# mountain/qingdai

Measured on AMD Instinct MI355X. Metric: simulated planet-days/sec at 721x1440 f64, higher is better.
Workload: dtype f64; 1 GPU; 721x1440 seed-42 planet, dt=300 s: forcing + time_step(Teq, dt, albedo) with QD_ENERGY_W=1 QD_CLOUD_COUPLE=1 + slab-ocean coupling + driver-side precipitation/cloud/albedo diagnostics (run_simulation.py:1766-1934,2063-2146) (BASELINE configs[2]; loop order of benchmark_jax.py:124-158); ocean_n_sub=13, parallelism=lat-bands x1

## Files before the change

include/qingdai_hip.h:

```cpp
#ifndef QINGDAI_HIP_H
#define QINGDAI_HIP_H

#include <stddef.h>
#include <stdint.h>

#ifdef __cplusplus
extern "C" {
#endif

#define QD_ABI_VERSION 1

typedef struct qd_ctx* qd_handle;

typedef struct qd_grid_desc {
    int32_t n_lat, n_lon;
    int32_t row0, n_rows, halo;
    int32_t device;
    int32_t rank, world;
} qd_grid_desc;

enum qd_field {
    QD_F_U = 0, QD_F_V, QD_F_H, QD_F_TS, QD_F_Q, QD_F_CLOUD, QD_F_HICE,
    QD_F_ISR, QD_F_ISR_A, QD_F_ISR_B, QD_F_TEQ, QD_F_ALBEDO,
    QD_F_OLR, QD_F_EFLUX, QD_F_PCOND, QD_F_LH, QD_F_LHREL, QD_F_CLOUD_EFF,
// ... 45 lines not shown
int qd_device_count(void);
int qd_create(const qd_grid_desc* desc, const qd_params* params, double q_init_rh, qd_handle* out);
int qd_destroy(qd_handle h);
const char* qd_last_error(qd_handle h);

int qd_upload(qd_handle h, int field, const void* host_global, size_t bytes);
int qd_download(qd_handle h, int field, void* host_global, size_t bytes);
int qd_set_params(qd_handle h, const qd_params* params, size_t sizeof_params);
int qd_get_step_counter(qd_handle h, int64_t* atmos_counter, int64_t* ocean_counter);
int qd_set_step_counter(qd_handle h, int64_t atmos_counter, int64_t ocean_counter);

int qd_forcing(qd_handle h, const double star_a[3], const double star_b[3], double theta, int with_teq);
int qd_simple_albedo(qd_handle h, double ocean_albedo);
int qd_atmos_step(qd_handle h, double dt, int has_albedo);
int qd_ocean_step(qd_handle h, double dt, int compute_qnet, int use_ice_mask, int inject_sst);
int qd_driver_physics(qd_handle h, double dt);
int qd_hydrology_commit(qd_handle h, double dt);
int qd_step_n(qd_handle h, int n, double dt, int flags, const double* stars);
int qd_last_ocean_nsub(qd_handle h, int* n_sub);
int qd_sync(qd_handle h);

int qd_op_laplacian(qd_handle h, const double* F, int cos_kind, double* out);
int qd_op_hyperdiffuse(qd_handle h, const double* F, const double* k4_row, double k4_scalar, double dt,
                       int n_substeps, int cos_kind, double* out);
int qd_op_advect(qd_handle h, const double* field, const double* u, const double* v, double dt,
                 int cos_kind, double* out);
int qd_op_shapiro(qd_handle h, const double* F, int n, double* out);
int qd_op_zonal_filter(qd_handle h, const double* F, double cutoff, double damp, double* out);
int qd_op_divergence(qd_handle h, const double* u, const double* v, double* out);
int qd_op_vorticity(qd_handle h, const double* u, const double* v, double* out);
int qd_op_gaussian(qd_handle h, const double* F, double sigma, int mode_wrap, double* out);
int qd_op_median_positive(qd_handle h, const double* x, double dflt, double* out);
int qd_median_state(qd_handle h, double* out64);

int qd_band_insolation(qd_handle h, int nb, const double* specA, const double* specB, const double* tray, double* out_host_or_null);

typedef struct qd_eco_params {
    double k_canopy;
    double leaf_scalar;
    double soil_ref;
    double w_lai;
    double light_update_hours;
    double recompute_lai_delta;
    int32_t substep_every_nphys;
    int32_t albedo_couple;
    int32_t bands_couple;
    int32_t water_couple;
    int32_t use_lai;
    int32_t map_f32;
} qd_eco_params;
int qd_eco_configure(qd_handle h, const qd_eco_params* p, size_t sizeof_params);
int qd_eco_set_lai_layers(qd_handle h, const double* layers, int n_planes, int init);
int qd_eco_substep(qd_handle h, double dt);
int qd_eco_banded_alpha(qd_handle h, int nb, const double* r_eff, const double* w_b);
int qd_eco_get_state(qd_handle h, double out[5]);
int qd_eco_set_state(qd_handle h, const double in[3]);

int qd_indiv_configure(qd_handle h, int n_cells, const int32_t* sample_j, const int32_t* sample_i, int n_indiv,
                       const int32_t* cell_index, const double* Ab, const double* tol, int nb, const double* specA,
                       const double* specB, const double* tray, int substeps_per_day, double day_seconds, double soil_cap,
                       int ab_f32);
int qd_indiv_substep(qd_handle h, double dt, int* fired_or_null);
int qd_indiv_download(qd_handle h, double* E_day, double* stress_days);
int qd_indiv_upload(qd_handle h, const double* E_day, const double* stress_days);

int qd_phyto_configure(qd_handle h, int n_species, double K_h, double adv_alpha);
// ... 266 lines not shown
```

qingdai_amd/_lib.py:

```python
from __future__ import annotations

import ctypes
import os

from .params import qd_params

_HERE = os.path.dirname(os.path.abspath(__file__))
LIB_PATH = os.environ.get("QD_LIB_PATH") or os.path.join(_HERE, "libqingdai_hip.so")

FIELDS = ["U", "V", "H", "TS", "Q", "CLOUD", "HICE", "ISR", "ISR_A", "ISR_B", "TEQ", "ALBEDO",
          "OLR", "EFLUX", "PCOND", "LH", "LHREL", "CLOUD_EFF", "FRICTION", "CSMAP", "BASE_ALBEDO", "ELEVATION",
          "UO", "VO", "ETA", "SST", "QNET", "PRECIP", "CLOUD_FROM_P", "CLOUD_SRC", "W_LAND", "S_SNOW", "C_SNOW",
          "S_SNOW_NEXT", "MELT", "P_RAIN", "GLACIER", "RUNOFF",
          "ECO_LAI", "ECO_LAI_SNAP", "ECO_F", "ECO_EDAY", "ECO_ALPHA", "ECO_ALPHA_BANDED", "WATER_ALPHA",
          "ECO_AGE", "ECO_SEEDBANK", "ECO_GATE", "PHYTO_N", "KD490"]
F = {n: i for i, n in enumerate(FIELDS)}
F["LAND_MASK"] = 100
F["ICE_MASK"] = 101
F.update({"ECO_DIV_LS": 110, "ECO_DIV_ALPHA": 111, "ECO_DIV_BC": 112, "ECO_DIV_SUMMARY": 113})
R_SUM, R_COSMEAN, R_MAX, R_MIN, R_MAXABS = 0, 1, 2, 3, 4

SYMBOLS = [
    "qd_abi_version", "qd_device_count", "qd_create", "qd_destroy", "qd_last_error", "qd_upload", "qd_download", "qd_set_params",
    "qd_get_step_counter", "qd_set_step_counter", "qd_forcing", "qd_simple_albedo", "qd_atmos_step",
    "qd_ocean_step", "qd_driver_physics", "qd_hydrology_commit", "qd_step_n", "qd_last_ocean_nsub", "qd_sync",
    "qd_op_laplacian", "qd_op_hyperdiffuse", "qd_op_advect", "qd_op_shapiro", "qd_op_zonal_filter", "qd_op_divergence",
    "qd_op_vorticity", "qd_op_gaussian", "qd_op_median_positive", "qd_median_state", "qd_reduce", "qd_energy_diagnostics", "qd_energy_diagnostics_last", "qd_band_insolation",
    "qd_comm_unique_id", "qd_comm_init", "qd_comm_init_local", "qd_comm_stats", "qd_comm_allreduce_count", "qd_comm_grouped_sum_count", "qd_comm_init_shm", "qd_comm_host_allreduce_count", "qd_hostring_open", "qd_hostring_allreduce",
    "qd_hostring_close", "qd_comm_barrier", "qd_comm_allreduce_max", "qd_peer_export", "qd_peer_connect", "qd_comm_peer_stats", "qd_comm_peer_carried", "qd_peer_selftest", "qd_peer_disable", "qd_tune_reload",
    "qd_plansim_create", "qd_plansim_destroy", "qd_plansim_plan", "qd_plansim_mark", "qd_plansim_margin", "qd_plansim_segments",
    "qd_plansim_pop_exchange", "qd_plansim_segments_rows",
    "qd_eco_configure", "qd_eco_set_lai_layers", "qd_eco_substep", "qd_eco_banded_alpha", "qd_eco_get_state", "qd_eco_set_state",
    "qd_indiv_configure", "qd_indiv_substep", "qd_indiv_download", "qd_indiv_upload",
    "qd_phyto_configure", "qd_phyto_upload", "qd_phyto_download", "qd_phyto_advect_diffuse",
    "qd_phyto_daily_configure", "qd_phyto_daily", "qd_phyto_daily_schedule", "qd_phyto_daily_log", "qd_phyto_daily_download_bands",
    "qd_phyto_daily_state", "qd_phyto_daily_insolation",
    "qd_eco_daily_configure", "qd_eco_daily_set_layers", "qd_eco_daily_get_layers", "qd_eco_daily_step", "qd_eco_daily_schedule",
    "qd_eco_daily_log", "qd_eco_daily_state", "qd_eco_daily_speciate",
    "qd_eco_state_restore",
    "qd_indiv_daily_configure", "qd_indiv_daily_step", "qd_indiv_daily_log", "qd_indiv_daily_weights", "qd_indiv_daily_state",
    "qd_eco_diversity", "qd_eco_diversity_on", "qd_eco_diversity_download",
    "qd_truecolor_configure", "qd_truecolor_render", "qd_truecolor_download",
    "qd_stateframe_configure", "qd_stateframe_scan", "qd_stateframe_render", "qd_stateframe_download",
    "qd_tiles_configure", "qd_tiles_set_plane", "qd_tiles_available", "qd_tiles_scan", "qd_tiles_order_stats", "qd_tiles_render", "qd_tiles_download",
    "qd_budget_diag_configure", "qd_budget_diag_schedule", "qd_budget_diag_log", "qd_budget_diag_reset",
    "qd_route_configure", "qd_route_free", "qd_route_reset", "qd_route_accumulate", "qd_route_event", "qd_route_schedule",
    "qd_route_download", "qd_route_events",
    "qd_hydronet_build", "qd_hydronet_sweeps",
    "qd_topogen_smooth", "qd_topogen_build", "qd_topogen_last_ms",
    "qd_copy_ceiling", "qd_timing_enable", "qd_timing_select", "qd_timing_get", "qd_timing_reset",
]


class qd_eco_params(ctypes.Structure):
    _fields_ = ([(n, ctypes.c_double) for n in ("k_canopy", "leaf_scalar", "soil_ref", "w_lai", "light_update_hours",
                                                 "recompute_lai_delta")] +
                [(n, ctypes.c_int32) for n in ("substep_every_nphys", "albedo_couple", "bands_couple", "water_couple", "use_lai", "map_f32")])


class qd_phyto_daily_params(ctypes.Structure):
# ... 169 lines not shown
    lib.qd_eco_daily_state.argtypes = [vp, ctypes.POINTER(i64)]
    lib.qd_eco_daily_speciate.argtypes = [vp, i32, ctypes.c_double, dp]
    lib.qd_indiv_daily_configure.argtypes = [vp, ctypes.POINTER(qd_indiv_daily_params), sz, ip, ip]
    lib.qd_indiv_daily_step.argtypes = [vp, vp]
    lib.qd_indiv_daily_log.argtypes = [vp, dp, i32, ip]
    lib.qd_indiv_daily_weights.argtypes = [vp, dp, i32]
    lib.qd_indiv_daily_state.argtypes = [vp, ctypes.POINTER(i64)]
    lib.qd_eco_diversity.argtypes = [vp, vp, i32, i32, dp, dp]
    lib.qd_eco_diversity_on.argtypes = [vp, i32, i32, u8p, vp, i32, i32, dp, dp]
    lib.qd_eco_diversity_download.argtypes = [vp, i32, dp, sz]
    lib.qd_truecolor_configure.argtypes = [vp, ctypes.POINTER(qd_truecolor_params), sz, dp, dp, dp, u8p]
    lib.qd_truecolor_render.argtypes = [vp, i32, dp, dp]
    lib.qd_truecolor_download.argtypes = [vp, i32, vp, sz]
    lib.qd_stateframe_configure.argtypes = [vp, ctypes.POINTER(qd_stateframe_params), sz, u8p]
    lib.qd_stateframe_scan.argtypes = [vp, dp, ctypes.POINTER(i64)]
    lib.qd_stateframe_render.argtypes = [vp, ctypes.POINTER(qd_stateframe_table), sz, dp, i32]
    lib.qd_stateframe_download.argtypes = [vp, i32, vp, sz]
    lib.qd_tiles_configure.argtypes = [vp, dbl, dp, i32, i32]
    lib.qd_tiles_set_plane.argtypes = [vp, dp]
    lib.qd_tiles_available.argtypes = [vp, ip]
    lib.qd_tiles_scan.argtypes = [vp, ctypes.POINTER(qd_tile_ref), i32, dp, ctypes.POINTER(i64)]
    lib.qd_tiles_order_stats.argtypes = [vp, i32, i32, ctypes.POINTER(i64), i32, dp, ctypes.POINTER(i64)]
    lib.qd_tiles_render.argtypes = [vp, ctypes.POINTER(qd_tile_desc), sz, i32, i32]
    lib.qd_tiles_download.argtypes = [vp, i32, vp, sz]
    lib.qd_budget_diag_configure.argtypes = [vp, i32, u8p]
    lib.qd_budget_diag_schedule.argtypes = [vp, i32, ip]
    lib.qd_budget_diag_log.argtypes = [vp, dp, i32, ip]
    lib.qd_budget_diag_reset.argtypes = [vp]
    lib.qd_comm_unique_id.argtypes = [vp, sz]
    lib.qd_comm_init.argtypes = [vp, vp, sz]
    lib.qd_comm_barrier.argtypes = [vp]
    lib.qd_comm_init_local.argtypes = [ctypes.POINTER(vp), i32]
    lib.qd_median_state.argtypes = [vp, dp]
    lib.qd_comm_stats.argtypes = [vp, ctypes.POINTER(i32)]
    lib.qd_comm_allreduce_count.argtypes = [vp, ctypes.POINTER(i32)]
    lib.qd_comm_grouped_sum_count.argtypes = [vp, ctypes.POINTER(i32)]
    lib.qd_comm_init_shm.argtypes = [vp, ctypes.c_char_p]
    lib.qd_comm_host_allreduce_count.argtypes = [vp, ctypes.POINTER(i32)]
    lib.qd_hostring_open.argtypes = [ctypes.c_char_p, i32, i32, ctypes.POINTER(vp)]
    lib.qd_hostring_allreduce.argtypes = [vp, dp, i32, i32]
    lib.qd_hostring_close.argtypes = [vp]
    lib.qd_comm_allreduce_max.argtypes = [vp, dp, i32]
    lib.qd_tune_reload.argtypes = [vp]
    lib.qd_peer_export.argtypes = [vp, vp, sz]
    lib.qd_peer_connect.argtypes = [vp, vp, sz, i32]
    lib.qd_peer_selftest.argtypes = [vp, i32, ctypes.POINTER(ctypes.c_longlong)]
    lib.qd_peer_disable.argtypes = [vp]
    lib.qd_comm_peer_stats.argtypes = [vp, ctypes.POINTER(i32), ctypes.POINTER(i32)]
    lib.qd_comm_peer_carried.argtypes = [vp]
    lib.qd_plansim_create.argtypes = [ctypes.POINTER(qd_grid_desc), ctypes.POINTER(vp)]
    lib.qd_plansim_destroy.argtypes = [vp]
    lib.qd_plansim_plan.argtypes = [vp, ip, ip, i32, i32]
    lib.qd_plansim_mark.argtypes = [vp, ip, i32, i32]
    lib.qd_plansim_margin.argtypes = [vp, i32]
    lib.qd_plansim_segments.argtypes = [vp, i32, ip]
    lib.qd_plansim_pop_exchange.argtypes = [vp, ip, i32, ip]
    lib.qd_plansim_segments_rows.argtypes = [vp, i32, i32, ip]
    lib.qd_route_configure.argtypes = [vp, ctypes.POINTER(qd_route_plan), sz]
    lib.qd_route_free.argtypes = [vp]
    lib.qd_route_reset.argtypes = [vp]
    lib.qd_route_accumulate.argtypes = [vp, dbl]
    lib.qd_route_event.argtypes = [vp, dbl, i32]
    lib.qd_route_schedule.argtypes = [vp, i32, dp]
    lib.qd_route_download.argtypes = [vp, i32, dp, sz]
    lib.qd_route_events.argtypes = [vp, dp, i32, ip]
    lib.qd_hydronet_build.argtypes = [vp, i32, i32, u8p, dp, dbl, i32, dp, dp, dp, dbl, dp, ip, ip, u8p, ip, ip, i32,
# ... 15 lines not shown
```

qingdai_amd/csrc/qd_api.hip:

```cpp
#include "qd_span.h"
#include <chrono>
#include <atomic>
#include <cstring>
#include <cstdio>
#include <cstdlib>
#include <algorithm>

thread_local std::string g_qd_create_err;

int qd_fail(qd_ctx* c, const char* what, hipError_t e) {
    std::string m = what ? what : "error";
    if (e != hipSuccess) { m += ": "; m += hipGetErrorString(e); }
    if (c) c->err = m; else g_qd_create_err = m;
    return -1;
}

static hipEvent_t qd_get_event(qd_ctx* c) {
    if (!c->ev_free.empty()) { hipEvent_t e = c->ev_free.back(); c->ev_free.pop_back(); return e; }
    hipEvent_t e = nullptr;
    hipEventCreate(&e);
    return e;
}
QdScope::QdScope(qd_ctx* c_, const char* n, bool attach_) : c(c_), name(n), attach(attach_) {
    on = c->timing == 1;
// ... 260 lines not shown
    { const int r = geti("QD_TAIL_RP", 0); if (r >= 3) t.tail_rp = r; }
    t.tail_v = geti("QD_TAIL_V", 0) == 1 ? 1 : 0;
    t.tail_general = geti("QD_TAIL_GENERAL", 0) == 1 ? 1 : 0;
    t.stream_r_dyn = std::max(0, geti("QD_STREAM_R_DYN", 0));
    t.stream_r_ocn = std::max(0, geti("QD_STREAM_R_OCN", 0));
    t.stream_vb = geti("QD_STREAM_VB", -1);
    { const int b = geti("QD_MED_BLOCKS", 0); if (b >= 16) t.med_blocks = b; }
    t.shapiro_r = std::max(0, geti("QD_SHAPIRO_R", 0));
    t.tile_tr = std::max(0, geti("QD_TILE_TR", 0));
    t.fused_r = std::max(0, geti("QD_FUSED_R", 0));
    t.fused_seq = geti("QD_FUSED_SEQ", 0) == 1 ? 1 : 0;
    t.fused_norot = geti("QD_FUSED_NOROT", 0) == 1 ? 1 : 0;
    t.stream_no_pair = geti("QD_STREAM_NO_PAIR", 0) == 1 ? 1 : 0;
}
extern "C" int qd_tune_reload(qd_handle c) { if (!c) return -1; qd_read_tuning(c); c->tile = QdTileShape{0, 0, 0, 0}; return 0; }

extern "C" int qd_create(const qd_grid_desc* d, const qd_params* params, double q_init_rh, qd_handle* out) {
    if (!d || !params || !out) return qd_fail(nullptr, "qd_create: null argument");
    if (d->n_lat < 5 || d->n_lon < 4) return qd_fail(nullptr, "qd_create: grid too small (need n_lat>=5, n_lon>=4)");
    if (d->row0 < 0 || d->n_rows < 1 || d->row0 + d->n_rows > d->n_lat || d->halo < 0)
        return qd_fail(nullptr, "qd_create: bad latitude band");
    const bool full = (d->row0 == 0 && d->n_rows == d->n_lat);
    if (full && d->halo != 0) return qd_fail(nullptr, "qd_create: a whole-globe handle takes halo = 0");
    if (!full && d->n_rows + 2 * d->halo > d->n_lat) return qd_fail(nullptr, "qd_create: band + 2 halos taller than the grid");
    if (!full && d->halo < 5) return qd_fail(nullptr, "qd_create: band handles need halo >= 5 rows");
    int ndev = 0;
    if (hipGetDeviceCount(&ndev) != hipSuccess || ndev == 0) return qd_fail(nullptr, "qd_create: no HIP device visible");
    if (d->device < 0 || d->device >= ndev) return qd_fail(nullptr, "qd_create: bad device ordinal");
    qd_ctx* c = new qd_ctx();
    c->desc = *d; c->p = *params;
    { const char* ef = std::getenv("QD_FUSED"); if (ef && ef[0] == '0') c->use_fused = 0; }
    { const char* ef = std::getenv("QD_FUSED_FAST"); if (ef) c->fused_fast = std::atoi(ef); }
    { const char* ef = std::getenv("QD_TAIL_ACC"); if (ef) c->tail_acc = std::atoi(ef); }
    { const char* ef = std::getenv("QD_SHAPIRO_STREAM"); if (ef) c->shapiro_stream = std::atoi(ef); }
    { const char* ef = std::getenv("QD_OCN_TAIL"); if (ef) c->ocn_tail = std::atoi(ef); }
    if (c->ocn_tail != 0) c->ocn_tail = 1;
    { const char* ef = std::getenv("QD_OCN_FUSED"); if (ef) c->ocn_fused = ef[0] == '1' ? 1 : 0; }
    { const char* ef = std::getenv("QD_BAND_TAIL"); if (ef) c->band_tail = ef[0] == '0' ? 0 : 1; }
    qd_read_tuning(c);
    { const char* ef = std::getenv("QD_GROUP_SUMS"); if (ef) c->group_sums = ef[0] == '0' ? 0 : 1; }
    c->geo = QdGeom{d->n_lat, d->n_lon, d->row0, d->n_rows, d->halo, full ? 1 : 0, d->row0 - d->halo, d->n_rows + 2 * d->halo};
    c->own_row0 = d->row0; c->own_nrows = d->n_rows;
    auto bail = [&](const char* w, hipError_t e) { qd_fail(nullptr, w, e); qd_destroy(c); return -1; };
    hipError_t e;
    if ((e = hipSetDevice(d->device)) != hipSuccess) return bail("hipSetDevice", e);
    if ((e = hipStreamCreate(&c->stream)) != hipSuccess) return bail("hipStreamCreate", e);
    { int ncu = 0; c->n_cu = (hipDeviceGetAttribute(&ncu, hipDeviceAttributeMultiprocessorCount, d->device) == hipSuccess && ncu > 0) ? ncu : 256; }
    const size_t cells = c->geo.cells() + (size_t)QD_PAD_ROWS * c->geo.nlon;
    for (int f = 0; f < QD_F_COUNT_F64; ++f) {
        if ((e = hipMalloc(&c->f[f], cells * sizeof(double))) != hipSuccess) return bail("hipMalloc field", e);
        hipMemsetAsync(c->f[f], 0, cells * sizeof(double), c->stream);
    }
    for (int s = 0; s < QD_NSCRATCH; ++s) {
        if ((e = hipMalloc(&c->scratch[s], cells * sizeof(double))) != hipSuccess) return bail("hipMalloc scratch", e);
        hipMemsetAsync(c->scratch[s], 0, cells * sizeof(double), c->stream);
    }
    if ((e = hipMalloc(&c->land, cells)) != hipSuccess) return bail("hipMalloc mask", e);
    if ((e = hipMalloc(&c->icemask, cells)) != hipSuccess) return bail("hipMalloc mask", e);
    hipMemsetAsync(c->land, 0, cells, c->stream); hipMemsetAsync(c->icemask, 0, cells, c->stream);
    if (build_tables(c)) return bail("table allocation", hipErrorOutOfMemory);
    if ((e = hipMalloc(&c->k4_atm, (size_t)5 * d->n_lat * sizeof(double))) != hipSuccess) return bail("hipMalloc", e);
    if ((e = hipMalloc(&c->k4_ocn, (size_t)3 * d->n_lat * sizeof(double))) != hipSuccess) return bail("hipMalloc", e);
    c->red_blocks = (12 + (d->n_lon + QD_BLOCK - 1) / QD_BLOCK) * c->geo.lrows() + 64;
    if ((e = hipMalloc(&c->red_partial, (size_t)c->red_blocks * sizeof(double))) != hipSuccess) return bail("hipMalloc", e);
    if ((e = hipMalloc(&c->dscal, QD_S_COUNT * sizeof(double))) != hipSuccess) return bail("hipMalloc", e);
    if ((e = hipMalloc(&c->dcount, 32 * sizeof(unsigned long long))) != hipSuccess) return bail("hipMalloc", e);
    if ((e = hipMalloc(&c->eta_acc, 512 * sizeof(unsigned long long))) != hipSuccess) return bail("hipMalloc", e);
    hipMemsetAsync(c->eta_acc, 0, 512 * sizeof(unsigned long long), c->stream);
    if ((e = hipMalloc(&c->hist, 2 * QD_HIST_BINS * sizeof(unsigned int))) != hipSuccess) return bail("hipMalloc", e);
    if ((e = hipMalloc(&c->sel_state, 8 * sizeof(unsigned long long))) != hipSuccess) return bail("hipMalloc", e);
    hipMemsetAsync(c->dscal, 0, QD_S_COUNT * sizeof(double), c->stream);
    hipMemsetAsync(c->dcount, 0, 32 * sizeof(unsigned long long), c->stream);
    hipMemsetAsync(c->hist, 0, 2 * QD_HIST_BINS * sizeof(unsigned int), c->stream);
    hipMemsetAsync(c->sel_state, 0, 8 * sizeof(unsigned long long), c->stream);
    { const char* ef = std::getenv("QD_TAIL_FIX"); if (ef) c->tail_fix = ef[0] == '0' ? 0 : 1; }
    c->fix_dense = 256.0 * (double)c->geo.cells() / (721.0 * 1440.0);
    { const char* ef = std::getenv("QD_TAIL_FIX_DENSE"); if (ef) c->fix_dense = std::atof(ef); }
    { const char* ef = std::getenv("QD_LAZY_DIAG"); if (ef) c->lazy_diag = ef[0] == '0' ? 0 : 1; }
    if (c->tail_fix) {
        if ((e = hipMalloc(&c->fix_count, 64)) != hipSuccess) return bail("hipMalloc", e);
        hipMemsetAsync(c->fix_count, 0, 64, c->stream);
        if ((e = hipMalloc(&c->fix_list, c->geo.cells() * 3 * sizeof(unsigned long long))) != hipSuccess) return bail("hipMalloc", e);
    }
    if (!full) {
        if ((e = hipMalloc(&c->med_pred, 64 * sizeof(double))) != hipSuccess) return bail("hipMalloc", e);
        hipMemsetAsync(c->med_pred, 0, 64 * sizeof(double), c->stream);
        if ((e = hipMalloc(&c->med_gather, (size_t)std::max(1, d->world) * 4096 * sizeof(double))) != hipSuccess) return bail("hipMalloc", e);
        if ((e = hipMalloc(&c->sel_ccount, 2 * sizeof(unsigned int))) != hipSuccess) return bail("hipMalloc", e);
        hipMemsetAsync(c->sel_ccount, 0, 2 * sizeof(unsigned int), c->stream);
        { const char* ef = std::getenv("QD_MEDIAN_PREDICT"); if (ef && ef[0] == '0') c->med_predict = 0; }
    }
    if (full) {
        if ((e = hipMalloc(&c->sel_cand, 2 * cells * sizeof(double))) != hipSuccess) return bail("hipMalloc", e);
        if ((e = hipMalloc(&c->sel_ccount, 2 * sizeof(unsigned int))) != hipSuccess) return bail("hipMalloc", e);
        hipMemsetAsync(c->sel_ccount, 0, 2 * sizeof(unsigned int), c->stream);
        if ((e = hipMalloc(&c->med_pred, 64 * sizeof(double))) != hipSuccess) return bail("hipMalloc", e);
        hipMemsetAsync(c->med_pred, 0, 64 * sizeof(double), c->stream);
        { const char* ef = std::getenv("QD_MEDIAN_PREDICT"); if (ef && ef[0] == '0') c->med_predict = 0; }
        { const char* ef = std::getenv("QD_MERGE_POINTWISE"); if (ef) c->merge_pointwise = ef[0] == '0' ? 0 : 1; }
        { const char* ef = std::getenv("QD_HOIST_PRECIP"); if (ef) c->hoist_precip = ef[0] == '0' ? 0 : 1; }
        { const char* ef = std::getenv("QD_SIDE_STREAM"); if (ef) c->side_stream_on = ef[0] == '0' ? 0 : 1; }
// ... 425 lines not shown
}
extern "C" int qd_op_divergence(qd_handle c, const double* u, const double* v, double* out) { return seam_divvort(c, u, v, out, 0); }
extern "C" int qd_op_vorticity(qd_handle c, const double* u, const double* v, double* out) { return seam_divvort(c, u, v, out, 1); }

extern "C" int qd_op_gaussian(qd_handle c, const double* F, double sigma, int mode_wrap, double* out) {
    if (!c || !F || !out) return -1;
    hipSetDevice(c->desc.device);
    if (seam_in(c, c->scratch[10], F)) return -1;
    if (qd_gaussian(c, c->scratch[10], c->scratch[11], c->scratch[12], sigma, mode_wrap, 0)) return -1;
    return seam_out(c, c->scratch[11], out);
}

extern "C" int qd_op_median_positive(qd_handle c, const double* x, double dflt, double* out) {
    if (!c || !x || !out) return -1;
    hipSetDevice(c->desc.device);
    if (seam_in(c, c->scratch[10], x)) return -1;
    qd_median_positive_dev(c, c->scratch[10], dflt, QD_S_MED_OUT, 0, 0.0, 0);
    QD_HIP(c, hipMemcpyAsync(c->hpin, c->dscal + QD_S_MED_OUT, sizeof(double), hipMemcpyDeviceToHost, c->stream));
    QD_HIP(c, hipStreamSynchronize(c->stream));
    *out = c->hpin[0];
    return 0;
}

extern "C" int qd_median_state(qd_handle c, double* out64) {
    if (!c || !out64) return -1;
    hipSetDevice(c->desc.device);
    for (int k = 0; k < 16 * 4; ++k) out64[k] = 0.0;
    if (!c->med_pred) return 0;
    QD_HIP(c, hipStreamSynchronize(c->stream));
    QD_HIP(c, hipMemcpy(out64, c->med_pred, sizeof(double) * 16 * 4, hipMemcpyDeviceToHost));
    return 0;
}

extern "C" int qd_reduce(qd_handle c, int field, int op, double* out) {
    if (!c || !out) return -1;
    if (field < 0 || field >= QD_F_COUNT_F64) return qd_fail(c, "qd_reduce: unknown field");
    hipSetDevice(c->desc.device);
    double v = 0;
    const int op1 = (op == QD_R_COSWEIGHTED_MEAN) ? 1 : (op == QD_R_SUM ? 0 : (op == QD_R_MAX ? 2 : (op == QD_R_MIN ? 3 : 4)));
    if (qd_reduce_field(c, c->f[field], op1, &v)) return -1;
    if (op == QD_R_COSWEIGHTED_MEAN) v = v / (c->wsum_all + 1e-15);
    *out = v;
    return 0;
}

extern "C" int qd_band_insolation(qd_handle c, int nb, const double* specA, const double* specB, const double* tray, double* out_host) {
    if (!c || !specA || !specB || !tray) return -1;
    hipSetDevice(c->desc.device);
    return qd_band_insolation_impl(c, nb, specA, specB, tray, out_host);
}
extern "C" int qd_energy_diagnostics_last(qd_handle c, double* out) {
    if (!c || !out) return -1;
    for (int k = 0; k < 10; ++k) out[k] = c->last_diag[k];
    return 0;
}
extern "C" int qd_energy_diagnostics(qd_handle c, double* out) {
    if (!c || !out) return -1;
    hipSetDevice(c->desc.device);
    return qd_energy_diag_impl(c, out);
}

extern "C" int qd_copy_ceiling(qd_handle c, size_t bytes, int reps, double* gbs) {
    if (!c || !gbs || bytes == 0 || reps < 1) return -1;
    hipSetDevice(c->desc.device);
    void *a = nullptr, *b = nullptr;
    if (hipMalloc(&a, bytes) != hipSuccess || hipMalloc(&b, bytes) != hipSuccess) { if (a) hipFree(a); return qd_fail(c, "qd_copy_ceiling: hipMalloc"); }
// ... 32 lines not shown
```

qingdai_amd/csrc/qd_blockred.h:

```cpp
#pragma once
#include "qd_internal.h"

__device__ __forceinline__ double qd_wave_sum(double x) {
#pragma unroll
    for (int o = 32; o > 0; o >>= 1) x += __shfl_down(x, o, 64);
    return x;
}
__device__ __forceinline__ double qd_wave_max(double x) {
#pragma unroll
    for (int o = 32; o > 0; o >>= 1) { double y = __shfl_down(x, o, 64); x = (y > x) ? y : x; }
    return x;
}
__device__ __forceinline__ double qd_wave_fmin(double x) {
#pragma unroll
    for (int o = 32; o > 0; o >>= 1) x = fmin(x, __shfl_down(x, o, 64));
    return x;
}
__device__ __forceinline__ double qd_wave_fmax(double x) {
#pragma unroll
    for (int o = 32; o > 0; o >>= 1) x = fmax(x, __shfl_down(x, o, 64));
    return x;
}

__device__ __forceinline__ double qd_pow_np(double x, double e) {
// ... 36 lines not shown
    const int q = threadIdx.x;
    if (q < count) partial[(size_t)q * nblk + b] = qd_block_total(sm, q, qd_red_op(op, q));
}

template <int N>
__device__ __forceinline__ void qd_planes_strided(const double* __restrict__ partial, int nblk, int planes, const QdRedOp* op, double (&v)[N]) {
#pragma unroll
    for (int q = 0; q < N; ++q)
        if (q < planes) {
            const QdRedOp o = qd_red_op(op, q);
            double a = qd_red_identity(o);
            for (int k = threadIdx.x; k < nblk; k += QD_BLOCK) a = qd_red_join(a, partial[(size_t)q * nblk + k], o);
            v[q] = a;
        }
}
template <int N>
__device__ __forceinline__ void qd_block_totals(double (&v)[N], const QdRedOp* op) {
    __shared__ double sm[N][QD_BLOCK / 64];
    qd_block_gather(sm, v, N, op);
    if (threadIdx.x == 0)
        for (int q = 0; q < N; ++q) v[q] = qd_block_total(sm, q, qd_red_op(op, q));
}

__device__ __forceinline__ void qd_planes_by_wave(const double* __restrict__ partial, int nblk, int planes, double* tot) {
    const int lane = threadIdx.x & 63, wv = threadIdx.x >> 6;
    for (int q = wv; q < planes; q += QD_BLOCK / 64) {
        double a = 0.0;
        for (int k = lane; k < nblk; k += 64) a += partial[(size_t)q * nblk + k];
        a = qd_wave_sum(a);
        if (lane == 0) tot[q] = a;
    }
    __syncthreads();
}
```

qingdai_amd/csrc/qd_fused.h:

```cpp
#pragma once
#include "qd_internal.h"

struct QdDynArgs {
    const double *u, *v, *h, *fric, *q, *cloud;
    double *uo, *vo, *ho, *qo, *co;
    const double* k4row[5];
    double k4s[5];
    int skip[5];
    double g, a, dt, dlat, dlon, f_min;
    double inv_dlon, inv_2dlon, inv_dlat, inv_2dlat, pgf_y;
    int primitive;
    int fast;
    QdTileShape ts;
};


struct QdOcnArgs {
    const double *uo, *vo, *eta, *taux, *tauy;
    const uint8_t* land;
    double *uo_out, *vo_out, *eta_out;
    const double* k4row[3];
    double k4s[3];
    int skip[3];
    double a, g, dlat, dlon, sub_dt, rhoH, r_bot;
    double inv_2dlon, inv_2dlat, inv_a, inv_rhoH;
    const double* eta_mean;
    double eta_cap;
    int fast;
    QdTileShape ts;
};


QdTileShape qd_pick_tile(const QdGeom& G);
int qd_launch_dyn_hyper(qd_ctx* c, QdDynArgs& P, int margin);
int qd_launch_ocn_hyper(qd_ctx* c, QdOcnArgs& P, int margin);

bool qd_stream_ok(const qd_ctx* c, int margin);
bool qd_ocn_stream_ok(const qd_ctx* c, int margin);
int qd_launch_dyn_stream(qd_ctx* c, const QdDynArgs& P, int margin);
int qd_launch_ocn_stream(qd_ctx* c, const QdOcnArgs& P, int margin);
bool qd_ocn_stream_ok_list(const qd_ctx* c, const QdSegList& S);
int qd_launch_ocn_stream_list(qd_ctx* c, const QdOcnArgs& P, const QdSegList& S);
```

qingdai_amd/csrc/qd_fused.hip:

```cpp
#include "qd_internal.h"
#include "qd_device.h"
#include "qd_fused.h"
#include "qd_wave.h"
#include <cstdlib>
#include <algorithm>

#define QD_TC 58
#define QD_S 64
#define QD_FBLOCK 512
#define QD_NW (QD_FBLOCK / 64)

struct QdLapC {
    double dphi, dlam, a;
    int n;
    const double* poleA;
    const double *sA, *sP, *sQ;
};

__device__ __forceinline__ int qd_pole_type(int g, int n) { return g == 0 ? 0 : (g == 1 ? 1 : (g == n - 2 ? 2 : (g == n - 1 ? 3 : -1))); }

__device__ __forceinline__ double qd_lap_lds_pole(const double* __restrict__ p, int g, int rho, const QdLapC& C) {
    const int S = QD_S, t = qd_pole_type(g, C.n);
    const double cc = p[0];
    double ahi = cc, alo, bhi, blo = cc;
// ... 672 lines not shown
    QdDynArgs Q = P;
    QD_ROWS(c, margin, G, Q.ts.ntr = (G.nrows + TR - 1) / TR; hipLaunchKernelGGL(k_dyn_hyper<TR>, dim3(Q.ts.ntr * Q.ts.ntc), dim3(QD_FBLOCK),
                                             QdPl<TR>::lds_bytes, c->stream, G, c->tabs, Q));
}
template <int TR> static void launch_ocn(qd_ctx* c, const QdOcnArgs& P, int margin) {
    static bool once[QD_MAX_DEVICES] = {false};
    const int dv = c->desc.device >= 0 && c->desc.device < QD_MAX_DEVICES ? c->desc.device : 0;
    if (!once[dv]) { hipFuncSetAttribute((const void*)k_ocn_hyper<TR>, hipFuncAttributeMaxDynamicSharedMemorySize, (int)QdPl<TR>::lds_bytes); once[dv] = c->desc.device == dv; }
    QdOcnArgs Q = P;
    QD_ROWS(c, margin, G, Q.ts.ntr = (G.nrows + TR - 1) / TR; hipLaunchKernelGGL(k_ocn_hyper<TR>, dim3(Q.ts.ntr * Q.ts.ntc), dim3(QD_FBLOCK),
                                             QdPl<TR>::lds_bytes, c->stream, G, c->tabs, Q));
}

#define QD_DISPATCH_TR(tr, CALL)                                                                              \
    switch (tr) {                                                                                             \
        case 6: CALL(6); break; case 10: CALL(10); break; case 14: CALL(14); break; case 18: CALL(18); break; \
        case 22: CALL(22); break; case 26: CALL(26); break; case 30: CALL(30); break; case 38: CALL(38); break; \
        default: return qd_fail(c, "fused kernel: no instantiation for this tile height");                    \
    }

int qd_launch_dyn_hyper(qd_ctx* c, QdDynArgs& P, int margin) {
    if (qd_stream_ok(c, margin)) return qd_launch_dyn_stream(c, P, margin);
    qd_tile_init(c);
    P.ts = c->tile;
    P.fast = c->fused_fast != 0;
    QdScope sc(c, "k_dyn_hyper");
#define QD_CALL_DYN(N) launch_dyn<N>(c, P, margin)
    QD_DISPATCH_TR(P.ts.tr, QD_CALL_DYN)
    return 0;
}

int qd_launch_ocn_hyper(qd_ctx* c, QdOcnArgs& P, int margin) {
    if (qd_ocn_stream_ok(c, margin)) return qd_launch_ocn_stream(c, P, margin);
    qd_tile_init(c);
    P.ts = c->tile;
    P.fast = c->fused_fast != 0;
    QdScope sc(c, "k_ocn_hyper");
#define QD_CALL_OCN(N) launch_ocn<N>(c, P, margin)
    QD_DISPATCH_TR(P.ts.tr, QD_CALL_OCN)
    return 0;
}
```

qingdai_amd/csrc/qd_internal.h:

```cpp
#pragma once

#include <hip/hip_runtime.h>
#include <hip/hip_ext.h>
#include <stdint.h>
#include <string>
#include <vector>
#include <functional>
#include <map>
#include <unordered_map>
#include <initializer_list>
#include <climits>
#include <cfloat>
#include <cmath>

#include "../../include/qingdai_hip.h"

#define QD_NSCRATCH 16
#define QD_MAX_DEVICES 64
#define QD_PAD_ROWS 8
#define QD_BLOCK 256
#define QD_MAXF 5
#define QD_HIST_BINS 2048

struct QdGeom {
// ... 184 lines not shown
    hipEvent_t med_fork = nullptr, med_done = nullptr;
    unsigned int* hist_b = nullptr; unsigned long long* sel_state_b = nullptr; double* sel_cand_b = nullptr; unsigned int* sel_ccount_b = nullptr;
    int want_pcond_ahead = 0;
    int pcond_ahead = 0;
    int tail_fix = 1;
    unsigned int* fix_count = nullptr;
    unsigned long long* fix_list = nullptr;
    double fix_avg = 0.0;
    double fix_dense = 256.0;
    int64_t fix_probe_at = 0;
    int fix_probe_every = 32;
    int merge_saf = 1;
    void* saf_pending = nullptr;
    int defer_final = 0;
    int merge_final = 1;
    struct { int on = 0; double dt = 0, decay = 0, dfac = 0; } final_pending;
    double* wgmax = nullptr;
    int n_wgmax = 0;
    int side_stream_on = 0;
    hipStream_t side_stream = nullptr;
    hipEvent_t side_fork = nullptr, side_done = nullptr;
    bool side_pending = false;
    double* red_partial_b = nullptr;
    std::function<int()> before_cfl_wait;
    int merge_pointwise = 1;
    double* med_gather = nullptr;
    double* hpin = nullptr;
    double* hpin_rows = nullptr;
    double wsum_ocean = 0, wsum_all = 0;
    int64_t atm_counter = 0, ocn_counter = 0;
    QdTileShape tile{0, 0, 0, 0};
    int use_fused = 1;
    int fused_fast = 1;
    int tail_acc = 1;
    unsigned long long* eta_acc = nullptr;
    int shapiro_stream = 1;
    int ocn_fused = 0;
    int ocn_tail = 1;
    int stream_rows = 0;
    double* qs_tab[2] = {nullptr, nullptr};
    double qs_key[2][8] = {{NAN, 0, 0, 0, 0, 0, 0, 0}, {NAN, 0, 0, 0, 0, 0, 0, 0}};
    std::vector<double> h_lapK[2];
    std::vector<double> h_k4[2];
    QdTune tune;
    int n_cu = 0;
    int qs_wgs_per_cu[3] = {0, 0, 0};
    int cloud_eff_valid = 0;
    int last_nsub = 0;
    void* stage = nullptr; size_t stage_bytes = 0;
    std::unordered_map<const void*, int> vm;
    int own_row0 = 0, own_nrows = 0;
    void* comm = nullptr;
    struct QdLocalGroup* lgroup = nullptr;
    struct QdPeer* peer = nullptr;
    std::vector<struct QdUse> split_pending;
    std::vector<struct QdUse> corefresh;
    int exchanges = 0;
    int allreduces = 0;
    double pub_seq = 0.0;
    double eta_seq = 0.0;
    void* hring = nullptr;
    void* plansim = nullptr;
    int host_allreduces = 0;
    const char* lap_tag = "k_laplacian";
    const char* hyp_tag = "k_hyper_apply";
    int timing = 0;
// ... 77 lines not shown
int qd_allgather_f64(qd_ctx* c, double* buf, int n_per_rank);
bool qd_peer_on(const qd_ctx* c);
int qd_host_allreduce(qd_ctx* c, double* host_vals, int n, int op);
bool qd_has_host_ring(const qd_ctx* c);
extern "C" int qd_hostring_close(void* ring);
void qd_comm_release(qd_ctx* c);
#define QD_ROWS(c, margin, G, ...) do { QdSegs _sg = qd_segments((c), (margin)); for (int _k = 0; _k < _sg.n; ++_k) { const QdGeom& G = _sg.g[_k]; __VA_ARGS__; } } while (0)

static inline dim3 qd_grid2d(const QdGeom& G, int fields = 1) {
    return dim3((G.nlon + QD_BLOCK - 1) / QD_BLOCK, G.nrows, fields);
}

struct QdFieldList {
    const double* in[QD_MAXF];
    double* out[QD_MAXF];
    const double* aux[QD_MAXF];
    const double* k4row[QD_MAXF];
    double k4s[QD_MAXF];
    int n;
};

void qd_launch_laplacian(qd_ctx* c, const QdFieldList& fl, const double* coslat, int m);
void qd_launch_hyper_apply(qd_ctx* c, const QdFieldList& fl, const double* coslat, double sub_dt, int m);
int  qd_hyperdiffuse_fields(qd_ctx* c, double** fields, int n, const double* k4tab, const int* skip,
                            const double* k4s_override, double dt, int nsub, const double* coslat, int m_out);
void qd_launch_shapiro_pass(qd_ctx* c, const QdFieldList& fl, int scrub, int m);
int  qd_shapiro_fields(qd_ctx* c, double** fields, int n, int npass, int m_out);
void qd_launch_advect(qd_ctx* c, const double* u, const double* v, const double* coslat, double dt,
                      const double* f0, double* o0, const double* f1, double* o1, double alpha, int clipq, int m);
void qd_launch_divvort(qd_ctx* c, const double* u, const double* v, double* out, int vort, int m);
int  qd_gaussian(qd_ctx* c, const double* in, double* out, double* tmp, double sigma, int mode_wrap, int m_out, int clip01 = 0,
                 const double* scale_p = nullptr, double scale_k = 1.0);
bool qd_gauss_pair_ok(const qd_ctx* c, double sigma);
int  qd_gaussian_pair(qd_ctx* c, const double* inA, const double* inB, double sigma, int mode_wrap, const double* scA_p, double scA_k,
                      double scB_k, const double* sc, int op, const double* blend5, double* outA, double* outB, double* out0, int m_out = 0);
int  qd_gaussian_swap(qd_ctx* c, double*& field, double*& tmp, double sigma, int mode_wrap, int m_out, int clip01 = 0,
                      const double* scale_p = nullptr, double scale_k = 1.0);
bool qd_gauss_can_fuse(const qd_ctx* c, double sigma);
int  qd_gauss_radius(double sigma);
int  qd_energy_diag_impl(qd_ctx* c, double* host_out);
int  qd_band_insolation_impl(qd_ctx* c, int nb, const double* specA, const double* specB, const double* tray, double* out_host);
int  qd_zonal_filter_fields(qd_ctx* c, double** fields, int nf, double cutoff, double damp, int m);
int  qd_adv_reach(const qd_ctx* c, double dt, double vmax);

int  qd_eco_canopy_impl(qd_ctx* c, double dt);
int  qd_eco_eday_impl(qd_ctx* c, double dt);
int  qd_indiv_substep_impl(qd_ctx* c, double dt, int* fired);
void qd_eco_free(qd_ctx* c);
int  qd_band_copy_in(qd_ctx* c, void* dst, const void* host, size_t esz);
int  qd_phyto_step_impl(qd_ctx* c, double dt);
void qd_phyto_release(qd_ctx* c);
struct QdSpanLane* qd_route_span_begin(qd_ctx* c, int n);
int  qd_route_step_impl(qd_ctx* c, double dt, int s);
void qd_route_release(qd_ctx* c);
struct QdSpanLane* qd_phyto_daily_span_begin(qd_ctx* c, int n, int with_phys);
int  qd_phyto_daily_step_impl(qd_ctx* c, const double* star_row, int use_sst);
void qd_phyto_daily_release(qd_ctx* c);
struct QdSpanLane* qd_eco_daily_span_begin(qd_ctx* c, int n, int with_eco);
int  qd_eco_daily_step_impl(qd_ctx* c, const double* soil_dev);
void qd_eco_daily_release(qd_ctx* c);
bool qd_eco_daily_stack(const qd_ctx* c, const double** L, int* n_species, int* n_layers);
double* qd_eco_daily_share_plane(qd_ctx* c);
double* qd_eco_daily_weights_dev(qd_ctx* c);
double qd_eco_daily_soil_cap(const qd_ctx* c);
double qd_eco_daily_lai_max(const qd_ctx* c);
void qd_eco_daily_adopt(qd_ctx* c, double* L1, double* w1);
struct QdSpanLane* qd_indiv_daily_span_begin(qd_ctx* c, const struct QdSpanLane* daily);
int  qd_indiv_daily_step_impl(qd_ctx* c, const double* soil_dev);
// ... 45 lines not shown
```

qingdai_amd/csrc/qd_ocean.hip:

```cpp
#include <cstdlib>
#include <atomic>
#include <chrono>
#include "qd_internal.h"
#include "qd_device.h"
#include "qd_wave.h"

#include "qd_fluxes.h"
#include "qd_fused.h"
#include "qd_ocntail.h"
#include "qd_band.h"
#include "qd_blockred.h"

QdColP qd_make_colp(const qd_ctx* c, double dt);

__global__ void __launch_bounds__(QD_BLOCK)
k_qnet(QdGeom G, QdColP P, const double* __restrict__ isr, const double* __restrict__ albedo,
       const double* __restrict__ cloud, const double* __restrict__ Ts, const double* __restrict__ h,
       const double* __restrict__ u, const double* __restrict__ v, const uint8_t* __restrict__ land,
       const double* __restrict__ hice, const double* __restrict__ LH, double* __restrict__ qnet,
       uint8_t* __restrict__ icemask) {
    const QdTile tl = qd_tile();
    const int j = tl.seg * QD_BLOCK + threadIdx.x;
    if (j >= G.nlon) return;
    const size_t o = (size_t)qd_lrow(G, G.row0 + tl.row) * G.nlon + j;
// ... 762 lines not shown
        c->last_nsub = n_sub;
    }
    bool fix_now = c->tail_fix && c->fix_count && (!band || band_fix_stats);
    if (fix_now) {
        if (c->fix_avg <= c->fix_dense) c->fix_probe_every = 32;
        else if (step >= c->fix_probe_at) {
            c->fix_probe_at = step + c->fix_probe_every;
            c->fix_probe_every = std::min(256, c->fix_probe_every * 2);
        } else fix_now = false;
    }
    const double sub_dt = dt / n_sub;
    QdOcnP OP{p.a, p.g_ocean, c->dlat, c->dlon, sub_dt, p.rho_w * H, p.r_bot};
    QdHeatP HP{sub_dt, p.K_h, p.rho_w * p.cp_w * H, p.ocean_ice_qfac, p.ocean_use_qnet ? 1 : 0, use_ice_mask ? 1 : 0};
    const bool do_diff = (p.ocean_diff_every > 0) && (step % p.ocean_diff_every == 0);
    const bool do_shap = (p.ocean_shapiro_n > 0) && (p.ocean_shapiro_every > 0) && (step % p.ocean_shapiro_every == 0);
    if (do_diff) { int rc = qd_build_k4_tables(c, dt, true, sub_dt); if (rc) return rc; }
    const double ov[3] = {p.ocean_k4_u, p.ocean_k4_v, p.ocean_k4_eta};
    const int Ro = qd_adv_reach(c, sub_dt, 4.0);

    const bool can_defer = do_diff && c->use_fused && p.ocean_k4_nsub == 1 && !do_shap && c->wsum_ocean > 0.0;
    const bool band_defer = band && can_defer && qd_has_host_ring(c);
    const bool band_tail = band && can_defer && !band_defer && c->ocn_tail == 1 && c->tail_acc && c->band_tail && G0.nlon >= 64 &&
                           G0.halo >= std::max(7, Ro + 2);
    const bool defer_eta = (!band && can_defer) || band_defer || band_tail;
    double* const mean_ptr = band_defer ? c->hpin + 42 : c->dscal + QD_S_ETA_MEAN;
    struct CoRefresh { qd_ctx* c; ~CoRefresh() { c->corefresh.clear(); } } corefresh_guard{c};
    if (band) c->corefresh = {QD_IN(F[QD_F_UO], 0), QD_IN(F[QD_F_VO], 0), QD_IN(F[QD_F_ETA], 0), QD_IN(F[QD_F_SST], 0), QD_IN(taux, 0),
                              QD_IN(tauy, 0), QD_IN(F[QD_F_QNET], 0), QD_IN8(c->icemask, 0)};
    const bool use_tail = c->use_fused && (!band || band_tail) && defer_eta && G0.nlon >= 64 && c->ocn_tail;
    const bool tail_acc = use_tail && c->tail_acc;
    const bool use_fused1 = use_tail && !band && c->ocn_fused && c->ocn_tail == 1 && tail_acc && c->fused_fast == 1 && do_diff &&
                            p.ocean_k4_nsub == 1 && !do_shap && HP.use_q && HP.K_h > 0.0 && qd_ocn_fused_ok(c) &&
                            !c->k4_ocn_skip[0] && !c->k4_ocn_skip[1] && !c->k4_ocn_skip[2];
    for (int s = 0; s < n_sub; ++s) {
        if (use_fused1) {
            QdOcnArgs O;
            O.uo = F[QD_F_UO]; O.vo = F[QD_F_VO]; O.eta = F[QD_F_ETA]; O.taux = taux; O.tauy = tauy; O.land = c->land;
            O.uo_out = qd_scratch(c, 0); O.vo_out = qd_scratch(c, 1); O.eta_out = qd_scratch(c, 6);
            for (int f = 0; f < 3; ++f) {
                const bool sc1 = !(ov[f] != ov[f]);
                O.k4row[f] = sc1 ? nullptr : c->k4_ocn + (size_t)f * G0.nlat;
                O.k4s[f] = sc1 ? ov[f] : 0.0;
                O.skip[f] = c->k4_ocn_skip[f];
            }
            O.a = p.a; O.g = p.g_ocean; O.dlat = c->dlat; O.dlon = c->dlon; O.sub_dt = sub_dt; O.rhoH = p.rho_w * H; O.r_bot = p.r_bot;
            O.inv_2dlon = 1.0 / (2.0 * c->dlon); O.inv_2dlat = 1.0 / (2.0 * c->dlat); O.inv_a = 1.0 / p.a; O.inv_rhoH = 1.0 / (p.rho_w * H);
            O.eta_mean = s > 0 ? mean_ptr : nullptr;
            O.eta_cap = p.eta_cap;
            QdTailArgs A;
            A.uo = O.uo_out; A.vo = O.vo_out; A.eta_in = O.eta_out; A.Ts = F[QD_F_SST]; A.qnet = F[QD_F_QNET]; A.land = c->land; A.ice = c->icemask;
            A.eta = qd_scratch(c, 2); A.Ts_out = qd_scratch(c, 3); A.uo_out = qd_scratch(c, 12); A.vo_out = qd_scratch(c, 13); A.partial = c->red_partial;
            A.a = p.a; A.dlat = c->dlat; A.dlon = c->dlon; A.sub_dt = sub_dt; A.msdtH = -sub_dt * H; A.alpha = p.ocean_adv_alpha;
            A.K_h = HP.K_h; A.rcH = HP.rcH; A.ice_qfac = HP.ice_qfac; A.cap = p.ocean_max_u;
            A.use_q = HP.use_q; A.has_ice = HP.has_ice; A.mean4 = p.ocean_outlier == 0 ? 1 : 0;
            A.r_a = 1.0 / p.a; A.r_dlon = 1.0 / c->dlon; A.r_dlat = 1.0 / c->dlat; A.r_2dlon = 1.0 / (2 * c->dlon); A.r_2dlat = 1.0 / (2 * c->dlat);
            A.r_rcH = 1.0 / HP.rcH;
            A.acc = c->eta_acc; A.mean_out = c->dscal + QD_S_ETA_MEAN; A.wsum = c->wsum_ocean;
            if (qd_launch_ocn_fused(c, O, A)) return -1;
            qd_swap(c, QD_F_UO, 12); qd_swap(c, QD_F_VO, 13); qd_swap(c, QD_F_ETA, 2); qd_swap(c, QD_F_SST, 3);
            continue;
        }
        if (do_diff && c->use_fused && p.ocean_k4_nsub == 1) {
            const QdUse narrow[5] = {QD_IN(F[QD_F_ETA], 5), QD_IN(F[QD_F_UO], 4), QD_IN(F[QD_F_VO], 4), QD_IN(taux, 4), QD_IN(tauy, 4)};
            bool pending = false;
            int m_old = 0;
            if (band_tail) {
                const QdUse wide[8] = {QD_IN(F[QD_F_ETA], 7), QD_IN(F[QD_F_UO], 6), QD_IN(F[QD_F_VO], 6), QD_IN(taux, 6), QD_IN(tauy, 6),
                                       QD_IN(F[QD_F_SST], Ro + 2), QD_IN(F[QD_F_QNET], 0), QD_IN8(c->icemask, 0)};
                if (qd_plan_begin(c, wide, 8, &pending) < 0) return -1;
                if (pending) m_old = qd_plan_peek(c, narrow, 5);
            }
            QdOcnArgs O;
            O.uo = F[QD_F_UO]; O.vo = F[QD_F_VO]; O.eta = F[QD_F_ETA]; O.taux = taux; O.tauy = tauy; O.land = c->land;
            O.uo_out = qd_scratch(c, 0); O.vo_out = qd_scratch(c, 1); O.eta_out = qd_scratch(c, 2);
            for (int f = 0; f < 3; ++f) {
                const bool sc1 = !(ov[f] != ov[f]);
                O.k4row[f] = sc1 ? nullptr : c->k4_ocn + (size_t)f * G0.nlat;
                O.k4s[f] = sc1 ? ov[f] : 0.0;
                O.skip[f] = c->k4_ocn_skip[f];
            }
            O.a = p.a; O.g = p.g_ocean; O.dlat = c->dlat; O.dlon = c->dlon; O.sub_dt = sub_dt; O.rhoH = p.rho_w * H; O.r_bot = p.r_bot;
            O.inv_2dlon = 1.0 / (2.0 * c->dlon); O.inv_2dlat = 1.0 / (2.0 * c->dlat); O.inv_a = 1.0 / p.a; O.inv_rhoH = 1.0 / (p.rho_w * H);
            O.eta_mean = (defer_eta && s > 0) ? mean_ptr : nullptr;
            O.eta_cap = p.eta_cap;
            int m_int = 0;
            bool split = false;
            if (pending) {
                m_int = m_old >= 0 ? m_old : -12;
                const QdSegList Si = qd_segments_rows(c, c->own_row0 - m_int, c->own_nrows + 2 * m_int);
                if (c->own_nrows + 2 * m_int >= 12 && qd_ocn_stream_ok_list(c, Si)) {
                    if (qd_launch_ocn_stream_list(c, O, Si)) return -1;
                    split = true;
                }
                if (qd_plan_end(c)) return -1;
            }
            const int m = qd_plan(c, narrow, 5);
            if (m < 0) return -1;
            if (qd_allreduce_flush(c)) return -1;
            if (split && m > m_int) {
                QdSegList Sb = qd_segments_rows(c, c->own_row0 - m, m - m_int);
                Sb = qd_segments_rows(c, c->own_row0 + c->own_nrows + m_int, m - m_int, Sb);
                if (!qd_ocn_stream_ok_list(c, Sb)) {
                    if (qd_launch_ocn_hyper(c, O, m)) return -1;
                } else if (qd_launch_ocn_stream_list(c, O, Sb)) return -1;
            } else if (!split) {
                if (qd_launch_ocn_hyper(c, O, m)) return -1;
            }
            qd_mark(c, {O.uo_out, O.vo_out, O.eta_out}, m);
            qd_swap(c, QD_F_UO, 0); qd_swap(c, QD_F_VO, 1); qd_swap(c, QD_F_ETA, 2);
        } else {
            {
                QdScope sc(c, "ocean_momentum");
                const int m = qd_plan(c, {QD_IN(F[QD_F_ETA], 1), QD_IN(F[QD_F_UO], 0), QD_IN(F[QD_F_VO], 0), QD_IN(taux, 0),
                                          QD_IN(tauy, 0)});
                if (m < 0) return -1;
                QD_ROWS(c, m, G, hipLaunchKernelGGL(k_ocean_momentum, qd_grid2d(G), blk, 0, c->stream, G, c->tabs, OP,
                                                    F[QD_F_ETA], taux, tauy, c->land, F[QD_F_UO], F[QD_F_VO]));
// ... 23 lines not shown
            QdTailArgs A;
            A.uo = F[QD_F_UO]; A.vo = F[QD_F_VO]; A.Ts = F[QD_F_SST]; A.qnet = F[QD_F_QNET]; A.land = c->land; A.ice = c->icemask;
            A.eta = F[QD_F_ETA]; A.Ts_out = qd_scratch(c, 1); A.uo_out = qd_scratch(c, 2); A.vo_out = qd_scratch(c, 3); A.partial = c->red_partial;
            A.a = p.a; A.dlat = c->dlat; A.dlon = c->dlon; A.sub_dt = sub_dt; A.msdtH = -sub_dt * H; A.alpha = p.ocean_adv_alpha;
            A.K_h = HP.K_h; A.rcH = HP.rcH; A.ice_qfac = HP.ice_qfac; A.cap = p.ocean_max_u;
            A.use_q = HP.use_q; A.has_ice = HP.has_ice; A.mean4 = p.ocean_outlier == 0 ? 1 : 0;
            A.r_a = 1.0 / p.a; A.r_dlon = 1.0 / c->dlon; A.r_dlat = 1.0 / c->dlat; A.r_2dlon = 1.0 / (2 * c->dlon); A.r_2dlat = 1.0 / (2 * c->dlat);
            A.r_rcH = 1.0 / HP.rcH;
            A.acc = tail_acc ? c->eta_acc : nullptr; A.mean_out = c->dscal + QD_S_ETA_MEAN; A.wsum = c->wsum_ocean;
            if (band) {
                const int m = qd_plan(c, {QD_IN(F[QD_F_UO], 2), QD_IN(F[QD_F_VO], 2), QD_IN(F[QD_F_ETA], 0), QD_IN(F[QD_F_SST], Ro + 2),
                                          QD_IN(F[QD_F_QNET], 0), QD_IN8(c->icemask, 0)});
                if (m < 0) return -1;
                A.own0 = c->own_row0; A.own1 = c->own_row0 + c->own_nrows;
                QdSegs S = qd_segments(c, m);
                size_t off = 0;
                QdPeerFold pf;
                const bool folded = qd_peer_fold_begin(c, &pf);
                if (fix_now && S.n == 1) { A.fix_count = c->fix_count; A.fix_list = c->fix_list; }
                for (int k = 0; k < S.n; ++k) {
                    const QdGeom& Gs = S.g[k];
                    const bool owned = Gs.row0 <= c->own_row0 && c->own_row0 < Gs.row0 + Gs.nrows;
                    A.acc = owned ? c->eta_acc : nullptr;
                    A.pf = owned ? pf : QdPeerFold();
                    A.partial = c->red_partial + off;
                    if (qd_launch_ocn_tail(c, Gs, A)) return -1;
                    off += (size_t)qd_ocn_tail_tiles(c, Gs);
                }
                if (!folded && qd_allreduce_sum_deferred(c, c->dscal + QD_S_ETA_MEAN)) return -1;
                if (A.fix_count) qd_mark(c, {F[QD_F_ETA], A.Ts_out, F[QD_F_UO], F[QD_F_VO]}, m);
                else qd_mark(c, {F[QD_F_ETA], A.Ts_out, A.uo_out, A.vo_out}, m);
            } else {
            if (fix_now) { A.fix_count = c->fix_count; A.fix_list = c->fix_list; }
            if (qd_launch_ocn_tail(c, Gown, A)) return -1;
            if (!tail_acc)
                hipLaunchKernelGGL(k_eta_mean_tail, dim3(1), dim3(256), 0, c->stream, c->red_partial, qd_ocn_tail_tiles(c, Gown), c->wsum_ocean,
                                   c->dscal + QD_S_ETA_MEAN);
            }
            qd_swap(c, QD_F_SST, 1);
            if (!A.fix_count) { qd_swap(c, QD_F_UO, 2); qd_swap(c, QD_F_VO, 3); }
        } else if (c->use_fused) {
            QdScope sc(c, "ocean_cont_sst");
            bool band_raw_mean = false;
            const int m = qd_plan(c, {QD_IN(F[QD_F_UO], 1), QD_IN(F[QD_F_VO], 1), QD_IN(F[QD_F_ETA], 0), QD_IN(F[QD_F_SST], Ro)});
            if (m < 0) return -1;
            double* T1 = qd_scratch(c, 0);
            const int own0 = c->own_row0, own1 = c->own_row0 + c->own_nrows;
            const int has_ocean = c->wsum_ocean > 0.0 ? 1 : 0;
            if (!band) {
                const dim3 g2 = qd_grid2d(Gown);
                hipLaunchKernelGGL(k_cont_sstadv, g2, blk, 0, c->stream, Gown, c->tabs, p.a, c->dlat, c->dlon, -sub_dt * H, sub_dt,
                                   p.ocean_adv_alpha, F[QD_F_UO], F[QD_F_VO], c->land, F[QD_F_ETA], F[QD_F_SST], T1, own0, own1,
                                   c->red_partial, (unsigned long long*)nullptr, 0.0, (double*)nullptr);
                if (!defer_eta)
                    hipLaunchKernelGGL(k_eta_mean, dim3(1), blk, 0, c->stream, c->red_partial, (int)(g2.x * g2.y), c->wsum_ocean,
                                       c->dscal + QD_S_ETA_MEAN);
            } else {
                QdSegs S = qd_segments(c, m);
                size_t off = 0;
                for (int k = 0; k < S.n; ++k) {
                    hipLaunchKernelGGL(k_cont_sstadv, qd_grid2d(S.g[k]), blk, 0, c->stream, S.g[k], c->tabs, p.a, c->dlat, c->dlon,
                                       -sub_dt * H, sub_dt, p.ocean_adv_alpha, F[QD_F_UO], F[QD_F_VO], c->land, F[QD_F_ETA],
                                       F[QD_F_SST], T1, own0, own1, c->red_partial + off, (unsigned long long*)nullptr, 0.0,
                                       (double*)nullptr);
                    off += (size_t)S.g[k].nrows * qd_grid2d(S.g[k]).x;
                }
// ... 126 lines not shown
```

qingdai_amd/csrc/qd_ocntail.h:

```cpp
#pragma once
#include "qd_internal.h"
#include "qd_peer_dev.h"

struct QdTailArgs {
    const double *uo, *vo, *Ts, *qnet;
    const uint8_t *land, *ice;
    double *eta, *Ts_out, *uo_out, *vo_out, *partial;
    const double* tab;
    unsigned long long* acc;
    double* mean_out;
    double wsum;
    double a, dlat, dlon, sub_dt, msdtH, alpha, K_h, rcH, ice_qfac, cap;
    double r_a, r_dlon, r_dlat, r_2dlon, r_2dlat, r_rcH;
    int use_q, has_ice, mean4, ntc, R, Rp;
    int nmid, flags;
    int own0, own1;
    const double* eta_in = nullptr;
    unsigned int* fix_count = nullptr;
    unsigned long long* fix_list = nullptr;
    QdPeerFold pf;
};

int qd_ocn_tail_tiles(const qd_ctx* c, const QdGeom& G);
int qd_launch_ocn_tail(qd_ctx* c, const QdGeom& G, QdTailArgs& P);

struct QdOcnArgs;
bool qd_ocn_fused_ok(const qd_ctx* c);
int qd_ocn_fused_tiles(const qd_ctx* c);
int qd_launch_ocn_fused(qd_ctx* c, const QdOcnArgs& O, QdTailArgs& P);
```

qingdai_amd/csrc/qd_ocntail.hip:

```cpp
#include "qd_internal.h"
#include "qd_device.h"
#include "qd_wave.h"
#include "qd_ocntail.h"
#include "qd_stream.h"
#include "qd_blockred.h"
#include <cstdlib>
#include <cstdio>
#include <vector>
#include <cstring>
#include <algorithm>


__device__ __forceinline__ double qt_div(double x, double c, double rc) {
    const double q0 = x * rc;
    const double e = __builtin_fma(-c, q0, x);
    const double q1 = __builtin_fma(e, rc, q0);
    return (q0 - q0 == 0.0) ? q1 : q0;
}

__device__ __forceinline__ double qt_div_fin(double x, double c, double rc) {
    const double q0 = x * rc;
    const double e = __builtin_fma(-c, q0, x);
    return __builtin_fma(e, rc, q0);
}
// ... 561 lines not shown
    const int k = rs - (q.ps > 0 ? 1 : 0);
    if (q.ps > 0 && rs == 0) { W.o0 = lo; W.o1 = lo + q.ps; }
    else if (k < q.nmid) {
        const int M = q.mid1 - q.mid0;
        W.o0 = q.mid0 + (int)(((long long)k * M) / q.nmid);
        W.o1 = q.mid0 + (int)(((long long)(k + 1) * M) / q.nmid);
    } else { W.o0 = q.mid1; W.o1 = hi; }
    const int wv = __builtin_amdgcn_readfirstlane(threadIdx.x >> 6);
    const bool plain = (P.flags & 1) == 0 && W.o0 - 3 - W.lbase >= 0 && W.o1 + 2 - W.lbase <= W.lrows - 1;
    QT_STAMP(0);
    if (wv >= 1) {
        __builtin_amdgcn_s_setprio(2);
        bool general = !(plain && W.o0 >= 3 && W.o1 <= W.n - 3 && P.use_q && P.K_h > 0.0);
        if (!general) {
            const bool edge_lane = W.lane >= 1 && W.lane <= 62 && (W.j == 0 || W.j == W.m - 1);
            general = __builtin_amdgcn_ballot_w64(edge_lane) != 0ull ? qt_sst_fast<true>(P, W) : qt_sst_fast<false>(P, W);
        }
        if (general) qt_sst_wave(G, T, P, W);
        QT_STAMP(2);
        if (!FIX) return;
        __syncthreads();
        return;
    }
    __shared__ unsigned long long s_fix[FIX ? 3 * QT_FIX_STAGE : 1];
    __shared__ unsigned int s_nfix;
    const QtFixW FX{P.fix_count, P.fix_list, s_fix, &s_nfix};
    if (FIX && W.lane == 0) __hip_atomic_store(&s_nfix, 0u, __ATOMIC_RELAXED, __HIP_MEMORY_SCOPE_WAVEFRONT);
    double acc = (plain && W.o0 >= 1 && W.o1 <= W.n - 1) ? qt_currents_fast<FIX>(P, W, FX) : qt_currents_wave<FIX>(T, P, W, FX);
    if (FIX) qt_fix_flush(FX);
    QT_STAMP(2);
    if (FIX) __syncthreads();
    acc = qd_wave_sum(acc);
    if (W.lane == 0) __hip_atomic_store(P.partial + w, acc, __ATOMIC_RELAXED, __HIP_MEMORY_SCOPE_AGENT);
    if (P.acc) {
        const bool last = W.lane == 0 && qd_acc_arrive(P.acc, w, gridDim.x, acc);
        if (__builtin_amdgcn_ballot_w64(last) != 0ull) {
            double mm = qd_acc_finish(P.acc, P.partial, (int)gridDim.x, P.wsum);
            if (P.pf.pbox) mm = qp_fold_sum(P.pf, mm);
            if (W.lane == 0) *P.mean_out = mm;
            if (FIX) {
                const unsigned nfix = __hip_atomic_load(P.fix_count, __ATOMIC_RELAXED, __HIP_MEMORY_SCOPE_AGENT);
                for (unsigned k0 = 0; k0 < nfix; k0 += 512u) {
                    unsigned long long off[8], ub[8], vb[8];
#pragma unroll
                    for (int q = 0; q < 8; ++q) {
                        const unsigned k = k0 + (unsigned)q * 64u + (unsigned)W.lane;
                        const unsigned long long* e = P.fix_list + (size_t)3 * (k < nfix ? k : nfix - 1u);
                        off[q] = __hip_atomic_load(e, __ATOMIC_RELAXED, __HIP_MEMORY_SCOPE_AGENT);
                        ub[q] = __hip_atomic_load(e + 1, __ATOMIC_RELAXED, __HIP_MEMORY_SCOPE_AGENT);
                        vb[q] = __hip_atomic_load(e + 2, __ATOMIC_RELAXED, __HIP_MEMORY_SCOPE_AGENT);
                    }
#pragma unroll
                    for (int q = 0; q < 8; ++q) {
                        if (k0 + (unsigned)q * 64u + (unsigned)W.lane >= nfix) continue;
                        *(unsigned long long*)((char*)const_cast<double*>(P.uo) + off[q]) = ub[q];
                        *(unsigned long long*)((char*)const_cast<double*>(P.vo) + off[q]) = vb[q];
                    }
                }
                if (W.lane == 0) {
                    __hip_atomic_store(P.fix_count, 0u, __ATOMIC_RELAXED, __HIP_MEMORY_SCOPE_AGENT);
                    P.fix_count[4] += nfix; P.fix_count[5] += 1u; if (nfix > P.fix_count[6]) P.fix_count[6] = nfix;
                }
            }
        }
    }
}
// ... 227 lines not shown
    A.G = c->geo;
    if (F.ntc * (1 + F.nmid) > c->red_blocks) return qd_fail(c, "k_ocn_fused: partial buffer too small");
    if (!c->qt_tab || c->qt_tab_a != P.a) {
        if (!c->qt_tab) {
            if (hipMalloc(&c->qt_tab, (size_t)c->geo.nlat * 16 * sizeof(double)) != hipSuccess) return qd_fail(c, "k_ocn_fused: row table");
            c->tab_alloc.push_back(c->qt_tab);
        }
        hipLaunchKernelGGL(k_tail_tab, dim3((c->geo.nlat + 255) / 256), dim3(256), 0, c->stream, c->tabs, c->geo.nlat, P.a, c->qt_tab);
        c->qt_tab_a = P.a;
    }
    P.tab = c->qt_tab; P.own0 = 0; P.own1 = c->geo.nlat; P.flags = 0; P.R = F.R; P.Rp = QFU_PH; P.ntc = F.ntc; P.nmid = F.nmid;
    QdScope sc(c, "ocean_step", true);
#ifdef QT_STAMPS
    static unsigned long long* stamps = nullptr;
    const size_t stamp_words = (size_t)8 * 5 * 8192;
    if (!stamps) { hipMalloc(&stamps, stamp_words * 8); hipMemcpyToSymbol(HIP_SYMBOL(qt_stamp_buf), &stamps, sizeof(stamps)); }
    hipMemsetAsync(stamps, 0, stamp_words * 8, c->stream);
#endif
    QD_LAUNCH_TIMED(sc, k_ocn_fused, dim3(F.ntc * (1 + F.nmid)), dim3(320), c->stream, A, c->tabs, P, F);
#ifdef QT_STAMPS
    if (const char* f = std::getenv("QD_STAMPS_FILE")) {
        std::vector<unsigned long long> h(stamp_words);
        hipStreamSynchronize(c->stream);
        hipMemcpy(h.data(), stamps, stamp_words * 8, hipMemcpyDeviceToHost);
        if (FILE* fp = std::fopen(f, "wb")) { std::fwrite(h.data(), 8, stamp_words, fp); std::fclose(fp); }
    }
#endif
    return 0;
}

static int qt_rows(const qd_ctx* c) { return c->tune.tail_r > 0 ? c->tune.tail_r : 7; }

static bool qt_use_fast(const qd_ctx* c) { return !c->tune.tail_v && c->ocn_tail == 1; }
static int qt_fast_rows(const qd_ctx* c, const QdGeom& G) {
    if (c->tune.tail_r > 0) return c->tune.tail_r;
    const int ntc = (G.nlon + QS_TCF - 1) / QS_TCF;
    const double target = 13.7 * 256;
    const int r = (int)std::lround((double)G.nrows * ntc * 2.0 / target);
    return r < 7 ? 7 : r;
}
static int qt_fast_pole_rows(const qd_ctx* c) { return c->tune.tail_rp; }

int qd_ocn_tail_tiles(const qd_ctx* c, const QdGeom& G) {
    if (qt_use_fast(c))
        return qt_part_strips(qt_partition(G.row0, G.row0 + G.nrows, G.nlat, qt_fast_rows(c, G), qt_fast_pole_rows(c))) * ((G.nlon + QS_TCF - 1) / QS_TCF);
    const int R = qt_rows(c);
    return ((G.nrows + R - 1) / R) * ((G.nlon + QS_TC2 - 1) / QS_TC2);
}

int qd_launch_ocn_tail(qd_ctx* c, const QdGeom& G, QdTailArgs& P) {
    if (G.nlon < 64) return qd_fail(c, "k_ocn_tail: >= 64 columns");
    if (G.full) { P.own0 = 0; P.own1 = G.nlat; }
    QdScope sc(c, "ocean_tail", true);
    const bool fast = qt_use_fast(c);
    if (fast && (!c->qt_tab || c->qt_tab_a != P.a)) {
        if (!c->qt_tab) {
            if (hipMalloc(&c->qt_tab, (size_t)G.nlat * 16 * sizeof(double)) != hipSuccess) return qd_fail(c, "k_ocn_tail_fast: row table");
            c->tab_alloc.push_back(c->qt_tab);
        }
        hipLaunchKernelGGL(k_tail_tab, dim3((G.nlat + 255) / 256), dim3(256), 0, c->stream, c->tabs, G.nlat, P.a, c->qt_tab);
        c->qt_tab_a = P.a;
    }
    P.tab = c->qt_tab;
    P.flags = c->tune.tail_general ? 1 : 0;
    P.R = fast ? qt_fast_rows(c, G) : qt_rows(c);
    P.Rp = qt_fast_pole_rows(c);
    P.ntc = fast ? (G.nlon + QS_TCF - 1) / QS_TCF : (G.nlon + QS_TC2 - 1) / QS_TC2;
    const QtPart part = qt_partition(G.row0, G.row0 + G.nrows, G.nlat, P.R, P.Rp);
    P.nmid = part.nmid;
    const int nrs = fast ? qt_part_strips(part) : (G.nrows + P.R - 1) / P.R;
    if (nrs * P.ntc > c->red_blocks) return qd_fail(c, "k_ocn_tail_stream: partial buffer too small");
#ifdef QT_STAMPS
    static unsigned long long* stamps = nullptr;
    const size_t stamp_words = (size_t)8 * 2 * 8192;
    if (!stamps) { hipMalloc(&stamps, stamp_words * 8); hipMemcpyToSymbol(HIP_SYMBOL(qt_stamp_buf), &stamps, sizeof(stamps)); }
    hipMemsetAsync(stamps, 0, stamp_words * 8, c->stream);
#endif
    if (!fast || !P.acc) { P.fix_count = nullptr; P.fix_list = nullptr; }
    if (fast && P.fix_count) QD_LAUNCH_TIMED(sc, k_ocn_tail_fast<true>, dim3(nrs * P.ntc), dim3(128), c->stream, G, c->tabs, P);
    else if (fast) QD_LAUNCH_TIMED(sc, k_ocn_tail_fast<false>, dim3(nrs * P.ntc), dim3(128), c->stream, G, c->tabs, P);
    else QD_LAUNCH_TIMED(sc, k_ocn_tail_stream<1>, dim3(nrs * P.ntc), dim3(128), c->stream, G, c->tabs, P);
#ifdef QT_STAMPS
    if (const char* f = std::getenv("QD_STAMPS_FILE")) {
        std::vector<unsigned long long> h(stamp_words);
        hipStreamSynchronize(c->stream);
        hipMemcpy(h.data(), stamps, stamp_words * 8, hipMemcpyDeviceToHost);
        if (FILE* fp = std::fopen(f, "wb")) { std::fwrite(h.data(), 8, stamp_words, fp); std::fclose(fp); }
    }
#endif
    return 0;
}
```

qingdai_amd/csrc/qd_physics.hip:

```cpp
#include "qd_internal.h"
#include "qd_band.h"
#include "qd_pointwise.h"
#include "qd_device.h"
#include "qd_saf.h"
#include "qd_fluxes.h"
#include "qd_blockred.h"
QdColP qd_make_colp(const qd_ctx* c, double dt);


__global__ void __launch_bounds__(QD_BLOCK)
k_precip_raw(QdGeom G, QdTabs T, const double* __restrict__ u, const double* __restrict__ v,
             const double* __restrict__ pcond, double a, double dlat, double dlon, double D_crit, double beta,
             const double* __restrict__ scale_p, const unsigned long long* __restrict__ sel_state,
             double* __restrict__ praw, double* __restrict__ pos_out, double* __restrict__ partial,
             const double* __restrict__ orog) {
    __shared__ double sm[2][QD_BLOCK / 64];
    const int i = G.row0 + blockIdx.y;
    const size_t b = (size_t)qd_lrow(G, i) * G.nlon;
    const double w = T.warea[i];
    const bool anypos = sel_state[0] > 0;
    const double scale = qd_max(*scale_p, 1e-12);
    double s_num = 0.0, s_den = 0.0;
    for (int j = threadIdx.x; j < G.nlon; j += QD_BLOCK) {
        const double div = qd_divvort_point(G, T, u, v, i, j, a, dlat, dlon, 0);
        const double pos = qd_max(0.0, -(div - D_crit));
        const double F_div = anypos ? qd_clip(pos / scale, 0.0, 5.0) : 0.0;
        const double Pq = qd_max(0.0, pcond[b + j]);
        const double F_orog = orog ? qd_clip(orog[b + j], 1.0, 3.0) : 1.0;
        const double F = (1.0 + beta * F_div) * F_orog;
        const double pr = Pq * F;
        praw[b + j] = pr;
        pos_out[b + j] = pos;
        s_num += Pq * w;
        s_den += pr * w;
    }
    s_num = qd_wave_sum(s_num); s_den = qd_wave_sum(s_den);
    const int lane = threadIdx.x & 63, wv = threadIdx.x >> 6;
    if (lane == 0) { sm[0][wv] = s_num; sm[1][wv] = s_den; }
    __syncthreads();
    if (threadIdx.x == 0) {
        for (int k = 1; k < QD_BLOCK / 64; ++k) { s_num += sm[0][k]; s_den += sm[1][k]; }
        partial[blockIdx.y] = s_num;
        partial[gridDim.y + blockIdx.y] = s_den;
    }
}

__global__ void __launch_bounds__(QD_BLOCK)
k_orog_factor(QdGeom G, QdTabs T, const double* __restrict__ elev, const double* __restrict__ u, const double* __restrict__ v,
              double a, double dlat, double dlon, double k_orog, double cap, double* __restrict__ out) {
    const QdTile tl = qd_tile();
    const int j = tl.seg * QD_BLOCK + threadIdx.x;
    if (j >= G.nlon) return;
    const int i = G.row0 + tl.row, n = G.nlat;
    const size_t b = (size_t)qd_lrow(G, i) * G.nlon;
    const int jp = qd_wrapc(j + 1, G.nlon), jm = qd_wrapc(j - 1, G.nlon);
    const double dx = a * T.cos6[i] * dlon, dy = a * dlat;
    const double dHdx = (elev[b + jp] - elev[b + jm]) / (2.0 * dx);
    double dHdy = 0.0;
    if (i != 0 && i != n - 1)
        dHdy = (elev[(size_t)qd_lrow(G, i + 1) * G.nlon + j] - elev[(size_t)qd_lrow(G, i - 1) * G.nlon + j]) / (2.0 * dy);
    const double gn = sqrt(dHdx * dHdx + dHdy * dHdy);
    const double nxh = gn > 1e-12 ? dHdx / (gn + 1e-12) : 0.0;
    const double nyh = gn > 1e-12 ? dHdy / (gn + 1e-12) : 0.0;
    out[b + j] = qd_clip(1.0 + k_orog * qd_max(0.0, u[b + j] * nxh + v[b + j] * nyh), 1.0, cap);
}

__global__ void __launch_bounds__(QD_BLOCK)
k_precip_scalars(const double* __restrict__ partial, int n, double wsum, double pq_min, double p_blend, int use_fb,
                 double* __restrict__ out) {
    __shared__ double sm[2][QD_BLOCK / 64];
    double a = 0.0, b = 0.0;
    for (int k = threadIdx.x; k < n; k += QD_BLOCK) { a += partial[k]; b += partial[n + k]; }
    a = qd_wave_sum(a); b = qd_wave_sum(b);
    const int lane = threadIdx.x & 63, wv = threadIdx.x >> 6;
    if (lane == 0) { sm[0][wv] = a; sm[1][wv] = b; }
    __syncthreads();
    if (threadIdx.x == 0) {
        for (int k = 1; k < QD_BLOCK / 64; ++k) { a += sm[0][k]; b += sm[1][k]; }
        const double den = b + 1e-20;
        out[0] = den > 0 ? a / den : 1.0;
        const double pq_mean = a / (wsum + 1e-15);
        out[1] = (use_fb && pq_mean < pq_min) ? p_blend : 0.0;
    }
}

__global__ void __launch_bounds__(QD_BLOCK)
k_scale_field(QdGeom G, const double* __restrict__ in, const double* __restrict__ s, double k, double* __restrict__ out) {
    const QdTile tl = qd_tile();
    const int j = tl.seg * QD_BLOCK + threadIdx.x;
    if (j >= G.nlon) return;
    const size_t o = (size_t)qd_lrow(G, G.row0 + tl.row) * G.nlon + j;
    out[o] = s ? in[o] * (*s) : k * in[o];
}

__global__ void __launch_bounds__(QD_BLOCK)
k_precip_blend(QdGeom G, const double* __restrict__ P, const double* __restrict__ Pdyn, const double* __restrict__ sc,
               double* __restrict__ out) {
    const QdTile tl = qd_tile();
    const int j = tl.seg * QD_BLOCK + threadIdx.x;
    if (j >= G.nlon) return;
    const size_t o = (size_t)qd_lrow(G, G.row0 + tl.row) * G.nlon + j;
    const double al = sc[1];
    double p = P[o];
    if (al != 0.0) p = (1.0 - al) * p + al * Pdyn[o];
    out[o] = qd_max(p, 0.0);
}

__global__ void __launch_bounds__(QD_BLOCK)
k_cloud_from_p(QdGeom G, const double* __restrict__ precip, const double* __restrict__ pref, double cmax,
               double* __restrict__ out) {
    const QdTile tl = qd_tile();
    const int j = tl.seg * QD_BLOCK + threadIdx.x;
    if (j >= G.nlon) return;
    const size_t o = (size_t)qd_lrow(G, G.row0 + tl.row) * G.nlon + j;
    out[o] = cmax * qd_tanh(precip[o] / (*pref + 1e-12));
}
// ... 211 lines not shown
                            c->timing != 1;
    if (pcond_side && qd_pcond_median_side(c, dt)) return -1;
    const bool pcond_pair = part != 1 && !pcond_side && c->want_pcond_ahead && c->med_pair && c->hist_b && c->geo.full && p.cloud_couple &&
                            !isset(p.pcond_ref) && !(isset(p.pref) && p.pref != 0.0);
    if (part != 2) {
        QdScope sc(c, "phys_precip");
        int m = qd_plan(c, {QD_IN(F[QD_F_U], 1), QD_IN(F[QD_F_V], 1), QD_IN(F[QD_F_PCOND], 0)});
        if (m < 0) return -1;
        qd_launch_divvort(c, F[QD_F_U], F[QD_F_V], tmp, 0, m);
        if (qd_median_positive_dev(c, tmp, 1e-12, QD_S_PSCALE, 1, p.D_crit, 2)) return -1;
        const double* orog = nullptr;
        if (p.orog_enable && c->has_elevation) {
            double*& of = c->scratch[8];
            const int mo = qd_plan(c, {QD_IN(F[QD_F_U], 0), QD_IN(F[QD_F_V], 0), QD_IN(F[QD_F_ELEVATION], 1)});
            if (mo < 0) return -1;
            QD_ROWS(c, mo, G, hipLaunchKernelGGL(k_orog_factor, qd_grid2d(G), blk, 0, c->stream, G, c->tabs, F[QD_F_ELEVATION],
                                                 F[QD_F_U], F[QD_F_V], p.a, c->dlat, c->dlon, p.orog_k, 2.0, of));
            qd_mark(c, {of}, mo);
            const int mb = qd_plan(c, {QD_IN(of, R1)});
            if (mb < 0) return -1;
            if (qd_gaussian_swap(c, of, tmp, 1.0, 0, mb)) return -1;
            orog = of;
            m = qd_plan(c, {QD_IN(F[QD_F_U], 1), QD_IN(F[QD_F_V], 1), QD_IN(F[QD_F_PCOND], 0), QD_IN(c->scratch[8], 0)});
            if (m < 0) return -1;
        }
        if (band && m > 0) {
            QdSegs S = qd_segments(c, m);
            const int own0 = c->own_row0, own1 = c->own_row0 + c->own_nrows;
            for (int k = 0; k < S.n; ++k) {
                const QdGeom& G = S.g[k];
                auto run = [&](int r0, int r1) {
                    if (r1 <= r0) return;
                    QdGeom g2 = G; g2.row0 = r0; g2.nrows = r1 - r0;
                    hipLaunchKernelGGL(k_precip_raw, dim3(1, g2.nrows), blk, 0, c->stream, g2, c->tabs, F[QD_F_U], F[QD_F_V],
                                       F[QD_F_PCOND], p.a, c->dlat, c->dlon, p.D_crit, p.p_betadiv, c->dscal + QD_S_PSCALE,
                                       c->dcount, praw, pos, rp + (size_t)2 * G0.lrows(), orog);
                };
                const int a0 = G.row0, a1 = G.row0 + G.nrows;
                if (a1 <= own0 || a0 >= own1) run(a0, a1);
                else { run(a0, std::max(a0, own0)); run(std::min(a1, own1), a1); }
            }
        }
        hipLaunchKernelGGL(k_precip_raw, dim3(1, Gown.nrows), blk, 0, c->stream, Gown, c->tabs, F[QD_F_U], F[QD_F_V],
                           F[QD_F_PCOND], p.a, c->dlat, c->dlon, p.D_crit, p.p_betadiv, c->dscal + QD_S_PSCALE, c->dcount, praw,
                           pos, rp, orog);
        qd_mark(c, {praw, pos}, m);
        if (band && qd_peer_hooks(c)) {
            QdPeerHook H; H.pre = 2; H.partial = rp; H.n = Gown.nrows;
            H.post = 1; H.wsum = c->wsum_all; H.pq_min = p.pq_min; H.p_blend = p.p_blend; H.use_fb = p.p_hybrid_fallback; H.out = c->dscal + QD_S_RENORM;
            c->allreduces++;
            if (qd_peer_allreduce_hooked(c, c->dscal + QD_S_TMP0, 2, 0, H)) return -1;
        } else if (band) {
            hipLaunchKernelGGL(k_precip_rawsums, dim3(1), blk, 0, c->stream, rp, Gown.nrows, c->dscal + QD_S_TMP0);
            if (qd_allreduce_f64(c, c->dscal + QD_S_TMP0, 2, 0)) return -1;
            hipLaunchKernelGGL(k_precip_scalars_post, dim3(1), dim3(64), 0, c->stream, c->dscal + QD_S_TMP0, c->wsum_all, p.pq_min,
                               p.p_blend, p.p_hybrid_fallback, c->dscal + QD_S_RENORM);
        } else {
            hipLaunchKernelGGL(k_precip_scalars, dim3(1), blk, 0, c->stream, rp, Gown.nrows, c->wsum_all, p.pq_min,
                               p.p_blend, p.p_hybrid_fallback, c->dscal + QD_S_RENORM);
        }
        if (qd_gauss_pair_ok(c, 1.0)) {
            const int mg = qd_plan(c, {QD_IN(praw, R1), QD_IN(pos, R1)});
            if (mg < 0) return -1;
            if (qd_gaussian_pair(c, praw, pos, 1.0, 0, c->dscal + QD_S_RENORM, 1.0, p.k_precip, c->dscal + QD_S_RENORM, 1, nullptr,
                                 nullptr, nullptr, F[QD_F_PRECIP], mg)) return -1;
            qd_mark(c, {F[QD_F_PRECIP]}, mg);
        } else if (qd_gauss_can_fuse(c, 1.0)) {
            const int mg = qd_plan(c, {QD_IN(praw, R1), QD_IN(pos, R1)});
            if (mg < 0) return -1;
            if (qd_gaussian_swap(c, praw, tmp, 1.0, 0, mg, 0, c->dscal + QD_S_RENORM)) return -1;
            if (qd_gaussian(c, pos, pdyn, nullptr, 1.0, 0, mg, 0, nullptr, p.k_precip)) return -1;
            QD_ROWS(c, mg, G, hipLaunchKernelGGL(k_precip_blend, qd_grid2d(G), blk, 0, c->stream, G, praw, pdyn,
                                                 c->dscal + QD_S_RENORM, F[QD_F_PRECIP]));
            qd_mark(c, {F[QD_F_PRECIP]}, mg);
        } else {
        QD_ROWS(c, m, G, hipLaunchKernelGGL(k_scale_field, qd_grid2d(G), blk, 0, c->stream, G, praw, c->dscal + QD_S_RENORM, 0.0, praw));
        QD_ROWS(c, m, G, hipLaunchKernelGGL(k_scale_field, qd_grid2d(G), blk, 0, c->stream, G, pos, (const double*)nullptr,
                                            p.k_precip, pdyn));
        qd_mark(c, {pdyn}, m);
        const int mg = qd_plan(c, {QD_IN(praw, R1), QD_IN(pdyn, R1)});
        if (mg < 0) return -1;
        if (qd_gaussian_swap(c, praw, tmp, 1.0, 0, mg)) return -1;
        if (qd_gaussian_swap(c, pdyn, tmp, 1.0, 0, mg)) return -1;
        QD_ROWS(c, mg, G, hipLaunchKernelGGL(k_precip_blend, qd_grid2d(G), blk, 0, c->stream, G, praw, pdyn,
                                             c->dscal + QD_S_RENORM, F[QD_F_PRECIP]));
        qd_mark(c, {F[QD_F_PRECIP]}, mg);
        }
    }
    if (part == 1) return 0;
    {
        QdScope sc(c, "phys_cloud");
        if (isset(p.pref) && p.pref != 0.0) {
            hipMemcpyAsync(c->dscal + QD_S_MED_OUT, &p.pref, sizeof(double), hipMemcpyHostToDevice, c->stream);
        } else if (pcond_pair) {
// ... 185 lines not shown
```

qingdai_amd/csrc/qd_stencil.hip:

```cpp
#include "qd_internal.h"
#include "qd_device.h"
#include "qd_wave.h"
#include <cstdlib>

__global__ void __launch_bounds__(QD_BLOCK)
k_laplacian(QdGeom G, QdFieldList fl, const double* __restrict__ cosf, double dphi, double dlam, double a) {
    const QdTile tl = qd_tile();
    const int j = tl.seg * QD_BLOCK + threadIdx.x;
    if (j >= G.nlon) return;
    const int i = G.row0 + tl.row;
    const int f = tl.fld;
    const size_t o = (size_t)qd_lrow(G, i) * G.nlon + j;
    fl.out[f][o] = qd_lap_point<true>(fl.in[f], G, cosf, i, j, dphi, dlam, a);
}

__global__ void __launch_bounds__(QD_BLOCK)
k_hyper_apply(QdGeom G, QdFieldList fl, const double* __restrict__ cosf, double dphi, double dlam, double a,
              double sub_dt) {
    const QdTile tl = qd_tile();
    const int j = tl.seg * QD_BLOCK + threadIdx.x;
    if (j >= G.nlon) return;
    const int i = G.row0 + tl.row;
    const int f = tl.fld;
    const size_t o = (size_t)qd_lrow(G, i) * G.nlon + j;
    const double L2 = qd_lap_point<true>(fl.in[f], G, cosf, i, j, dphi, dlam, a);
    const double k4 = fl.k4row[f] ? fl.k4row[f][i] : fl.k4s[f];
    const double F0 = qd_nn(fl.aux[f][o]);
    fl.out[f][o] = qd_nn(F0 - (k4 * L2) * sub_dt);
}

void qd_launch_laplacian(qd_ctx* c, const QdFieldList& fl, const double* coslat, int m) {
    QdScope sc(c, c->lap_tag);
    QD_ROWS(c, m, G, hipLaunchKernelGGL(k_laplacian, qd_grid2d(G, fl.n), dim3(QD_BLOCK), 0, c->stream,
                                        G, fl, coslat, c->dlat, c->dlon, c->p.a));
}
// ... 352 lines not shown
    }
}

template <int RR>
static void qd_launch_gauss_rows(qd_ctx* c, const double* in, double* out, const QdGaussW& W, int mode_wrap, int clip01,
                                 const double* scale_p, double scale_k, int m_out) {
    constexpr int OWN = QD_BLOCK - 2 * RR;
    QD_ROWS(c, m_out, G, hipLaunchKernelGGL(k_gauss_rows<RR>, dim3((G.nlon + OWN - 1) / OWN, (G.nrows + QD_GB - 1) / QD_GB),
                                            dim3(QD_BLOCK), 0, c->stream, G, in, out, W, mode_wrap, clip01, scale_p, scale_k));
}

static bool qd_gauss_weights(double sigma, QdGaussW& W) {
    const int r = (int)(4.0 * sigma + 0.5);
    if (r > QD_GAUSS_MAXR) return false;
    W.r = r;
    std::vector<double> phi(2 * r + 1);
    const double s2 = sigma * sigma;
    for (int x = -r; x <= r; ++x) phi[x + r] = std::exp(-0.5 / s2 * (double)(x * x));
    double tot;
    const int m = 2 * r + 1;
    if (m < 8) { tot = 0.0; for (int k = 0; k < m; ++k) tot += phi[k]; }
    else {
        double acc[8];
        for (int k = 0; k < 8; ++k) acc[k] = phi[k];
        int k = 8;
        for (; k < m - (m % 8); k += 8) for (int t = 0; t < 8; ++t) acc[t] += phi[k + t];
        tot = ((acc[0] + acc[1]) + (acc[2] + acc[3])) + ((acc[4] + acc[5]) + (acc[6] + acc[7]));
        for (; k < m; ++k) tot += phi[k];
    }
    for (int k = 0; k <= r; ++k) W.w[k] = phi[r + k] / tot;
    return true;
}

struct QdGaussPairP { int op; double w_mem, w_p, w_src, tend, c_floor; };
template <int RR>
__device__ __forceinline__ void qd_gauss_rows_pass(const QdGeom& G, const double* __restrict__ in, double sc, const double (&w)[RR + 1],
                                                   int mode_wrap, int i0, int nvalid, int jbase, double (*sm)[QD_BLOCK], double (&acc)[QD_GB]) {
    {
        const int s = threadIdx.x;
        const int jj = jbase - RR + s;
        if (jj < G.nlon + RR) {
            const int j = qd_ext(jj, G.nlon, mode_wrap);
            double x[QD_GB + 2 * RR];
#pragma unroll
            for (int q = 0; q < QD_GB + 2 * RR; ++q) {
                const int qq = q < nvalid + 2 * RR ? q : nvalid + 2 * RR - 1;
                x[q] = in[(size_t)qd_lrow(G, qd_ext(i0 - RR + qq, G.nlat, mode_wrap)) * G.nlon + j] * sc;
            }
#pragma unroll
            for (int k = 0; k < QD_GB; ++k) {
                double tmp = x[k + RR] * w[0];
#pragma unroll
                for (int q = RR; q >= 1; --q) tmp += (x[k + RR - q] + x[k + RR + q]) * w[q];
                sm[k][s] = tmp;
            }
        }
    }
    __syncthreads();
    const int c0 = threadIdx.x;
    if (c0 >= RR && c0 < QD_BLOCK - RR) {
#pragma unroll
        for (int k = 0; k < QD_GB; ++k) {
            double a = sm[k][c0] * w[0];
#pragma unroll
            for (int q = RR; q >= 1; --q) a += (sm[k][c0 - q] + sm[k][c0 + q]) * w[q];
            acc[k] = a;
        }
    }
    __syncthreads();
}

template <int RR>
__global__ void __launch_bounds__(QD_BLOCK)
k_gauss_pair(QdGeom G, const double* __restrict__ inA, const double* __restrict__ inB, QdGaussW W, int mode_wrap,
             const double* __restrict__ scA_p, double scA_k, double scB_k, const double* __restrict__ sc, QdGaussPairP P,
             double* __restrict__ outA, double* __restrict__ outB, double* __restrict__ out0) {
    constexpr int OWN = QD_BLOCK - 2 * RR;
    __shared__ double sm[QD_GB][QD_BLOCK];
    const int i0 = G.row0 + (int)blockIdx.y * QD_GB;
    const int nvalid = min(QD_GB, G.row0 + G.nrows - i0);
    const int jbase = (int)blockIdx.x * OWN;
    double w[RR + 1];
#pragma unroll
    for (int k = 0; k <= RR; ++k) w[k] = W.w[k];
    const double al = (P.op == 1) ? sc[1] : 0.0;
    double a[QD_GB], b[QD_GB];
#pragma unroll
    for (int k = 0; k < QD_GB; ++k) { a[k] = 0.0; b[k] = 0.0; }
    qd_gauss_rows_pass<RR>(G, inA, scA_p ? *scA_p : scA_k, w, mode_wrap, i0, nvalid, jbase, sm, a);
    if (P.op != 1 || al != 0.0) qd_gauss_rows_pass<RR>(G, inB, scB_k, w, mode_wrap, i0, nvalid, jbase, sm, b);
    const int c0 = threadIdx.x;
    const int j = jbase + c0 - RR;
    if (c0 < RR || c0 >= QD_BLOCK - RR || j >= G.nlon) return;
#pragma unroll
    for (int k = 0; k < QD_GB; ++k) {
        if (k >= nvalid) break;
        const size_t o = (size_t)qd_lrow(G, i0 + k) * G.nlon + j;
        if (P.op == 1) {
            double p = a[k];
            if (al != 0.0) p = (1.0 - al) * p + al * b[k];
            out0[o] = qd_max(p, 0.0);
        } else {
            const double cp = qd_clip(a[k], 0.0, 1.0), sr = qd_clip(b[k], 0.0, 1.0);
            outA[o] = cp; outB[o] = sr;
            const double c0v = out0[o];
            const double tendency = sr * P.tend;
            double c = (P.w_mem * c0v + P.w_p * cp + P.w_src * qd_clip(c0v + tendency, 0.0, 1.0));
            if (P.c_floor > 0.0) c = qd_max(c, qd_clip(P.c_floor * cp, 0.0, 1.0));
            out0[o] = qd_clip(c, 0.0, 1.0);
        }
    }
}

bool qd_gauss_pair_ok(const qd_ctx* c, double sigma) {
    const int r = qd_gauss_radius(sigma);
    return c->use_fused && c->merge_pointwise && sigma > 1e-15 && c->geo.nlon > 2 * r && (r == 1 || r == 2 || r == 4);
}
int qd_gaussian_pair(qd_ctx* c, const double* inA, const double* inB, double sigma, int mode_wrap, const double* scA_p, double scA_k,
                     double scB_k, const double* sc, int op, const double* blend5, double* outA, double* outB, double* out0, int m_out) {
    QdGaussW W;
    if (!qd_gauss_weights(sigma, W)) return qd_fail(c, "gaussian radius too large");
    QdGaussPairP P{op, 0, 0, 0, 0, 0};
    if (blend5) { P.w_mem = blend5[0]; P.w_p = blend5[1]; P.w_src = blend5[2]; P.tend = blend5[3]; P.c_floor = blend5[4]; }
    const int r = W.r;
    QD_ROWS(c, m_out, G,
        const dim3 grid((G.nlon + (QD_BLOCK - 2 * r) - 1) / (QD_BLOCK - 2 * r), (G.nrows + QD_GB - 1) / QD_GB);
        if (r == 1) hipLaunchKernelGGL(k_gauss_pair<1>, grid, dim3(QD_BLOCK), 0, c->stream, G, inA, inB, W, mode_wrap, scA_p, scA_k, scB_k, sc, P, outA, outB, out0);
        else if (r == 2) hipLaunchKernelGGL(k_gauss_pair<2>, grid, dim3(QD_BLOCK), 0, c->stream, G, inA, inB, W, mode_wrap, scA_p, scA_k, scB_k, sc, P, outA, outB, out0);
        else hipLaunchKernelGGL(k_gauss_pair<4>, grid, dim3(QD_BLOCK), 0, c->stream, G, inA, inB, W, mode_wrap, scA_p, scA_k, scB_k, sc, P, outA, outB, out0));
    return 0;
}

int qd_gaussian(qd_ctx* c, const double* in, double* out, double* tmp, double sigma, int mode_wrap, int m_out, int clip01,
                const double* scale_p, double scale_k) {
    const bool scaled = scale_p != nullptr || scale_k != 1.0;
    if (scaled && !(c->use_fused && out != in && sigma > 1e-15 && c->geo.nlon > 2 * qd_gauss_radius(sigma)))
        return qd_fail(c, "qd_gaussian: input scaling needs the fused blur");
    if (!(sigma > 1e-15)) {
        if (out != in) hipMemcpyAsync(out, in, c->geo.cells() * sizeof(double), hipMemcpyDeviceToDevice, c->stream);
        qd_mark(c, {out}, m_out);
        return 0;
    }
    QdGaussW W;
    if (!qd_gauss_weights(sigma, W)) return qd_fail(c, "gaussian radius too large");
    const int r = W.r;
    if (c->use_fused && out != in && c->geo.nlon > 2 * r && (r == 1 || r == 2 || r == 4)) {
        QdScope sc(c, r == 1 ? "k_gauss_rows1" : (r == 2 ? "k_gauss_rows2" : "k_gauss_rows4"));
        if (r == 1) qd_launch_gauss_rows<1>(c, in, out, W, mode_wrap, clip01, scale_p, scale_k, m_out);
        else if (r == 2) qd_launch_gauss_rows<2>(c, in, out, W, mode_wrap, clip01, scale_p, scale_k, m_out);
        else qd_launch_gauss_rows<4>(c, in, out, W, mode_wrap, clip01, scale_p, scale_k, m_out);
        qd_mark(c, {out}, m_out);
        return 0;
    }
    if (c->use_fused && out != in && c->geo.nlon > 2 * r) {
        QdScope sc(c, "k_gauss_fused");
        QD_ROWS(c, m_out, G, hipLaunchKernelGGL(k_gauss_fused, qd_grid2d(G), dim3(QD_BLOCK), 0, c->stream, G, in, out, W, mode_wrap, clip01, scale_p, scale_k));
// ... 112 lines not shown
```

qingdai_amd/csrc/qd_stream.h:

```cpp
#pragma once
#include "qd_internal.h"
#include "qd_device.h"
#include "qd_fused.h"
#include "qd_wave.h"

#ifndef QS_STAMP
#define QS_STAMP(k) ((void)0)
#endif

#define QS_TC 58

struct QsRec { const double* in; const double* aux; double* out; const double* tab; int skip; int pad_; };

struct QsDynArgs {
    QdGeom G;
    const double *poleA, *c8, *c9;
    const double *h, *fric;
    double dt, inv_dlon, inv_2dlon, inv_dlat, inv_2dlat, pgf_y;
    int vb, ntc, nrs, exact;
    QsRec rec[5];
};

struct QsOcnArgs {
    QdGeom G;
    const double *poleA, *fcor, *igx, *rx;
    const double *uo, *vo, *eta;
    const uint8_t* land;
    const double* eta_mean;
    double eta_cap, sub_dt, g, r_bot, inv_2dlon, inv_2dlat, inv_a, inv_rhoH;
    int vb, ntc, nrs, exact;
    QsRec rec[3];
};

typedef unsigned int qs_u32x2 __attribute__((ext_vector_type(2)));
typedef __amdgpu_buffer_rsrc_t qs_rsrc;
#define QS_RSRC_FLAGS 0x00020000
#define QS_OOB 0x80000000u

__device__ __forceinline__ qs_rsrc qs_make_rsrc(const void* p, unsigned bytes) {
    return __builtin_amdgcn_make_buffer_rsrc(const_cast<void*>(p), 0, (int)bytes, QS_RSRC_FLAGS);
}
__device__ __forceinline__ double qs_ld(qs_rsrc r, unsigned row, unsigned vo) {
    return __builtin_bit_cast(double, __builtin_amdgcn_raw_buffer_load_b64(r, vo, row * 8u, 0));
}
__device__ __forceinline__ void qs_st(qs_rsrc r, unsigned row, unsigned vo, double v) {
    __builtin_amdgcn_raw_buffer_store_b64(__builtin_bit_cast(qs_u32x2, v), r, vo, row * 8u, 0);
}
__device__ __forceinline__ int qs_ld8(qs_rsrc r, unsigned row, unsigned vo8) {
    return (int)__builtin_amdgcn_raw_buffer_load_b8(r, vo8, row, 0);
}

__device__ __forceinline__ unsigned qs_off(const QdGeom& G, int g) {
    g = qd_clampi(g, 0, G.nlat - 1);
    int l = qd_lrow(G, g);
    l = l < G.lrows_ ? l : G.lrows_ - 1;
    return (unsigned)l * (unsigned)G.nlon;
}
__device__ __forceinline__ unsigned qs_off_roll(const QdGeom& G, int g) {
    if (g < 0) g += G.nlat; else if (g >= G.nlat) g -= G.nlat;
    return qs_off(G, g);
}

#ifndef QS_PD_DYN
#define QS_PD_DYN 4
// ... 7 lines not shown
    unsigned vo, vs, vo8;
    unsigned slab_bytes;
    bool west_edge, east_edge;
};

enum { QS_FAST = 0, QS_EXACT = 2 };

template <int V> __device__ __forceinline__ double qs_clip200(double x, bool& bad) {
    if (V == QS_EXACT) return qd_clip(x, -200.0, 200.0);
    bad |= qd_nonfinite(x);
    return fmin(fmax(x, -200.0), 200.0);
}


__device__ __forceinline__ double qs_own(double x) {
#if QS_OWN_ASM
    double y;
    asm("v_mov_b64 %0, %1" : "=v"(y) : "v"(x));
    return y;
#else
    const int lo = __builtin_amdgcn_update_dpp(0, __double2loint(x), 0xE4, 0xf, 0xf, true);
    const int hi = __builtin_amdgcn_update_dpp(0, __double2hiint(x), 0xE4, 0xf, 0xf, true);
    return __hiloint2double(hi, lo);
#endif
}

template <int V, int PD> struct QsSrcPlain {
    qs_rsrc p; const QdGeom& G; const QsW& W; double q[PD]; unsigned ro;
    __device__ __forceinline__ void start(int g0, bool&) {
        ro = qs_off(G, g0);
#pragma unroll
        for (int k = 0; k < PD; ++k) { q[k] = qs_ld(p, ro, W.vo); ro += W.nlon; }
    }
    template <int K> __device__ __forceinline__ double get(int, bool&) { return qs_own(q[K % PD]); }
    template <int K> __device__ __forceinline__ double get_edge(int g, bool& bad) { return get<K>(g, bad); }
    template <int K> __device__ __forceinline__ void refill() { q[K % PD] = qs_ld(p, ro, W.vo); ro += W.nlon; }
};

template <bool PRIM, int V, int PD> struct QsSrcLat {
    const QsDynArgs& A; const QsW& W;
    qs_rsrc H, FR, X, Y;
    double hm, hc, hq[PD], x[PD], y[PD], fr[PD];
    unsigned ro;
    __device__ __forceinline__ void start(int g0, bool&) {
        hm = qs_ld(H, qs_off(A.G, g0 - 1), W.vo);
        ro = qs_off(A.G, g0);
        hc = qs_ld(H, ro, W.vo);
#pragma unroll
        for (int k = 0; k < PD; ++k) {
            x[k] = qs_ld(X, ro, W.vo); fr[k] = qs_ld(FR, ro, W.vo); y[k] = PRIM ? qs_ld(Y, ro, W.vo) : 0.0;
            ro += W.nlon;
            hq[k] = qs_ld(H, ro, W.vo);
        }
    }
    template <int EDGE> __device__ __forceinline__ double eval(int g, double hn, double x0, double y0, double f0, bool& bad) {
        double dh = (hn - hm) * A.inv_2dlat;
        if (EDGE) { if (g == 0) dh = (hn - hc) * A.inv_dlat; if (g == W.n - 1) dh = (hc - hm) * A.inv_dlat; }
        double val;
        if (PRIM) {
            const double vx = x0 + (A.pgf_y * dh - qd_sload(A.c9, g) * y0 - f0 * x0) * A.dt;
            val = qs_clip200<V>(vx, bad);
        } else {
            const double u_g = qs_clip200<V>(qd_sload(A.c8, g) * dh, bad);
            const double ur = x0 * 0.8 + u_g * 0.2;
            val = ur + (-f0 * ur) * A.dt;
        }
        hm = hc; hc = hn;
        return val;
    }
    template <int K> __device__ __forceinline__ double get(int g, bool& bad) { return eval<0>(g, qs_own(hq[K % PD]), x[K % PD], y[K % PD], fr[K % PD], bad); }
    template <int K> __device__ __forceinline__ double get_edge(int g, bool& bad) { return eval<1>(g, qs_own(hq[K % PD]), x[K % PD], y[K % PD], fr[K % PD], bad); }
    template <int K> __device__ __forceinline__ void refill() {
        x[K % PD] = qs_ld(X, ro, W.vo); fr[K % PD] = qs_ld(FR, ro, W.vo); if (PRIM) y[K % PD] = qs_ld(Y, ro, W.vo);
        ro += W.nlon;
        hq[K % PD] = qs_ld(H, ro, W.vo);
    }
};

template <bool PRIM, int V, int PD, bool EC> struct QsSrcLon {
    const QsDynArgs& A; const QsW& W;
    qs_rsrc H, FR, X, Y;
    double hh[PD], x[PD], y[PD], fr[PD];
    unsigned ro;
    template <int K> __device__ __forceinline__ void load() {
        hh[K % PD] = qs_ld(H, ro, W.vo); x[K % PD] = qs_ld(X, ro, W.vo); fr[K % PD] = qs_ld(FR, ro, W.vo); y[K % PD] = PRIM ? qs_ld(Y, ro, W.vo) : 0.0;
        ro += W.nlon;
    }
    __device__ __forceinline__ void start(int g0, bool&) {
        ro = qs_off(A.G, g0);
        load<0>(); if (PD > 1) load<1>(); if (PD > 2) { load<2>(); load<3>(); }
    }
    __device__ __forceinline__ double eval(int g, double hc, double x0, double y0, double f0, bool& bad) {
        const double hw = qd_west(hc), he = qd_east(hc);
        double dh;
        if (EC) {
            const double inv_lon = (W.west_edge || W.east_edge) ? A.inv_dlon : A.inv_2dlon;
            dh = ((W.east_edge ? hc : he) - (W.west_edge ? hc : hw)) * inv_lon;
        } else dh = (he - hw) * A.inv_2dlon;
        double val;
        if (PRIM) {
            const double ux = x0 + (qd_sload(A.c8, g) * dh + qd_sload(A.c9, g) * y0 - f0 * x0) * A.dt;
            val = qs_clip200<V>(ux, bad);
        } else {
            const double v_g = qs_clip200<V>(qd_sload(A.c9, g) * dh, bad);
            const double vr = x0 * 0.8 + v_g * 0.2;
            val = vr + (-f0 * vr) * A.dt;
        }
        return val;
    }
    template <int K> __device__ __forceinline__ double get(int g, bool& bad) { return eval(g, hh[K % PD], x[K % PD], y[K % PD], fr[K % PD], bad); }
    template <int K> __device__ __forceinline__ double get_edge(int g, bool& bad) { return get<K>(g, bad); }
    template <int K> __device__ __forceinline__ void refill() { load<K>(); }
};

template <int V> __device__ __forceinline__ double qs_eta(double raw, bool defer, double em, double cap, bool& bad) {
    if (V == QS_EXACT) {
        if (!defer) return raw;
        return qd_clip(qd_nn(raw - em), -cap, cap);
    }
    const double e = raw - em;
    bad |= qd_nonfinite(e);
    return fmin(fmax(e, -cap), cap);
}

template <int V, int PD> struct QsSrcEta {
    const QsOcnArgs& A; const QsW& W; qs_rsrc E; bool defer; double em, cap; double q[PD]; unsigned ro;
    __device__ __forceinline__ void start(int g0, bool&) {
        ro = qs_off(A.G, g0);
#pragma unroll
        for (int k = 0; k < PD; ++k) { q[k] = qs_ld(E, ro, W.vo); ro += W.nlon; }
    }
    template <int K> __device__ __forceinline__ double get(int, bool& bad) { return qs_eta<V>(qs_own(q[K % PD]), defer, em, cap, bad); }
    template <int K> __device__ __forceinline__ double get_edge(int g, bool& bad) { return get<K>(g, bad); }
    template <int K> __device__ __forceinline__ void refill() { q[K % PD] = qs_ld(E, ro, W.vo); ro += W.nlon; }
};

template <int V, int PD> struct QsSrcOcnU {
    const QsOcnArgs& A; const QsW& W; qs_rsrc E, U, Vv, T, L; bool defer; double em, cap;
    double e[PD], u0[PD], v0[PD], tx[PD]; int ld[PD]; unsigned ro;
    template <int K> __device__ __forceinline__ void load() {
        e[K % PD] = qs_ld(E, ro, W.vo); u0[K % PD] = qs_ld(U, ro, W.vo); v0[K % PD] = qs_ld(Vv, ro, W.vo); tx[K % PD] = qs_ld(T, ro, W.vo);
        ld[K % PD] = qs_ld8(L, ro, W.vo8);
        ro += W.nlon;
    }
    __device__ __forceinline__ void start(int g0, bool&) {
        ro = qs_off(A.G, g0);
        load<0>(); if (PD > 1) load<1>(); if (PD > 2) { load<2>(); load<3>(); }
    }
    __device__ __forceinline__ double eval(int g, double eraw, double u, double v, double t, int land, bool& bad) {
        const double ec = qs_eta<V>(eraw, defer, em, cap, bad);
        const double f = qd_sload(A.fcor, g);
        const double gx = ((qd_east(ec) - qd_west(ec)) * A.inv_2dlon) * qd_sload(A.igx, g);
        const double du = (f * v - A.g * gx + t * A.inv_rhoH - A.r_bot * u);
        double un = u + A.sub_dt * du;
        if (land == 1) un = 0.0;
        const double sx = A.sub_dt * qd_sload(A.rx, g);
        return un - sx * un;
    }
    template <int K> __device__ __forceinline__ double get(int g, bool& bad) { return eval(g, e[K % PD], u0[K % PD], v0[K % PD], tx[K % PD], ld[K % PD], bad); }
    template <int K> __device__ __forceinline__ double get_edge(int g, bool& bad) { return get<K>(g, bad); }
    template <int K> __device__ __forceinline__ void refill() { load<K>(); }
};

template <int V, int PD> struct QsSrcOcnV {
    const QsOcnArgs& A; const QsW& W; qs_rsrc E, U, Vv, T, L; bool defer; double em, cap;
    double es, ec, en[PD], u0[PD], v0[PD], ty[PD]; int ld[PD];
    unsigned ro;
    template <int K> __device__ __forceinline__ void load() {
        u0[K % PD] = qs_ld(U, ro, W.vo); v0[K % PD] = qs_ld(Vv, ro, W.vo); ty[K % PD] = qs_ld(T, ro, W.vo);
        ld[K % PD] = qs_ld8(L, ro, W.vo8);
        ro += W.nlon;
        en[K % PD] = qs_ld(E, ro, W.vo);
    }
    __device__ __forceinline__ void start(int g0, bool& bad) {
        es = qs_eta<V>(qs_ld(E, qs_off_roll(A.G, g0 - 1), W.vo), defer, em, cap, bad);
        ro = qs_off(A.G, g0);
        ec = qs_eta<V>(qs_ld(E, ro, W.vo), defer, em, cap, bad);
        load<0>(); if (PD > 1) load<1>(); if (PD > 2) { load<2>(); load<3>(); }
    }
    template <int EDGE> __device__ __forceinline__ double eval(int g, double enr, double u, double v, double t, int land, bool& bad) {
        if (EDGE) { if (g == W.n - 1) enr = qs_ld(E, qs_off_roll(A.G, g + 1), W.vo); }
        const double enc = qs_eta<V>(enr, defer, em, cap, bad);
        const double f = qd_sload(A.fcor, g);
        const double gy = ((enc - es) * A.inv_2dlat) * A.inv_a;
        const double dv = (-f * u - A.g * gy + t * A.inv_rhoH - A.r_bot * v);
        double vn = v + A.sub_dt * dv;
        if (land == 1) vn = 0.0;
        const double sx = A.sub_dt * qd_sload(A.rx, g);
        es = ec; ec = enc;
        return vn - sx * vn;
    }
    template <int K> __device__ __forceinline__ double get(int g, bool& bad) { return eval<0>(g, qs_own(en[K % PD]), u0[K % PD], v0[K % PD], ty[K % PD], ld[K % PD], bad); }
    template <int K> __device__ __forceinline__ double get_edge(int g, bool& bad) { return eval<1>(g, qs_own(en[K % PD]), u0[K % PD], v0[K % PD], ty[K % PD], ld[K % PD], bad); }
    template <int K> __device__ __forceinline__ void refill() { load<K>(); }
};

template <int V> __device__ __forceinline__ double qs_d2(double c) {
    return (V == QS_EXACT ? (qd_east(c) - 2.0 * c) : __builtin_fma(-2.0, c, qd_east(c))) + qd_west(c);
}
template <int V> __device__ __forceinline__ double qs_nn(double x) { return V == QS_EXACT ? qd_nnf(x) : x; }

struct QsCoef { double a, p, q, k; };
__device__ __forceinline__ QsCoef qs_coef(const double* tab, int r, int n) {
    r = qd_clampi(r, 0, n - 1);
    const qd_cptr t = (qd_cptr)(unsigned long long)tab + 4u * (unsigned)r;
    return QsCoef{t[0], t[1], t[2], t[3]};
}

struct QsPipe {
    double f1, f2, f3, f4;
    double gf1, gf2;
// ... 23 lines not shown
template <int STAGE, int K, int V, class SRC, class OUT>
__device__ __forceinline__ void qs_step(SRC& S, QsPipe& p, int gg, const QsW& W, const double* tab, double dt, OUT& out, bool& bad) {
    QsCoef k0, k2;
    if (STAGE >= 4) { k2 = QsCoef{p.kp[0], p.kp[1], p.kp[2], p.kp[3]}; k0 = QsCoef{p.kp[8], p.kp[9], p.kp[10], p.kp[11]}; p.kp += 4; }
    else { k0 = qs_coef(tab, STAGE >= 1 ? gg - 2 : 0, W.n); k2 = qs_coef(tab, STAGE >= 3 ? gg - 4 : 0, W.n); }
    const double x = qs_nn<V>(S.template get<K>(gg, bad));
    double gb = 0.0, dn = 0.0, gb2 = 0.0;
    if (STAGE >= 1) {
        gb = k0.a * (x - p.f2);
        if (STAGE >= 2) dn = qs_nn<V>(k0.p * (gb - p.gf2) + k0.q * qs_d2<V>(p.f2));
    }
    if (STAGE >= 3) {
        gb2 = k2.a * (dn - p.d2);
        if (STAGE >= 4) {
            const double L2 = k2.p * (gb2 - p.gd2) + k2.q * qs_d2<V>(p.d2);
            double val = p.f4 - (k2.k * L2) * dt;
            if (V == QS_EXACT) val = qd_nnf(val); else bad |= qd_nonfinite(val);
            out.put(val);
        }
    }
    p.f4 = p.f3; p.f3 = p.f2; p.f2 = p.f1; p.f1 = x;
    if (STAGE >= 1) { p.gf2 = p.gf1; p.gf1 = gb; }
    if (STAGE >= 2) { p.d2 = p.d1; p.d1 = dn; }
    if (STAGE >= 3) { p.gd2 = p.gd1; p.gd1 = gb2; }
    QS_REFILL(S, K);
}

template <int V, class SRC, class OUT>
__device__ __forceinline__ bool qs_del4_stream(SRC& S, const QdGeom& G, const QsW& W, const double* poleA,
                                               const QsRec QD_CONST* fp, double dt, OUT& out) {
    const int n = W.n, o0 = W.o0, o1 = W.o1;
    bool bad = false;
    if (fp->skip) {
        S.start(o0, bad);
#define QS_PASS(K) if (g + K < o1) { const int gg = g + K; \
            const double x = (gg == 0 || gg == n - 1) ? S.template get_edge<K>(gg, bad) : S.template get<K>(gg, bad); \
            out.put(x); QS_REFILL(S, K); }
        for (int g = o0; g < o1; g += 4) { QS_PASS(0) QS_PASS(1) QS_PASS(2) QS_PASS(3) }
#undef QS_PASS
        return bad;
    }
    const double* __restrict__ tab = fp->tab;
    const bool top = o0 == 0, bot = o1 == n;
    QsPipe p{0, 0, 0, 0, 0, 0, 0, 0, 0, 0, (qd_cptr)(unsigned long long)tab + 4u * (unsigned)o0};
    if (!top) {
        S.start(o0 - 4, bad);
        qs_step<0, 0, V>(S, p, o0 - 4, W, tab, dt, out, bad);
        qs_step<0, 1, V>(S, p, o0 - 3, W, tab, dt, out, bad);
        qs_step<1, 2, V>(S, p, o0 - 2, W, tab, dt, out, bad);
        qs_step<1, 3, V>(S, p, o0 - 1, W, tab, dt, out, bad);
        qs_step<2, 0, V>(S, p, o0, W, tab, dt, out, bad);
        qs_step<2, 1, V>(S, p, o0 + 1, W, tab, dt, out, bad);
        qs_step<3, 2, V>(S, p, o0 + 2, W, tab, dt, out, bad);
        qs_step<3, 3, V>(S, p, o0 + 3, W, tab, dt, out, bad);
    } else {
        const double pA0 = qd_sload(poleA, 0);
        S.start(0, bad);
        const double x0 = qs_nn<V>(S.template get_edge<0>(0, bad));
        QS_REFILL(S, 0);
        const double x1 = qs_nn<V>(S.template get<1>(1, bad));
        QS_REFILL(S, 1);
        p.f2 = x0; p.f1 = x1;
        p.gf1 = pA0 * (x1 - x0); p.gf2 = p.gf1;
        qs_step<2, 2, V>(S, p, 2, W, tab, dt, out, bad);
        const double dd0 = p.d1;
        qs_step<2, 3, V>(S, p, 3, W, tab, dt, out, bad);
        p.gd1 = pA0 * (p.d1 - dd0); p.gd2 = p.gd1;
    }
    QS_STAMP(1);
    const int gEnd = bot ? n - 1 : o1 + 4;
    int g = o0 + 4;
    __builtin_amdgcn_s_waitcnt(0x0F70);
    for (; g + 4 <= gEnd; g += 4) {
        qs_step<4, 0, V>(S, p, g, W, tab, dt, out, bad);
        qs_step<4, 1, V>(S, p, g + 1, W, tab, dt, out, bad);
        qs_step<4, 2, V>(S, p, g + 2, W, tab, dt, out, bad);
        qs_step<4, 3, V>(S, p, g + 3, W, tab, dt, out, bad);
    }
    const int rem = gEnd - g;
    if (rem > 0) qs_step<4, 0, V>(S, p, g, W, tab, dt, out, bad);
    if (rem > 1) qs_step<4, 1, V>(S, p, g + 1, W, tab, dt, out, bad);
    if (rem > 2) qs_step<4, 2, V>(S, p, g + 2, W, tab, dt, out, bad);
    if (bot) {
        const double pA5 = qd_sload(poleA, 5);
        {
            const QsCoef k0 = qs_coef(tab, n - 3, n), k2 = qs_coef(tab, n - 5, n);
            double xe;
            switch (rem) {
            case 0: xe = S.template get_edge<0>(n - 1, bad); break;
            case 1: xe = S.template get_edge<1>(n - 1, bad); break;
// ... 56 lines not shown
    W.vs = QS_OOB;
#endif
    W.slab_bytes = (unsigned)(G.lrows_ + QD_PAD_ROWS) * (unsigned)G.nlon * 8u;
    W.west_edge = W.j == 0; W.east_edge = W.j == G.nlon - 1;
    W.o0 = G.row0 + qs_cut(G.nrows, nrs, vb, rs);
    W.o1 = G.row0 + qs_cut(G.nrows, nrs, vb, rs + 1);
}
__device__ __forceinline__ void qs_strip(const QdGeom& G, int vb, int ntc, int nrs, QsW& W) { qs_strip(G, vb, ntc, nrs, W, blockIdx.x, gridDim.x); }

template <bool PRIM, int V>
__device__ __forceinline__ bool qs_dyn_wave(const QsDynArgs& A, const QsW& W, int wv) {
    const QsDynArgs QD_CONST* Ak = (const QsDynArgs QD_CONST*)__builtin_amdgcn_kernarg_segment_ptr();
    const QsRec QD_CONST* fp = &Ak->rec[wv];
    const unsigned sb = W.slab_bytes;
    QsOutGlobal out{qs_make_rsrc(fp->out, sb), qs_off(A.G, W.o0), W.vs, (unsigned)W.nlon};
    if (wv <= 1) {
        const qs_rsrc H = qs_make_rsrc(A.h, sb), FR = qs_make_rsrc(A.fric, sb), X = qs_make_rsrc(fp->in, sb), Y = qs_make_rsrc(fp->aux, sb);
        if ((wv == 0) == PRIM) {
            if (__builtin_amdgcn_ballot_w64(W.west_edge || W.east_edge) != 0ull) {
                QsSrcLon<PRIM, V, QS_PD_DYN, true> S{A, W, H, FR, X, Y};
                return qs_del4_stream<V>(S, A.G, W, A.poleA, fp, A.dt, out);
            }
            QsSrcLon<PRIM, V, QS_PD_DYN, false> S{A, W, H, FR, X, Y};
            return qs_del4_stream<V>(S, A.G, W, A.poleA, fp, A.dt, out);
        }
        QsSrcLat<PRIM, V, QS_PD_DYN> S{A, W, H, FR, X, Y};
        return qs_del4_stream<V>(S, A.G, W, A.poleA, fp, A.dt, out);
    }
    QsSrcPlain<V, QS_PD_DYN> S{qs_make_rsrc(fp->in, sb), A.G, W};
    return qs_del4_stream<V>(S, A.G, W, A.poleA, fp, A.dt, out);
}

template <int V, class OUT>
__device__ __forceinline__ bool qs_ocn_wave(const QsOcnArgs& A, const QsW& W, int wv, const QsRec QD_CONST* fp, OUT& out) {
    const bool defer = A.eta_mean != nullptr;
    const double em = defer ? *A.eta_mean : 0.0;
    const double cap = (V == QS_EXACT || defer) ? A.eta_cap : __builtin_inf();
    const unsigned sb = W.slab_bytes;
    const qs_rsrc E = qs_make_rsrc(A.eta, sb);
    if (wv <= 1) {
        const qs_rsrc U = qs_make_rsrc(A.uo, sb), Vv = qs_make_rsrc(A.vo, sb), T = qs_make_rsrc(fp->aux, sb), L = qs_make_rsrc(A.land, sb / 8u);
        if (wv == 0) { QsSrcOcnU<V, QS_PD_OCN> S{A, W, E, U, Vv, T, L, defer, em, cap}; return qs_del4_stream<V>(S, A.G, W, A.poleA, fp, A.sub_dt, out); }
        QsSrcOcnV<V, QS_PD_OCN> S{A, W, E, U, Vv, T, L, defer, em, cap};
        return qs_del4_stream<V>(S, A.G, W, A.poleA, fp, A.sub_dt, out);
    }
    QsSrcEta<V, QS_PD_OCN> S{A, W, E, defer, em, cap};
    return qs_del4_stream<V>(S, A.G, W, A.poleA, fp, A.sub_dt, out);
}


const double* qd_stream_tables(qd_ctx* c, int kind, int nf, const double* const* k4row, const double* k4s, const int* skip);
bool qd_stream_ocn_args(qd_ctx* c, const QdOcnArgs& P, QsOcnArgs& A);
```

qingdai_amd/csrc/qd_stream.hip:

```cpp
#include "qd_internal.h"
#include <cstdlib>
#include <cstdio>
#include <vector>
#include <algorithm>

#ifdef QS_STAMPS
__device__ unsigned long long* qs_stamp_buf;
__device__ __forceinline__ void qs_stamp(int slot) {
    if ((threadIdx.x & 63) == 0) {
        const unsigned wid = blockIdx.x * (blockDim.x >> 6) + (threadIdx.x >> 6);
        qs_stamp_buf[(size_t)wid * 8 + slot] = __builtin_amdgcn_s_memrealtime();
        if (slot == 0) {
            unsigned hw, xcc;
            asm volatile("s_getreg_b32 %0, hwreg(HW_REG_HW_ID)" : "=s"(hw));
            asm volatile("s_getreg_b32 %0, hwreg(HW_REG_XCC_ID)" : "=s"(xcc));
            qs_stamp_buf[(size_t)wid * 8 + 4] = hw; qs_stamp_buf[(size_t)wid * 8 + 5] = xcc;
        }
    }
}
#define QS_STAMP(k) qs_stamp(k)
#endif

#include "qd_stream.h"
#include "qd_band.h"

template <bool PRIM>
__global__ void __launch_bounds__(320)
k_dyn_stream(QsDynArgs A) {
    QsW W;
    qs_strip(A.G, A.vb, A.ntc, A.nrs, W);
    const int wv = __builtin_amdgcn_readfirstlane(threadIdx.x >> 6);
    if (wv <= 1) __builtin_amdgcn_s_setprio(2);
    QS_STAMP(0);
    if (!A.exact) {
        const bool bad = qs_dyn_wave<PRIM, QS_FAST>(A, W, wv);
        QS_STAMP(2);
        if (__builtin_amdgcn_ballot_w64(bad) == 0ull) return;
    }
    qs_dyn_wave<PRIM, QS_EXACT>(A, W, wv);
}

__global__ void __launch_bounds__(192)
k_ocn_stream(QsOcnArgs A) {
    QsW W;
    qs_strip(A.G, A.vb, A.ntc, A.nrs, W);
    const int wv = __builtin_amdgcn_readfirstlane(threadIdx.x >> 6);
    if (wv <= 1) __builtin_amdgcn_s_setprio(2);
    const QsOcnArgs QD_CONST* Ak = (const QsOcnArgs QD_CONST*)__builtin_amdgcn_kernarg_segment_ptr();
    const QsRec QD_CONST* fp = &Ak->rec[wv];
    if (!A.exact) {
        QsOutGlobal out{qs_make_rsrc(fp->out, W.slab_bytes), qs_off(A.G, W.o0), W.vs, (unsigned)W.nlon};
        const bool bad = qs_ocn_wave<QS_FAST>(A, W, wv, fp, out);
        if (__builtin_amdgcn_ballot_w64(bad) == 0ull) return;
    }
    QsOutGlobal out{qs_make_rsrc(fp->out, W.slab_bytes), qs_off(A.G, W.o0), W.vs, (unsigned)W.nlon};
    qs_ocn_wave<QS_EXACT>(A, W, wv, fp, out);
}

static int qs_wgs_per_cu(qd_ctx* c, int which) {
    if (c->qs_wgs_per_cu[which] > 0) return c->qs_wgs_per_cu[which];
    int nb = 0;
    hipError_t e = hipSuccess;
    if (which == 0) e = hipOccupancyMaxActiveBlocksPerMultiprocessor(&nb, k_dyn_stream<false>, 320, 0);
    else if (which == 1) e = hipOccupancyMaxActiveBlocksPerMultiprocessor(&nb, k_dyn_stream<true>, 320, 0);
    else e = hipOccupancyMaxActiveBlocksPerMultiprocessor(&nb, k_ocn_stream, 192, 0);
    if (e != hipSuccess || nb < 1) nb = which == 2 ? 6 : 4;
    c->qs_wgs_per_cu[which] = nb;
    return nb;
}

struct QsShape { int R, nrs, vb; };
static QsShape qs_shape(qd_ctx* c, int nrows, int nlon, int which, bool north_pole) {
    const int ntc = (nlon + QS_TC - 1) / QS_TC;
    int R = 0;
    R = which == 2 ? c->tune.stream_r_ocn : c->tune.stream_r_dyn;
    if (R <= 0) R = c->stream_rows;
    int nrs;
    if (R > 0) nrs = std::max(1, nrows / std::max(R, 5));
    else {
        const long target = which == 2 ? 1000 : 760;
        nrs = (int)std::max(1L, (target + ntc / 2) / ntc);
    }
    nrs = std::max(1, std::min(nrs, nrows / 12));
    int vb = 0;
    if (north_pole && nrs > 1) {
        vb = 6;
        if (c->tune.stream_vb >= 0) vb = c->tune.stream_vb;
        while (vb > 0 && nrows - qs_cut(nrows, nrs, vb, nrs - 1) < 12) --vb;
    }
// ... 127 lines not shown
}

int qd_launch_ocn_stream_list(qd_ctx* c, const QdOcnArgs& P, const QdSegList& S) {
    QsOcnArgs A;
    if (!qd_stream_ocn_args(c, P, A)) return qd_fail(c, "fused kernel: coefficient row tables");
    if (S.n == 2 && !c->tune.stream_no_pair && !qd_peer_job_waiting(c)) {
        const QsShape s0 = qs_shape(c, S.g[0].nrows, S.g[0].nlon, 2, S.g[0].row0 + S.g[0].nrows == S.g[0].nlat);
        const QsShape s1 = qs_shape(c, S.g[1].nrows, S.g[1].nlon, 2, S.g[1].row0 + S.g[1].nrows == S.g[1].nlat);
        A.G = S.g[0]; A.vb = s0.vb; A.nrs = s0.nrs; A.ntc = (S.g[0].nlon + QS_TC - 1) / QS_TC;
        qd_launch_ocn_stream_pair(c, A, S.g[1], s1.vb, s1.nrs, (S.g[1].nlon + QS_TC - 1) / QS_TC);
        return 0;
    }
    for (int k = 0; k < S.n; ++k) {
        const QdGeom& G = S.g[k];
        const QsShape sh = qs_shape(c, G.nrows, G.nlon, 2, G.row0 + G.nrows == G.nlat);
        A.G = G; A.vb = sh.vb; A.nrs = sh.nrs; A.ntc = (G.nlon + QS_TC - 1) / QS_TC;
        if (!qd_launch_ocn_stream_push(c, A)) hipLaunchKernelGGL(k_ocn_stream, dim3(A.nrs * A.ntc), dim3(192), 0, c->stream, A);
    }
    return 0;
}

int qd_launch_ocn_stream(qd_ctx* c, const QdOcnArgs& P, int margin) {
    QsOcnArgs A;
    A.poleA = c->tabs.lapPoleA[1];
    A.fcor = c->tabs.fcor; A.igx = c->tabs.ocn_igx; A.rx = c->tabs.r_extra;
    A.uo = P.uo; A.vo = P.vo; A.eta = P.eta; A.land = P.land;
    const double* tab = qd_stream_tables(c, 1, 3, P.k4row, P.k4s, P.skip);
    if (!tab) return qd_fail(c, "fused kernel: coefficient row tables");
    const double* in[3] = {P.uo, P.vo, P.eta};
    const double* aux[3] = {P.taux, P.tauy, nullptr};
    double* out[3] = {P.uo_out, P.vo_out, P.eta_out};
    for (int f = 0; f < 3; ++f) A.rec[f] = QsRec{in[f], aux[f], out[f], tab + (size_t)f * c->geo.nlat * 4, P.skip[f], 0};
    A.eta_mean = P.eta_mean; A.eta_cap = P.eta_cap; A.sub_dt = P.sub_dt; A.g = P.g; A.r_bot = P.r_bot;
    A.inv_2dlon = P.inv_2dlon; A.inv_2dlat = P.inv_2dlat; A.inv_a = P.inv_a; A.inv_rhoH = P.inv_rhoH;
    A.exact = c->fused_fast == 2;
    QdScope sc(c, "k_ocn_hyper", c->geo.full != 0);
    QD_ROWS(c, margin, G,
            const QsShape sh = qs_shape(c, G.nrows, G.nlon, 2, G.row0 + G.nrows == G.nlat);
            A.G = G; A.vb = sh.vb; A.nrs = sh.nrs; A.ntc = (G.nlon + QS_TC - 1) / QS_TC;
            QD_LAUNCH_TIMED(sc, k_ocn_stream, dim3(A.nrs * A.ntc), dim3(192), c->stream, A));
    return 0;
}
```

qingdai_amd/csrc/qd_wave.h:

```cpp
#pragma once
#include "qd_internal.h"

__device__ __forceinline__ double qd_nnf(double x) {
    const double c = fmin(fmax(x, -DBL_MAX), DBL_MAX);
    return (x == x) ? c : 0.0;
}

#define QD_CONST __attribute__((address_space(4)))
typedef const double __attribute__((address_space(4)))* qd_cptr;
__device__ __forceinline__ double qd_sload(const double* p, int idx) { return ((qd_cptr)(unsigned long long)p)[idx]; }
__device__ __forceinline__ bool qd_nonfinite(double x) { return __builtin_amdgcn_class(x, 0x207); }

__device__ __forceinline__ double qd_east(double x) {
    const int lo = __builtin_amdgcn_update_dpp(0, __double2loint(x), 0x130, 0xf, 0xf, true);
    const int hi = __builtin_amdgcn_update_dpp(0, __double2hiint(x), 0x130, 0xf, 0xf, true);
    return __hiloint2double(hi, lo);
}
__device__ __forceinline__ double qd_west(double x) {
    const int lo = __builtin_amdgcn_update_dpp(0, __double2loint(x), 0x138, 0xf, 0xf, true);
    const int hi = __builtin_amdgcn_update_dpp(0, __double2hiint(x), 0x138, 0xf, 0xf, true);
    return __hiloint2double(hi, lo);
}
__device__ __forceinline__ int qd_clampi(int x, int lo, int hi) { return x < lo ? lo : (x > hi ? hi : x); }

// ... 5 lines not shown
    return __builtin_amdgcn_make_buffer_rsrc(const_cast<void*>(p), 0, (int)bytes, QD_BUF_FLAGS);
}
__device__ __forceinline__ double qd_buf_ld(qd_rsrc r, unsigned row, unsigned vo) {
    return __builtin_bit_cast(double, __builtin_amdgcn_raw_buffer_load_b64(r, vo, row * 8u, 0));
}
__device__ __forceinline__ void qd_buf_st(qd_rsrc r, unsigned row, unsigned vo, double v) {
    __builtin_amdgcn_raw_buffer_store_b64(__builtin_bit_cast(qd_u32x2, v), r, vo, row * 8u, 0);
}

__device__ __forceinline__ unsigned qd_xcd_chunk(unsigned L, unsigned nb) {
    const unsigned per = nb >> 3, rem = nb & 7u, x = L & 7u;
    return x * per + (x < rem ? x : rem) + (L >> 3);
}

#define QD_ACC_SLOTS 64
#define QD_ACC_STRIDE 4
#define QD_ACC_WORDS (QD_ACC_SLOTS * QD_ACC_STRIDE + 4)
__device__ __forceinline__ bool qd_acc_arrive(unsigned long long* acc, unsigned w, unsigned nwg, double p) {
    const unsigned k = w & (QD_ACC_SLOTS - 1);
    unsigned long long* a = acc + QD_ACC_STRIDE * k;
    if (fabs(p) < 0x1p62) {
        const double fl = floor(p);
        __hip_atomic_fetch_add(a, (unsigned long long)(long long)fl, __ATOMIC_RELAXED, __HIP_MEMORY_SCOPE_AGENT);
        __hip_atomic_fetch_add(a + 1, (unsigned long long)(long long)((p - fl) * 0x1p50), __ATOMIC_RELAXED, __HIP_MEMORY_SCOPE_AGENT);
    } else {
        __hip_atomic_fetch_or(a + 3, 1ull, __ATOMIC_RELAXED, __HIP_MEMORY_SCOPE_AGENT);
    }
    const unsigned in_slot = (nwg - 1u - k) / QD_ACC_SLOTS + 1u;
    const unsigned slots = nwg < QD_ACC_SLOTS ? nwg : QD_ACC_SLOTS;
    __builtin_amdgcn_s_waitcnt(0x0F70);
    if (__hip_atomic_fetch_add(a + 2, 1ull, __ATOMIC_RELAXED, __HIP_MEMORY_SCOPE_AGENT) != in_slot - 1u) return false;
    return __hip_atomic_fetch_add(acc + QD_ACC_SLOTS * QD_ACC_STRIDE, 1ull, __ATOMIC_RELAXED, __HIP_MEMORY_SCOPE_AGENT) == slots - 1u;
}
__device__ __forceinline__ double qd_acc_finish(unsigned long long* acc, const double* partial, int n, double wsum) {
    const int lane = threadIdx.x & 63;
    unsigned long long* s = acc + QD_ACC_STRIDE * lane;
    long long hi = (long long)__hip_atomic_load(s, __ATOMIC_RELAXED, __HIP_MEMORY_SCOPE_AGENT);
    long long lo = (long long)__hip_atomic_load(s + 1, __ATOMIC_RELAXED, __HIP_MEMORY_SCOPE_AGENT);
    unsigned long long fl = __hip_atomic_load(s + 3, __ATOMIC_RELAXED, __HIP_MEMORY_SCOPE_AGENT);
#pragma unroll
    for (int k = 0; k < QD_ACC_STRIDE; ++k) __hip_atomic_store(s + k, 0ull, __ATOMIC_RELAXED, __HIP_MEMORY_SCOPE_AGENT);
    if (lane == 0) __hip_atomic_store(acc + QD_ACC_SLOTS * QD_ACC_STRIDE, 0ull, __ATOMIC_RELAXED, __HIP_MEMORY_SCOPE_AGENT);
#pragma unroll
    for (int o = 32; o > 0; o >>= 1) { hi += __shfl_down(hi, o, 64); lo += __shfl_down(lo, o, 64); fl |= __shfl_down(fl, o, 64); }
    hi = __shfl(hi, 0, 64); lo = __shfl(lo, 0, 64); fl = __shfl(fl, 0, 64);
    if (fl) {
        double a = 0.0;
        for (int k = lane; k < n; k += 64) a += __hip_atomic_load(partial + k, __ATOMIC_RELAXED, __HIP_MEMORY_SCOPE_AGENT);
#pragma unroll
        for (int o = 32; o > 0; o >>= 1) a += __shfl_down(a, o, 64);
        const double tot = __shfl(a, 0, 64);
        return wsum < 0.0 ? tot : tot / (wsum + 1e-15);
    }
    const double tot = (double)hi + (double)lo * 0x1p-50;
    return wsum < 0.0 ? tot : tot / (wsum + 1e-15);
}
```

qingdai_amd/device.py:

```python
from __future__ import annotations

import ctypes

import numpy as np

from . import _lib
from ._lib import F, QdError
from .params import QdParams


def _c(a, dtype=np.float64):
    return np.ascontiguousarray(a, dtype=dtype)


class Device:
    def __init__(self, grid, params: QdParams | None = None, device=0, row0=0, n_rows=None, halo=0, rank=0, world=1):
        self.lib = _lib.load()
        self.grid = grid
        self.params = params or QdParams.from_env()
        self.shape = (grid.n_lat, grid.n_lon)
        n_rows = grid.n_lat if n_rows is None else n_rows
        desc = _lib.qd_grid_desc(grid.n_lat, grid.n_lon, row0, n_rows, halo, device, rank, world)
        h = ctypes.c_void_p()
        ps = self.params.to_struct()
# ... 470 lines not shown
        return out

    def tiles_planes(self):
        out = np.empty((getattr(self, "_tiles_n", 1),) + self.shape, dtype=np.float64)
        self._chk(self.lib.qd_tiles_download(self.h, 2, out.ctypes.data, out.size), "qd_tiles_download")
        return out

    def phyto_configure(self, n_species, K_h, adv_alpha):
        self._chk(self.lib.qd_phyto_configure(self.h, int(n_species), float(K_h), float(adv_alpha)), "qd_phyto_configure")
        self._phyto_S = int(n_species)

    def phyto_upload(self, C_s):
        C_s = np.ascontiguousarray(C_s, dtype=np.float64)
        assert C_s.ndim == 3 and C_s.shape[0] == getattr(self, "_phyto_S", -1) and C_s.shape[1:] == self.shape
        for s in range(C_s.shape[0]):
            self._chk(self.lib.qd_phyto_upload(self.h, s, C_s[s].ctypes.data), "qd_phyto_upload")

    def phyto_download(self):
        self.flush()
        out = np.zeros((self._phyto_S,) + self.shape, dtype=np.float64)
        for s in range(self._phyto_S):
            self._chk(self.lib.qd_phyto_download(self.h, s, out[s].ctypes.data), "qd_phyto_download")
        return out

    def phyto_advect_diffuse(self, dt_seconds):
        self.flush()
        self._chk(self.lib.qd_phyto_advect_diffuse(self.h, float(dt_seconds)), "qd_phyto_advect_diffuse")

    def last_ocean_nsub(self):
        n = ctypes.c_int(0)
        self.lib.qd_last_ocean_nsub(self.h, ctypes.byref(n))
        return n.value

    def counters(self):
        a, o = ctypes.c_int64(0), ctypes.c_int64(0)
        self.lib.qd_get_step_counter(self.h, ctypes.byref(a), ctypes.byref(o))
        return a.value, o.value

    def set_counters(self, a, o):
        self.lib.qd_set_step_counter(self.h, int(a), int(o))

    def reduce(self, name, op):
        self.flush()
        out = ctypes.c_double(0.0)
        self._chk(self.lib.qd_reduce(self.h, F[name], int(op), ctypes.byref(out)), "qd_reduce")
        return out.value

    def timing(self, on=True, select=None):
        if select:
            self.lib.qd_timing_select(self.h, select.encode())
        else:
            self.lib.qd_timing_enable(self.h, 1 if on else 0)
        self.lib.qd_timing_reset(self.h)

    def timing_get(self, name):
        ms, n = ctypes.c_double(0), ctypes.c_int64(0)
        self.lib.qd_timing_get(self.h, name.encode(), ctypes.byref(ms), ctypes.byref(n))
        return ms.value, n.value

    def _out(self):
        return np.empty(self.shape, dtype=np.float64)

    def op_laplacian(self, Fh, ocean=False):
        a, out = _c(Fh), self._out()
        self._chk(self.lib.qd_op_laplacian(self.h, a.ctypes.data, 1 if ocean else 0, out.ctypes.data), "qd_op_laplacian")
        return out
# ... 72 lines not shown
```

Measured before the change: 5.011 planet-days/s.

## Defer ocean eta-mean reduction into next sub-step's hyperdiffusion kernel and fold precip scalars

Ocean sub-steps no longer finish the global eta mean with a last-arriving-block atomic handshake in the tail kernel. Each tail launch instead adds its partials into a double-buffered fixed-point accumulator, and the next streaming hyperdiffusion launch reads and reduces it. This removes the serialized finishing step and the immediate fix pass. The precipitation path also gets a slab variant of k_precip_raw that reads a precomputed divergence and skips writing pos, plus a precip-scalar reduction that can be folded into the gaussian pair. The exchange adds more atomics, an extra accumulator set, and restrictions that fail loudly on unsupported paths.

```diff
diff --git a/include/qingdai_hip.h b/include/qingdai_hip.h
--- a/include/qingdai_hip.h
+++ b/include/qingdai_hip.h
@@ -101,6 +101,8 @@
 int qd_op_gaussian(qd_handle h, const double* F, double sigma, int mode_wrap, double* out);
 int qd_op_median_positive(qd_handle h, const double* x, double dflt, double* out);
 int qd_median_state(qd_handle h, double* out64);
+int qd_step_scalars(qd_handle h, double* out8);
+int qd_ocean_mean_next_count(qd_handle h, int64_t* out);
 
 int qd_band_insolation(qd_handle h, int nb, const double* specA, const double* specB, const double* tray, double* out_host_or_null);
 
diff --git a/qingdai_amd/_lib.py b/qingdai_amd/_lib.py
--- a/qingdai_amd/_lib.py
+++ b/qingdai_amd/_lib.py
@@ -25,7 +25,7 @@
     "qd_get_step_counter", "qd_set_step_counter", "qd_forcing", "qd_simple_albedo", "qd_atmos_step",
     "qd_ocean_step", "qd_driver_physics", "qd_hydrology_commit", "qd_step_n", "qd_last_ocean_nsub", "qd_sync",
     "qd_op_laplacian", "qd_op_hyperdiffuse", "qd_op_advect", "qd_op_shapiro", "qd_op_zonal_filter", "qd_op_divergence",
-    "qd_op_vorticity", "qd_op_gaussian", "qd_op_median_positive", "qd_median_state", "qd_reduce", "qd_energy_diagnostics", "qd_energy_diagnostics_last", "qd_band_insolation",
+    "qd_op_vorticity", "qd_op_gaussian", "qd_op_median_positive", "qd_median_state", "qd_step_scalars", "qd_ocean_mean_next_count", "qd_reduce", "qd_energy_diagnostics", "qd_energy_diagnostics_last", "qd_band_insolation",
     "qd_comm_unique_id", "qd_comm_init", "qd_comm_init_local", "qd_comm_stats", "qd_comm_allreduce_count", "qd_comm_grouped_sum_count", "qd_comm_init_shm", "qd_comm_host_allreduce_count", "qd_hostring_open", "qd_hostring_allreduce",
     "qd_hostring_close", "qd_comm_barrier", "qd_comm_allreduce_max", "qd_peer_export", "qd_peer_connect", "qd_comm_peer_stats", "qd_comm_peer_carried", "qd_peer_selftest", "qd_peer_disable", "qd_tune_reload",
     "qd_plansim_create", "qd_plansim_destroy", "qd_plansim_plan", "qd_plansim_mark", "qd_plansim_margin", "qd_plansim_segments",
@@ -261,6 +261,8 @@
     lib.qd_comm_barrier.argtypes = [vp]
     lib.qd_comm_init_local.argtypes = [ctypes.POINTER(vp), i32]
     lib.qd_median_state.argtypes = [vp, dp]
+    lib.qd_step_scalars.argtypes = [vp, dp]
+    lib.qd_ocean_mean_next_count.argtypes = [vp, ctypes.POINTER(i64)]
     lib.qd_comm_stats.argtypes = [vp, ctypes.POINTER(i32)]
     lib.qd_comm_allreduce_count.argtypes = [vp, ctypes.POINTER(i32)]
     lib.qd_comm_grouped_sum_count.argtypes = [vp, ctypes.POINTER(i32)]
diff --git a/qingdai_amd/csrc/qd_api.hip b/qingdai_amd/csrc/qd_api.hip
--- a/qingdai_amd/csrc/qd_api.hip
+++ b/qingdai_amd/csrc/qd_api.hip
@@ -316,6 +316,7 @@
     { const char* ef = std::getenv("QD_FUSED"); if (ef && ef[0] == '0') c->use_fused = 0; }
     { const char* ef = std::getenv("QD_FUSED_FAST"); if (ef) c->fused_fast = std::atoi(ef); }
     { const char* ef = std::getenv("QD_TAIL_ACC"); if (ef) c->tail_acc = std::atoi(ef); }
+    { const char* ef = std::getenv("QD_MEAN_IN_MOMENTUM"); if (ef) c->mean_in_momentum = ef[0] == '0' ? 0 : 1; }
     { const char* ef = std::getenv("QD_SHAPIRO_STREAM"); if (ef) c->shapiro_stream = std::atoi(ef); }
     { const char* ef = std::getenv("QD_OCN_TAIL"); if (ef) c->ocn_tail = std::atoi(ef); }
     if (c->ocn_tail != 0) c->ocn_tail = 1;
@@ -349,8 +350,8 @@
     if ((e = hipMalloc(&c->red_partial, (size_t)c->red_blocks * sizeof(double))) != hipSuccess) return bail("hipMalloc", e);
     if ((e = hipMalloc(&c->dscal, QD_S_COUNT * sizeof(double))) != hipSuccess) return bail("hipMalloc", e);
     if ((e = hipMalloc(&c->dcount, 32 * sizeof(unsigned long long))) != hipSuccess) return bail("hipMalloc", e);
-    if ((e = hipMalloc(&c->eta_acc, 512 * sizeof(unsigned long long))) != hipSuccess) return bail("hipMalloc", e);
-    hipMemsetAsync(c->eta_acc, 0, 512 * sizeof(unsigned long long), c->stream);
+    if ((e = hipMalloc(&c->eta_acc, 1024 * sizeof(unsigned long long))) != hipSuccess) return bail("hipMalloc", e);
+    hipMemsetAsync(c->eta_acc, 0, 1024 * sizeof(unsigned long long), c->stream);
     if ((e = hipMalloc(&c->hist, 2 * QD_HIST_BINS * sizeof(unsigned int))) != hipSuccess) return bail("hipMalloc", e);
     if ((e = hipMalloc(&c->sel_state, 8 * sizeof(unsigned long long))) != hipSuccess) return bail("hipMalloc", e);
     hipMemsetAsync(c->dscal, 0, QD_S_COUNT * sizeof(double), c->stream);
@@ -842,6 +843,20 @@
     return 0;
 }
 
+extern "C" int qd_step_scalars(qd_handle c, double* out8) {
+    if (!c || !out8) return -1;
+    hipSetDevice(c->desc.device);
+    QD_HIP(c, hipStreamSynchronize(c->stream));
+    QD_HIP(c, hipMemcpy(out8, c->dscal, sizeof(double) * 8, hipMemcpyDeviceToHost));
+    return 0;
+}
+
+extern "C" int qd_ocean_mean_next_count(qd_handle c, int64_t* out) {
+    if (!c || !out) return -1;
+    *out = c->mean_next_count;
+    return 0;
+}
+
 extern "C" int qd_reduce(qd_handle c, int field, int op, double* out) {
     if (!c || !out) return -1;
     if (field < 0 || field >= QD_F_COUNT_F64) return qd_fail(c, "qd_reduce: unknown field");
diff --git a/qingdai_amd/csrc/qd_blockred.h b/qingdai_amd/csrc/qd_blockred.h
--- a/qingdai_amd/csrc/qd_blockred.h
+++ b/qingdai_amd/csrc/qd_blockred.h
@@ -92,3 +92,22 @@
     }
     __syncthreads();
 }
+
+__device__ __forceinline__ void qd_precip_scalars_wg(const double* __restrict__ partial, int n, double wsum, double pq_min, double p_blend,
+                                                     int use_fb, double* out) {
+    __shared__ double sm[2][QD_BLOCK / 64];
+    double a = 0.0, b = 0.0;
+    for (int k = threadIdx.x; k < n; k += QD_BLOCK) { a += partial[k]; b += partial[n + k]; }
+    a = qd_wave_sum(a); b = qd_wave_sum(b);
+    const int lane = threadIdx.x & 63, wv = threadIdx.x >> 6;
+    if (lane == 0) { sm[0][wv] = a; sm[1][wv] = b; }
+    __syncthreads();
+    if (threadIdx.x == 0) {
+        for (int k = 1; k < QD_BLOCK / 64; ++k) { a += sm[0][k]; b += sm[1][k]; }
+        const double den = b + 1e-20;
+        out[0] = den > 0 ? a / den : 1.0;
+        const double pq_mean = a / (wsum + 1e-15);
+        out[1] = (use_fb && pq_mean < pq_min) ? p_blend : 0.0;
+    }
+    __syncthreads();
+}
diff --git a/qingdai_amd/csrc/qd_fused.h b/qingdai_amd/csrc/qd_fused.h
--- a/qingdai_amd/csrc/qd_fused.h
+++ b/qingdai_amd/csrc/qd_fused.h
@@ -28,6 +28,10 @@
     double eta_cap;
     int fast;
     QdTileShape ts;
+    const unsigned long long* acc_read = nullptr;
+    const double* acc_partial = nullptr;
+    int acc_n = 0;
+    double acc_wsum = 0.0;
 };
 
 
diff --git a/qingdai_amd/csrc/qd_fused.hip b/qingdai_amd/csrc/qd_fused.hip
--- a/qingdai_amd/csrc/qd_fused.hip
+++ b/qingdai_amd/csrc/qd_fused.hip
@@ -728,6 +728,7 @@
 
 int qd_launch_ocn_hyper(qd_ctx* c, QdOcnArgs& P, int margin) {
     if (qd_ocn_stream_ok(c, margin)) return qd_launch_ocn_stream(c, P, margin);
+    if (P.acc_read) return qd_fail(c, "k_ocn_hyper: an unfinished eta mean needs the streaming kernel");
     qd_tile_init(c);
     P.ts = c->tile;
     P.fast = c->fused_fast != 0;
diff --git a/qingdai_amd/csrc/qd_internal.h b/qingdai_amd/csrc/qd_internal.h
--- a/qingdai_amd/csrc/qd_internal.h
+++ b/qingdai_amd/csrc/qd_internal.h
@@ -240,6 +240,8 @@
     QdTileShape tile{0, 0, 0, 0};
     int use_fused = 1;
     int fused_fast = 1;
+    long long mean_next_count = 0;
+    int mean_in_momentum = 1;
     int tail_acc = 1;
     unsigned long long* eta_acc = nullptr;
     int shapiro_stream = 1;
@@ -383,8 +385,10 @@
 int  qd_gaussian(qd_ctx* c, const double* in, double* out, double* tmp, double sigma, int mode_wrap, int m_out, int clip01 = 0,
                  const double* scale_p = nullptr, double scale_k = 1.0);
 bool qd_gauss_pair_ok(const qd_ctx* c, double sigma);
+struct QdPrecipFold { const double* partial; int n; double wsum, pq_min, p_blend; int use_fb; double dcrit; double* out; };
 int  qd_gaussian_pair(qd_ctx* c, const double* inA, const double* inB, double sigma, int mode_wrap, const double* scA_p, double scA_k,
-                      double scB_k, const double* sc, int op, const double* blend5, double* outA, double* outB, double* out0, int m_out = 0);
+                      double scB_k, const double* sc, int op, const double* blend5, double* outA, double* outB, double* out0, int m_out = 0,
+                      const QdPrecipFold* fold = nullptr);
 int  qd_gaussian_swap(qd_ctx* c, double*& field, double*& tmp, double sigma, int mode_wrap, int m_out, int clip01 = 0,
                       const double* scale_p = nullptr, double scale_k = 1.0);
 bool qd_gauss_can_fuse(const qd_ctx* c, double sigma);
diff --git a/qingdai_amd/csrc/qd_ocean.hip b/qingdai_amd/csrc/qd_ocean.hip
--- a/qingdai_amd/csrc/qd_ocean.hip
+++ b/qingdai_amd/csrc/qd_ocean.hip
@@ -818,6 +818,11 @@
     const bool use_fused1 = use_tail && !band && c->ocn_fused && c->ocn_tail == 1 && tail_acc && c->fused_fast == 1 && do_diff &&
                             p.ocean_k4_nsub == 1 && !do_shap && HP.use_q && HP.K_h > 0.0 && qd_ocn_fused_ok(c) &&
                             !c->k4_ocn_skip[0] && !c->k4_ocn_skip[1] && !c->k4_ocn_skip[2];
+    const bool mean_form_ok = c->mean_in_momentum && !band && G0.full && tail_acc && !use_fused1 && do_diff && c->use_fused && n_sub > 1 &&
+                              p.ocean_k4_nsub == 1 && !do_shap && qd_ocn_tail_is_fast(c) && qd_ocn_stream_ok(c, 0);
+    if (mean_form_ok) fix_now = false;
+    const bool mean_next_ok = mean_form_ok;
+    unsigned long long* acc_pending = nullptr;
     for (int s = 0; s < n_sub; ++s) {
         if (use_fused1) {
             QdOcnArgs O;
@@ -869,6 +874,7 @@
             O.inv_2dlon = 1.0 / (2.0 * c->dlon); O.inv_2dlat = 1.0 / (2.0 * c->dlat); O.inv_a = 1.0 / p.a; O.inv_rhoH = 1.0 / (p.rho_w * H);
             O.eta_mean = (defer_eta && s > 0) ? mean_ptr : nullptr;
             O.eta_cap = p.eta_cap;
+            if (acc_pending) { O.acc_read = acc_pending; O.acc_partial = c->red_partial; O.acc_n = qd_ocn_tail_tiles(c, Gown); O.acc_wsum = c->wsum_ocean; }
             int m_int = 0;
             bool split = false;
             if (pending) {
@@ -958,6 +964,10 @@
                 else qd_mark(c, {F[QD_F_ETA], A.Ts_out, A.uo_out, A.vo_out}, m);
             } else {
             if (fix_now) { A.fix_count = c->fix_count; A.fix_list = c->fix_list; }
+            A.acc_clear = acc_pending;
+            acc_pending = (mean_next_ok && s + 1 < n_sub) ? QD_ACC_NEXT_SET(c->eta_acc, s & 1) : nullptr;
+            A.acc_next = acc_pending;
+            if (acc_pending) c->mean_next_count++;
             if (qd_launch_ocn_tail(c, Gown, A)) return -1;
             if (!tail_acc)
                 hipLaunchKernelGGL(k_eta_mean_tail, dim3(1), dim3(256), 0, c->stream, c->red_partial, qd_ocn_tail_tiles(c, Gown), c->wsum_ocean,
diff --git a/qingdai_amd/csrc/qd_ocntail.h b/qingdai_amd/csrc/qd_ocntail.h
--- a/qingdai_amd/csrc/qd_ocntail.h
+++ b/qingdai_amd/csrc/qd_ocntail.h
@@ -18,11 +18,14 @@
     const double* eta_in = nullptr;
     unsigned int* fix_count = nullptr;
     unsigned long long* fix_list = nullptr;
+    unsigned long long* acc_next = nullptr;
+    unsigned long long* acc_clear = nullptr;
     QdPeerFold pf;
 };
 
 int qd_ocn_tail_tiles(const qd_ctx* c, const QdGeom& G);
 int qd_launch_ocn_tail(qd_ctx* c, const QdGeom& G, QdTailArgs& P);
+bool qd_ocn_tail_is_fast(const qd_ctx* c);
 
 struct QdOcnArgs;
 bool qd_ocn_fused_ok(const qd_ctx* c);
diff --git a/qingdai_amd/csrc/qd_ocntail.hip b/qingdai_amd/csrc/qd_ocntail.hip
--- a/qingdai_amd/csrc/qd_ocntail.hip
+++ b/qingdai_amd/csrc/qd_ocntail.hip
@@ -617,6 +617,11 @@
     if (FIX) __syncthreads();
     acc = qd_wave_sum(acc);
     if (W.lane == 0) __hip_atomic_store(P.partial + w, acc, __ATOMIC_RELAXED, __HIP_MEMORY_SCOPE_AGENT);
+    if (!FIX && P.acc_clear && w == 0u) qd_acc_clear_set(P.acc_clear);
+    if (!FIX && P.acc_next) {
+        if (W.lane == 0) qd_acc_add(P.acc_next, w, acc);
+        return;
+    }
     if (P.acc) {
         const bool last = W.lane == 0 && qd_acc_arrive(P.acc, w, gridDim.x, acc);
         if (__builtin_amdgcn_ballot_w64(last) != 0ull) {
@@ -910,6 +915,7 @@
 static int qt_rows(const qd_ctx* c) { return c->tune.tail_r > 0 ? c->tune.tail_r : 7; }
 
 static bool qt_use_fast(const qd_ctx* c) { return !c->tune.tail_v && c->ocn_tail == 1; }
+bool qd_ocn_tail_is_fast(const qd_ctx* c) { return qt_use_fast(c); }
 static int qt_fast_rows(const qd_ctx* c, const QdGeom& G) {
     if (c->tune.tail_r > 0) return c->tune.tail_r;
     const int ntc = (G.nlon + QS_TCF - 1) / QS_TCF;
@@ -954,6 +960,8 @@
     if (!stamps) { hipMalloc(&stamps, stamp_words * 8); hipMemcpyToSymbol(HIP_SYMBOL(qt_stamp_buf), &stamps, sizeof(stamps)); }
     hipMemsetAsync(stamps, 0, stamp_words * 8, c->stream);
 #endif
+    if ((P.acc_next || P.acc_clear) && (!fast || P.fix_count || !G.full))
+        return qd_fail(c, "k_ocn_tail: the mean of a sub-step can only be left to the next launch by the storing fast form");
     if (!fast || !P.acc) { P.fix_count = nullptr; P.fix_list = nullptr; }
     if (fast && P.fix_count) QD_LAUNCH_TIMED(sc, k_ocn_tail_fast<true>, dim3(nrs * P.ntc), dim3(128), c->stream, G, c->tabs, P);
     else if (fast) QD_LAUNCH_TIMED(sc, k_ocn_tail_fast<false>, dim3(nrs * P.ntc), dim3(128), c->stream, G, c->tabs, P);
diff --git a/qingdai_amd/csrc/qd_physics.hip b/qingdai_amd/csrc/qd_physics.hip
--- a/qingdai_amd/csrc/qd_physics.hip
+++ b/qingdai_amd/csrc/qd_physics.hip
@@ -8,6 +8,7 @@
 QdColP qd_make_colp(const qd_ctx* c, double dt);
 
 
+template <bool SLAB>
 __global__ void __launch_bounds__(QD_BLOCK)
 k_precip_raw(QdGeom G, QdTabs T, const double* __restrict__ u, const double* __restrict__ v,
              const double* __restrict__ pcond, double a, double dlat, double dlon, double D_crit, double beta,
@@ -22,7 +23,7 @@
     const double scale = qd_max(*scale_p, 1e-12);
     double s_num = 0.0, s_den = 0.0;
     for (int j = threadIdx.x; j < G.nlon; j += QD_BLOCK) {
-        const double div = qd_divvort_point(G, T, u, v, i, j, a, dlat, dlon, 0);
+        const double div = SLAB ? u[b + j] : qd_divvort_point(G, T, u, v, i, j, a, dlat, dlon, 0);
         const double pos = qd_max(0.0, -(div - D_crit));
         const double F_div = anypos ? qd_clip(pos / scale, 0.0, 5.0) : 0.0;
         const double Pq = qd_max(0.0, pcond[b + j]);
@@ -30,7 +31,7 @@
         const double F = (1.0 + beta * F_div) * F_orog;
         const double pr = Pq * F;
         praw[b + j] = pr;
-        pos_out[b + j] = pos;
+        if (!SLAB) pos_out[b + j] = pos;
         s_num += Pq * w;
         s_den += pr * w;
     }
@@ -68,20 +69,7 @@
 __global__ void __launch_bounds__(QD_BLOCK)
 k_precip_scalars(const double* __restrict__ partial, int n, double wsum, double pq_min, double p_blend, int use_fb,
                  double* __restrict__ out) {
-    __shared__ double sm[2][QD_BLOCK / 64];
-    double a = 0.0, b = 0.0;
-    for (int k = threadIdx.x; k < n; k += QD_BLOCK) { a += partial[k]; b += partial[n + k]; }
-    a = qd_wave_sum(a); b = qd_wave_sum(b);
-    const int lane = threadIdx.x & 63, wv = threadIdx.x >> 6;
-    if (lane == 0) { sm[0][wv] = a; sm[1][wv] = b; }
-    __syncthreads();
-    if (threadIdx.x == 0) {
-        for (int k = 1; k < QD_BLOCK / 64; ++k) { a += sm[0][k]; b += sm[1][k]; }
-        const double den = b + 1e-20;
-        out[0] = den > 0 ? a / den : 1.0;
-        const double pq_mean = a / (wsum + 1e-15);
-        out[1] = (use_fb && pq_mean < pq_min) ? p_blend : 0.0;
-    }
+    qd_precip_scalars_wg(partial, n, wsum, pq_min, p_blend, use_fb, out);
 }
 
 __global__ void __launch_bounds__(QD_BLOCK)
@@ -359,7 +347,7 @@
                 auto run = [&](int r0, int r1) {
                     if (r1 <= r0) return;
                     QdGeom g2 = G; g2.row0 = r0; g2.nrows = r1 - r0;
-                    hipLaunchKernelGGL(k_precip_raw, dim3(1, g2.nrows), blk, 0, c->stream, g2, c->tabs, F[QD_F_U], F[QD_F_V],
+                    hipLaunchKernelGGL(k_precip_raw<false>, dim3(1, g2.nrows), blk, 0, c->stream, g2, c->tabs, F[QD_F_U], F[QD_F_V],
                                        F[QD_F_PCOND], p.a, c->dlat, c->dlon, p.D_crit, p.p_betadiv, c->dscal + QD_S_PSCALE,
                                        c->dcount, praw, pos, rp + (size_t)2 * G0.lrows(), orog);
                 };
@@ -368,10 +356,16 @@
                 else { run(a0, std::max(a0, own0)); run(std::min(a1, own1), a1); }
             }
         }
-        hipLaunchKernelGGL(k_precip_raw, dim3(1, Gown.nrows), blk, 0, c->stream, Gown, c->tabs, F[QD_F_U], F[QD_F_V],
+        const bool fold = !band && !orog && qd_gauss_pair_ok(c, 1.0);
+        if (fold)
+            hipLaunchKernelGGL(k_precip_raw<true>, dim3(1, Gown.nrows), blk, 0, c->stream, Gown, c->tabs, tmp, (const double*)nullptr,
+                               F[QD_F_PCOND], p.a, c->dlat, c->dlon, p.D_crit, p.p_betadiv, c->dscal + QD_S_PSCALE, c->dcount, praw,
+                               (double*)nullptr, rp, orog);
+        else
+        hipLaunchKernelGGL(k_precip_raw<false>, dim3(1, Gown.nrows), blk, 0, c->stream, Gown, c->tabs, F[QD_F_U], F[QD_F_V],
                            F[QD_F_PCOND], p.a, c->dlat, c->dlon, p.D_crit, p.p_betadiv, c->dscal + QD_S_PSCALE, c->dcount, praw,
                            pos, rp, orog);
-        qd_mark(c, {praw, pos}, m);
+        if (fold) qd_mark(c, {praw}, m); else qd_mark(c, {praw, pos}, m);
         if (band && qd_peer_hooks(c)) {
             QdPeerHook H; H.pre = 2; H.partial = rp; H.n = Gown.nrows;
             H.post = 1; H.wsum = c->wsum_all; H.pq_min = p.pq_min; H.p_blend = p.p_blend; H.use_fb = p.p_hybrid_fallback; H.out = c->dscal + QD_S_RENORM;
@@ -382,11 +376,18 @@
             if (qd_allreduce_f64(c, c->dscal + QD_S_TMP0, 2, 0)) return -1;
             hipLaunchKernelGGL(k_precip_scalars_post, dim3(1), dim3(64), 0, c->stream, c->dscal + QD_S_TMP0, c->wsum_all, p.pq_min,
                                p.p_blend, p.p_hybrid_fallback, c->dscal + QD_S_RENORM);
-        } else {
+        } else if (!fold) {
             hipLaunchKernelGGL(k_precip_scalars, dim3(1), blk, 0, c->stream, rp, Gown.nrows, c->wsum_all, p.pq_min,
                                p.p_blend, p.p_hybrid_fallback, c->dscal + QD_S_RENORM);
         }
-        if (qd_gauss_pair_ok(c, 1.0)) {
+        if (fold) {
+            const int mg = qd_plan(c, {QD_IN(praw, R1), QD_IN(tmp, R1)});
+            if (mg < 0) return -1;
+            const QdPrecipFold PF{rp, Gown.nrows, c->wsum_all, p.pq_min, p.p_blend, p.p_hybrid_fallback, p.D_crit, c->dscal + QD_S_RENORM};
+            if (qd_gaussian_pair(c, praw, tmp, 1.0, 0, nullptr, 1.0, p.k_precip, nullptr, 1, nullptr, nullptr, nullptr,
+                                 F[QD_F_PRECIP], mg, &PF)) return -1;
+            qd_mark(c, {F[QD_F_PRECIP]}, mg);
+        } else if (qd_gauss_pair_ok(c, 1.0)) {
             const int mg = qd_plan(c, {QD_IN(praw, R1), QD_IN(pos, R1)});
             if (mg < 0) return -1;
             if (qd_gaussian_pair(c, praw, pos, 1.0, 0, c->dscal + QD_S_RENORM, 1.0, p.k_precip, c->dscal + QD_S_RENORM, 1, nullptr,
diff --git a/qingdai_amd/csrc/qd_stencil.hip b/qingdai_amd/csrc/qd_stencil.hip
--- a/qingdai_amd/csrc/qd_stencil.hip
+++ b/qingdai_amd/csrc/qd_stencil.hip
@@ -1,6 +1,7 @@
 #include "qd_internal.h"
 #include "qd_device.h"
 #include "qd_wave.h"
+#include "qd_blockred.h"
 #include <cstdlib>
 
 __global__ void __launch_bounds__(QD_BLOCK)
@@ -419,10 +420,14 @@
     return true;
 }
 
-struct QdGaussPairP { int op; double w_mem, w_p, w_src, tend, c_floor; };
-template <int RR>
+struct QdGaussPairP {
+    int op; double w_mem, w_p, w_src, tend, c_floor;
+    int fold, fold_n, use_fb; const double* partial; double wsum, pq_min, p_blend, dcrit; double* scal_out;
+};
+template <int RR, bool POS>
 __device__ __forceinline__ void qd_gauss_rows_pass(const QdGeom& G, const double* __restrict__ in, double sc, const double (&w)[RR + 1],
-                                                   int mode_wrap, int i0, int nvalid, int jbase, double (*sm)[QD_BLOCK], double (&acc)[QD_GB]) {
+                                                   int mode_wrap, int i0, int nvalid, int jbase, double (*sm)[QD_BLOCK], double (&acc)[QD_GB],
+                                                   double dcrit = 0.0) {
     {
         const int s = threadIdx.x;
         const int jj = jbase - RR + s;
@@ -432,7 +437,8 @@
 #pragma unroll
             for (int q = 0; q < QD_GB + 2 * RR; ++q) {
                 const int qq = q < nvalid + 2 * RR ? q : nvalid + 2 * RR - 1;
-                x[q] = in[(size_t)qd_lrow(G, qd_ext(i0 - RR + qq, G.nlat, mode_wrap)) * G.nlon + j] * sc;
+                const double v = in[(size_t)qd_lrow(G, qd_ext(i0 - RR + qq, G.nlat, mode_wrap)) * G.nlon + j];
+                x[q] = (POS ? qd_max(0.0, -(v - dcrit)) : v) * sc;
             }
 #pragma unroll
             for (int k = 0; k < QD_GB; ++k) {
@@ -470,12 +476,22 @@
     double w[RR + 1];
 #pragma unroll
     for (int k = 0; k <= RR; ++k) w[k] = W.w[k];
-    const double al = (P.op == 1) ? sc[1] : 0.0;
+    double scA, al;
+    if (P.fold) {
+        __shared__ double s_sc[2];
+        qd_precip_scalars_wg(P.partial, P.fold_n, P.wsum, P.pq_min, P.p_blend, P.use_fb, s_sc);
+        if (threadIdx.x == 0 && blockIdx.x == 0 && blockIdx.y == 0) { P.scal_out[0] = s_sc[0]; P.scal_out[1] = s_sc[1]; }
+        scA = s_sc[0]; al = s_sc[1];
+    } else {
+        scA = scA_p ? *scA_p : scA_k;
+        al = (P.op == 1) ? sc[1] : 0.0;
+    }
     double a[QD_GB], b[QD_GB];
 #pragma unroll
     for (int k = 0; k < QD_GB; ++k) { a[k] = 0.0; b[k] = 0.0; }
-    qd_gauss_rows_pass<RR>(G, inA, scA_p ? *scA_p : scA_k, w, mode_wrap, i0, nvalid, jbase, sm, a);
-    if (P.op != 1 || al != 0.0) qd_gauss_rows_pass<RR>(G, inB, scB_k, w, mode_wrap, i0, nvalid, jbase, sm, b);
+    qd_gauss_rows_pass<RR, false>(G, inA, scA, w, mode_wrap, i0, nvalid, jbase, sm, a);
+    if (P.fold) { if (al != 0.0) qd_gauss_rows_pass<RR, true>(G, inB, scB_k, w, mode_wrap, i0, nvalid, jbase, sm, b, P.dcrit); }
+    else if (P.op != 1 || al != 0.0) qd_gauss_rows_pass<RR, false>(G, inB, scB_k, w, mode_wrap, i0, nvalid, jbase, sm, b);
     const int c0 = threadIdx.x;
     const int j = jbase + c0 - RR;
     if (c0 < RR || c0 >= QD_BLOCK - RR || j >= G.nlon) return;
@@ -504,11 +520,17 @@
     return c->use_fused && c->merge_pointwise && sigma > 1e-15 && c->geo.nlon > 2 * r && (r == 1 || r == 2 || r == 4);
 }
 int qd_gaussian_pair(qd_ctx* c, const double* inA, const double* inB, double sigma, int mode_wrap, const double* scA_p, double scA_k,
-                     double scB_k, const double* sc, int op, const double* blend5, double* outA, double* outB, double* out0, int m_out) {
+                     double scB_k, const double* sc, int op, const double* blend5, double* outA, double* outB, double* out0, int m_out,
+                     const QdPrecipFold* fold) {
     QdGaussW W;
     if (!qd_gauss_weights(sigma, W)) return qd_fail(c, "gaussian radius too large");
-    QdGaussPairP P{op, 0, 0, 0, 0, 0};
+    QdGaussPairP P{op, 0, 0, 0, 0, 0, 0, 0, 0, nullptr, 0, 0, 0, 0, nullptr};
     if (blend5) { P.w_mem = blend5[0]; P.w_p = blend5[1]; P.w_src = blend5[2]; P.tend = blend5[3]; P.c_floor = blend5[4]; }
+    if (fold) {
+        if (op != 1 || !c->geo.full) return qd_fail(c, "qd_gaussian_pair: the folded scalars belong to the precipitation blend of a whole-globe handle");
+        P.fold = 1; P.fold_n = fold->n; P.use_fb = fold->use_fb; P.partial = fold->partial; P.wsum = fold->wsum; P.pq_min = fold->pq_min;
+        P.p_blend = fold->p_blend; P.dcrit = fold->dcrit; P.scal_out = fold->out;
+    }
     const int r = W.r;
     QD_ROWS(c, m_out, G,
         const dim3 grid((G.nlon + (QD_BLOCK - 2 * r) - 1) / (QD_BLOCK - 2 * r), (G.nrows + QD_GB - 1) / QD_GB);
diff --git a/qingdai_amd/csrc/qd_stream.h b/qingdai_amd/csrc/qd_stream.h
--- a/qingdai_amd/csrc/qd_stream.h
+++ b/qingdai_amd/csrc/qd_stream.h
@@ -30,6 +30,10 @@
     double eta_cap, sub_dt, g, r_bot, inv_2dlon, inv_2dlat, inv_a, inv_rhoH;
     int vb, ntc, nrs, exact;
     QsRec rec[3];
+    const unsigned long long* acc_read = nullptr;
+    const double* acc_partial = nullptr;
+    int acc_n = 0;
+    double acc_wsum = 0.0;
 };
 
 typedef unsigned int qs_u32x2 __attribute__((ext_vector_type(2)));
@@ -103,6 +107,7 @@
 #pragma unroll
         for (int k = 0; k < PD; ++k) { q[k] = qs_ld(p, ro, W.vo); ro += W.nlon; }
     }
+    __device__ __forceinline__ void settle(bool&) {}
     template <int K> __device__ __forceinline__ double get(int, bool&) { return qs_own(q[K % PD]); }
     template <int K> __device__ __forceinline__ double get_edge(int g, bool& bad) { return get<K>(g, bad); }
     template <int K> __device__ __forceinline__ void refill() { q[K % PD] = qs_ld(p, ro, W.vo); ro += W.nlon; }
@@ -124,6 +129,7 @@
             hq[k] = qs_ld(H, ro, W.vo);
         }
     }
+    __device__ __forceinline__ void settle(bool&) {}
     template <int EDGE> __device__ __forceinline__ double eval(int g, double hn, double x0, double y0, double f0, bool& bad) {
         double dh = (hn - hm) * A.inv_2dlat;
         if (EDGE) { if (g == 0) dh = (hn - hc) * A.inv_dlat; if (g == W.n - 1) dh = (hc - hm) * A.inv_dlat; }
@@ -161,6 +167,7 @@
         ro = qs_off(A.G, g0);
         load<0>(); if (PD > 1) load<1>(); if (PD > 2) { load<2>(); load<3>(); }
     }
+    __device__ __forceinline__ void settle(bool&) {}
     __device__ __forceinline__ double eval(int g, double hc, double x0, double y0, double f0, bool& bad) {
         const double hw = qd_west(hc), he = qd_east(hc);
         double dh;
@@ -194,13 +201,24 @@
     return fmin(fmax(e, -cap), cap);
 }
 
+__device__ __forceinline__ double qs_mean_handover(const QsOcnArgs& A, double* sy, bool reader) {
+    if (reader) {
+        const double m = qd_acc_read(A.acc_read, A.acc_partial, A.acc_n, A.acc_wsum);
+        if ((threadIdx.x & 63) == 0) __hip_atomic_store(sy, m, __ATOMIC_RELAXED, __HIP_MEMORY_SCOPE_WORKGROUP);
+        __builtin_amdgcn_s_waitcnt(0xC07F);
+    }
+    __builtin_amdgcn_s_barrier();
+    return __hip_atomic_load(sy, __ATOMIC_RELAXED, __HIP_MEMORY_SCOPE_WORKGROUP);
+}
+
 template <int V, int PD> struct QsSrcEta {
-    const QsOcnArgs& A; const QsW& W; qs_rsrc E; bool defer; double em, cap; double q[PD]; unsigned ro;
+    const QsOcnArgs& A; const QsW& W; qs_rsrc E; bool defer; double em, cap; double q[PD]; unsigned ro; double* sy = nullptr;
     __device__ __forceinline__ void start(int g0, bool&) {
         ro = qs_off(A.G, g0);
 #pragma unroll
         for (int k = 0; k < PD; ++k) { q[k] = qs_ld(E, ro, W.vo); ro += W.nlon; }
     }
+    __device__ __forceinline__ void settle(bool&) { if (sy) em = qs_mean_handover(A, sy, true); }
     template <int K> __device__ __forceinline__ double get(int, bool& bad) { return qs_eta<V>(qs_own(q[K % PD]), defer, em, cap, bad); }
     template <int K> __device__ __forceinline__ double get_edge(int g, bool& bad) { return get<K>(g, bad); }
     template <int K> __device__ __forceinline__ void refill() { q[K % PD] = qs_ld(E, ro, W.vo); ro += W.nlon; }
@@ -208,7 +226,8 @@
 
 template <int V, int PD> struct QsSrcOcnU {
     const QsOcnArgs& A; const QsW& W; qs_rsrc E, U, Vv, T, L; bool defer; double em, cap;
-    double e[PD], u0[PD], v0[PD], tx[PD]; int ld[PD]; unsigned ro;
+    double e[PD], u0[PD], v0[PD], tx[PD]; int ld[PD]; unsigned ro; double* sy = nullptr;
+    __device__ __forceinline__ void settle(bool&) { if (sy) em = qs_mean_handover(A, sy, false); }
     template <int K> __device__ __forceinline__ void load() {
         e[K % PD] = qs_ld(E, ro, W.vo); u0[K % PD] = qs_ld(U, ro, W.vo); v0[K % PD] = qs_ld(Vv, ro, W.vo); tx[K % PD] = qs_ld(T, ro, W.vo);
         ld[K % PD] = qs_ld8(L, ro, W.vo8);
@@ -237,17 +256,23 @@
     const QsOcnArgs& A; const QsW& W; qs_rsrc E, U, Vv, T, L; bool defer; double em, cap;
     double es, ec, en[PD], u0[PD], v0[PD], ty[PD]; int ld[PD];
     unsigned ro;
+    double* sy = nullptr;
     template <int K> __device__ __forceinline__ void load() {
         u0[K % PD] = qs_ld(U, ro, W.vo); v0[K % PD] = qs_ld(Vv, ro, W.vo); ty[K % PD] = qs_ld(T, ro, W.vo);
         ld[K % PD] = qs_ld8(L, ro, W.vo8);
         ro += W.nlon;
         en[K % PD] = qs_ld(E, ro, W.vo);
     }
-    __device__ __forceinline__ void start(int g0, bool& bad) {
-        es = qs_eta<V>(qs_ld(E, qs_off_roll(A.G, g0 - 1), W.vo), defer, em, cap, bad);
+    __device__ __forceinline__ void start(int g0, bool&) {
+        es = qs_ld(E, qs_off_roll(A.G, g0 - 1), W.vo);
         ro = qs_off(A.G, g0);
-        ec = qs_eta<V>(qs_ld(E, ro, W.vo), defer, em, cap, bad);
+        ec = qs_ld(E, ro, W.vo);
         load<0>(); if (PD > 1) load<1>(); if (PD > 2) { load<2>(); load<3>(); }
+    }
+    __device__ __forceinline__ void settle(bool& bad) {
+        if (sy) em = qs_mean_handover(A, sy, false);
+        es = qs_eta<V>(es, defer, em, cap, bad);
+        ec = qs_eta<V>(ec, defer, em, cap, bad);
     }
     template <int EDGE> __device__ __forceinline__ double eval(int g, double enr, double u, double v, double t, int land, bool& bad) {
         if (EDGE) { if (g == W.n - 1) enr = qs_ld(E, qs_off_roll(A.G, g + 1), W.vo); }
@@ -337,7 +362,7 @@
     const int n = W.n, o0 = W.o0, o1 = W.o1;
     bool bad = false;
     if (fp->skip) {
-        S.start(o0, bad);
+        S.start(o0, bad); S.settle(bad);
 #define QS_PASS(K) if (g + K < o1) { const int gg = g + K; \
             const double x = (gg == 0 || gg == n - 1) ? S.template get_edge<K>(gg, bad) : S.template get<K>(gg, bad); \
             out.put(x); QS_REFILL(S, K); }
@@ -349,7 +374,7 @@
     const bool top = o0 == 0, bot = o1 == n;
     QsPipe p{0, 0, 0, 0, 0, 0, 0, 0, 0, 0, (qd_cptr)(unsigned long long)tab + 4u * (unsigned)o0};
     if (!top) {
-        S.start(o0 - 4, bad);
+        S.start(o0 - 4, bad); S.settle(bad);
         qs_step<0, 0, V>(S, p, o0 - 4, W, tab, dt, out, bad);
         qs_step<0, 1, V>(S, p, o0 - 3, W, tab, dt, out, bad);
         qs_step<1, 2, V>(S, p, o0 - 2, W, tab, dt, out, bad);
@@ -360,7 +385,7 @@
         qs_step<3, 3, V>(S, p, o0 + 3, W, tab, dt, out, bad);
     } else {
         const double pA0 = qd_sload(poleA, 0);
-        S.start(0, bad);
+        S.start(0, bad); S.settle(bad);
         const double x0 = qs_nn<V>(S.template get_edge<0>(0, bad));
         QS_REFILL(S, 0);
         const double x1 = qs_nn<V>(S.template get<1>(1, bad));
@@ -483,20 +508,36 @@
 }
 
 template <int V, class OUT>
-__device__ __forceinline__ bool qs_ocn_wave(const QsOcnArgs& A, const QsW& W, int wv, const QsRec QD_CONST* fp, OUT& out) {
-    const bool defer = A.eta_mean != nullptr;
-    const double em = defer ? *A.eta_mean : 0.0;
+__device__ __forceinline__ bool qs_ocn_wave(const QsOcnArgs& A, const QsW& W, int wv, const QsRec QD_CONST* fp, OUT& out,
+                                            double* sy = nullptr, double* em_io = nullptr) {
+    const bool handover = em_io != nullptr && A.acc_read != nullptr;
+    const bool defer = handover || A.eta_mean != nullptr;
+    const double em = handover ? *em_io : (defer ? *A.eta_mean : 0.0);
+    if (!handover) sy = nullptr;
     const double cap = (V == QS_EXACT || defer) ? A.eta_cap : __builtin_inf();
     const unsigned sb = W.slab_bytes;
     const qs_rsrc E = qs_make_rsrc(A.eta, sb);
+    bool bad;
     if (wv <= 1) {
         const qs_rsrc U = qs_make_rsrc(A.uo, sb), Vv = qs_make_rsrc(A.vo, sb), T = qs_make_rsrc(fp->aux, sb), L = qs_make_rsrc(A.land, sb / 8u);
-        if (wv == 0) { QsSrcOcnU<V, QS_PD_OCN> S{A, W, E, U, Vv, T, L, defer, em, cap}; return qs_del4_stream<V>(S, A.G, W, A.poleA, fp, A.sub_dt, out); }
+        if (wv == 0) {
+            QsSrcOcnU<V, QS_PD_OCN> S{A, W, E, U, Vv, T, L, defer, em, cap};
+            S.sy = sy;
+            bad = qs_del4_stream<V>(S, A.G, W, A.poleA, fp, A.sub_dt, out);
+            if (handover) *em_io = S.em;
+            return bad;
+        }
         QsSrcOcnV<V, QS_PD_OCN> S{A, W, E, U, Vv, T, L, defer, em, cap};
-        return qs_del4_stream<V>(S, A.G, W, A.poleA, fp, A.sub_dt, out);
+        S.sy = sy;
+        bad = qs_del4_stream<V>(S, A.G, W, A.poleA, fp, A.sub_dt, out);
+        if (handover) *em_io = S.em;
+        return bad;
     }
     QsSrcEta<V, QS_PD_OCN> S{A, W, E, defer, em, cap};
-    return qs_del4_stream<V>(S, A.G, W, A.poleA, fp, A.sub_dt, out);
+    S.sy = sy;
+    bad = qs_del4_stream<V>(S, A.G, W, A.poleA, fp, A.sub_dt, out);
+    if (handover) *em_io = S.em;
+    return bad;
 }
 
 
diff --git a/qingdai_amd/csrc/qd_stream.hip b/qingdai_amd/csrc/qd_stream.hip
--- a/qingdai_amd/csrc/qd_stream.hip
+++ b/qingdai_amd/csrc/qd_stream.hip
@@ -48,13 +48,15 @@
     if (wv <= 1) __builtin_amdgcn_s_setprio(2);
     const QsOcnArgs QD_CONST* Ak = (const QsOcnArgs QD_CONST*)__builtin_amdgcn_kernarg_segment_ptr();
     const QsRec QD_CONST* fp = &Ak->rec[wv];
+    __shared__ double s_em;
+    double em = 0.0;
     if (!A.exact) {
         QsOutGlobal out{qs_make_rsrc(fp->out, W.slab_bytes), qs_off(A.G, W.o0), W.vs, (unsigned)W.nlon};
-        const bool bad = qs_ocn_wave<QS_FAST>(A, W, wv, fp, out);
+        const bool bad = qs_ocn_wave<QS_FAST>(A, W, wv, fp, out, &s_em, &em);
         if (__builtin_amdgcn_ballot_w64(bad) == 0ull) return;
     }
     QsOutGlobal out{qs_make_rsrc(fp->out, W.slab_bytes), qs_off(A.G, W.o0), W.vs, (unsigned)W.nlon};
-    qs_ocn_wave<QS_EXACT>(A, W, wv, fp, out);
+    qs_ocn_wave<QS_EXACT>(A, W, wv, fp, out, A.exact ? &s_em : (double*)nullptr, &em);
 }
 
 static int qs_wgs_per_cu(qd_ctx* c, int which) {
@@ -248,6 +250,7 @@
     double* out[3] = {P.uo_out, P.vo_out, P.eta_out};
     for (int f = 0; f < 3; ++f) A.rec[f] = QsRec{in[f], aux[f], out[f], tab + (size_t)f * c->geo.nlat * 4, P.skip[f], 0};
     A.eta_mean = P.eta_mean; A.eta_cap = P.eta_cap; A.sub_dt = P.sub_dt; A.g = P.g; A.r_bot = P.r_bot;
+    A.acc_read = P.acc_read; A.acc_partial = P.acc_partial; A.acc_n = P.acc_n; A.acc_wsum = P.acc_wsum;
     A.inv_2dlon = P.inv_2dlon; A.inv_2dlat = P.inv_2dlat; A.inv_a = P.inv_a; A.inv_rhoH = P.inv_rhoH;
     A.exact = c->fused_fast == 2;
     QdScope sc(c, "k_ocn_hyper", c->geo.full != 0);
diff --git a/qingdai_amd/csrc/qd_wave.h b/qingdai_amd/csrc/qd_wave.h
--- a/qingdai_amd/csrc/qd_wave.h
+++ b/qingdai_amd/csrc/qd_wave.h
@@ -61,19 +61,29 @@
     if (__hip_atomic_fetch_add(a + 2, 1ull, __ATOMIC_RELAXED, __HIP_MEMORY_SCOPE_AGENT) != in_slot - 1u) return false;
     return __hip_atomic_fetch_add(acc + QD_ACC_SLOTS * QD_ACC_STRIDE, 1ull, __ATOMIC_RELAXED, __HIP_MEMORY_SCOPE_AGENT) == slots - 1u;
 }
-__device__ __forceinline__ double qd_acc_finish(unsigned long long* acc, const double* partial, int n, double wsum) {
-    const int lane = threadIdx.x & 63;
-    unsigned long long* s = acc + QD_ACC_STRIDE * lane;
-    long long hi = (long long)__hip_atomic_load(s, __ATOMIC_RELAXED, __HIP_MEMORY_SCOPE_AGENT);
-    long long lo = (long long)__hip_atomic_load(s + 1, __ATOMIC_RELAXED, __HIP_MEMORY_SCOPE_AGENT);
-    unsigned long long fl = __hip_atomic_load(s + 3, __ATOMIC_RELAXED, __HIP_MEMORY_SCOPE_AGENT);
+#define QD_ACC_SET_WORDS (QD_ACC_SLOTS * QD_ACC_STRIDE)
+#define QD_ACC_NEXT_SET(acc, k) ((acc) + 512 + (k) * QD_ACC_SET_WORDS)
+__device__ __forceinline__ void qd_acc_add(unsigned long long* acc, unsigned w, double p) {
+    unsigned long long* a = acc + QD_ACC_STRIDE * (w & (QD_ACC_SLOTS - 1));
+    if (fabs(p) < 0x1p62) {
+        const double fl = floor(p);
+        __hip_atomic_fetch_add(a, (unsigned long long)(long long)fl, __ATOMIC_RELAXED, __HIP_MEMORY_SCOPE_AGENT);
+        __hip_atomic_fetch_add(a + 1, (unsigned long long)(long long)((p - fl) * 0x1p50), __ATOMIC_RELAXED, __HIP_MEMORY_SCOPE_AGENT);
+    } else {
+        __hip_atomic_fetch_or(a + 3, 1ull, __ATOMIC_RELAXED, __HIP_MEMORY_SCOPE_AGENT);
+    }
+}
+__device__ __forceinline__ void qd_acc_clear_set(unsigned long long* acc) {
+    unsigned long long* s = acc + QD_ACC_STRIDE * (threadIdx.x & 63);
 #pragma unroll
     for (int k = 0; k < QD_ACC_STRIDE; ++k) __hip_atomic_store(s + k, 0ull, __ATOMIC_RELAXED, __HIP_MEMORY_SCOPE_AGENT);
-    if (lane == 0) __hip_atomic_store(acc + QD_ACC_SLOTS * QD_ACC_STRIDE, 0ull, __ATOMIC_RELAXED, __HIP_MEMORY_SCOPE_AGENT);
+}
+__device__ __forceinline__ double qd_acc_reduce(long long hi, long long lo, unsigned long long fl, const double* partial, int n, double wsum) {
+    const int lane = threadIdx.x & 63;
 #pragma unroll
-    for (int o = 32; o > 0; o >>= 1) { hi += __shfl_down(hi, o, 64); lo += __shfl_down(lo, o, 64); fl |= __shfl_down(fl, o, 64); }
-    hi = __shfl(hi, 0, 64); lo = __shfl(lo, 0, 64); fl = __shfl(fl, 0, 64);
-    if (fl) {
+    for (int o = 32; o > 0; o >>= 1) { hi += __shfl_down(hi, o, 64); lo += __shfl_down(lo, o, 64); }
+    hi = __shfl(hi, 0, 64); lo = __shfl(lo, 0, 64);
+    if (__builtin_amdgcn_ballot_w64(fl != 0ull) != 0ull) {
         double a = 0.0;
         for (int k = lane; k < n; k += 64) a += __hip_atomic_load(partial + k, __ATOMIC_RELAXED, __HIP_MEMORY_SCOPE_AGENT);
 #pragma unroll
@@ -84,3 +94,21 @@
     const double tot = (double)hi + (double)lo * 0x1p-50;
     return wsum < 0.0 ? tot : tot / (wsum + 1e-15);
 }
+__device__ __forceinline__ double qd_acc_read(const unsigned long long* acc, const double* partial, int n, double wsum) {
+    const unsigned long long* s = acc + QD_ACC_STRIDE * (threadIdx.x & 63);
+    const long long hi = (long long)__hip_atomic_load(s, __ATOMIC_RELAXED, __HIP_MEMORY_SCOPE_AGENT);
+    const long long lo = (long long)__hip_atomic_load(s + 1, __ATOMIC_RELAXED, __HIP_MEMORY_SCOPE_AGENT);
+    const unsigned long long fl = __hip_atomic_load(s + 3, __ATOMIC_RELAXED, __HIP_MEMORY_SCOPE_AGENT);
+    return qd_acc_reduce(hi, lo, fl, partial, n, wsum);
+}
+__device__ __forceinline__ double qd_acc_finish(unsigned long long* acc, const double* partial, int n, double wsum) {
+    const int lane = threadIdx.x & 63;
+    unsigned long long* s = acc + QD_ACC_STRIDE * lane;
+    const long long hi = (long long)__hip_atomic_load(s, __ATOMIC_RELAXED, __HIP_MEMORY_SCOPE_AGENT);
+    const long long lo = (long long)__hip_atomic_load(s + 1, __ATOMIC_RELAXED, __HIP_MEMORY_SCOPE_AGENT);
+    const unsigned long long fl = __hip_atomic_load(s + 3, __ATOMIC_RELAXED, __HIP_MEMORY_SCOPE_AGENT);
+#pragma unroll
+    for (int k = 0; k < QD_ACC_STRIDE; ++k) __hip_atomic_store(s + k, 0ull, __ATOMIC_RELAXED, __HIP_MEMORY_SCOPE_AGENT);
+    if (lane == 0) __hip_atomic_store(acc + QD_ACC_SLOTS * QD_ACC_STRIDE, 0ull, __ATOMIC_RELAXED, __HIP_MEMORY_SCOPE_AGENT);
+    return qd_acc_reduce(hi, lo, fl, partial, n, wsum);
+}
diff --git a/qingdai_amd/device.py b/qingdai_amd/device.py
--- a/qingdai_amd/device.py
+++ b/qingdai_amd/device.py
@@ -526,6 +526,16 @@
         self.lib.qd_last_ocean_nsub(self.h, ctypes.byref(n))
         return n.value
 
+    def step_scalars(self):
+        out = np.zeros(8)
+        self._chk(self.lib.qd_step_scalars(self.h, out.ctypes.data_as(ctypes.POINTER(ctypes.c_double))), "qd_step_scalars")
+        return dict(zip(("PREF", "ETA_MEAN", "MED_OUT", "PSCALE", "RENORM", "BLEND_W", "TMP0", "TMP1"), out))
+
+    def ocean_mean_next_count(self):
+        n = ctypes.c_int64(0)
+        self._chk(self.lib.qd_ocean_mean_next_count(self.h, ctypes.byref(n)), "qd_ocean_mean_next_count")
+        return n.value
+
     def counters(self):
         a, o = ctypes.c_int64(0), ctypes.c_int64(0)
         self.lib.qd_get_step_counter(self.h, ctypes.byref(a), ctypes.byref(o))
```

Result: faster. 5.111 planet-days/s (median of 6 runs) (+2.0%).
